# thegedge/StereoReconstruction

Hardware: AMD Instinct MI355X
Metric: Mdisparity-hypotheses/s (WxHxD) (higher is better)
Workload: dtype f64; 1 GPU; C3: synthetic rectified 1920x1080 pair, 256 depth levels, GeodesicWeight r=5; TwoView WTA both directions + cross-check; one pair per GPU; width=1920, height=1080, depth_levels=256, window_radius=5, weights=geodesic, pairs_per_gpu=1, pair_seed_rank0=1592590339, pair_seed_of_rank_r=seed + 0x10000*r, parallelism=single GPU

## Files before the change

### stereoreconstruction_amd/csrc/srh_api.hip

```cpp
#include "srh_internal.hpp"
#include "srh_geom.hpp"

#include <algorithm>
#include <cassert>
#include <cstdarg>
#include <cstdio>
#include <cstdlib>
#include <cstring>
#include <map>
#include <mutex>
#include <string>
#include <utility>
#include <limits>
#include <vector>

using namespace srh;

static thread_local char g_err[512] = "";

static int fail(int code, const char *fmt, ...) {
	va_list ap;
	va_start(ap, fmt);
	vsnprintf(g_err, sizeof(g_err), fmt, ap);
	va_end(ap);
	return code;
}

#define HIP_TRY(expr)                                                                   \
	do {                                                                                \
		hipError_t e_ = (expr);                                                         \
		if (e_ != hipSuccess)                                                           \
			return fail(SRH_E_DEVICE, "%s: %s (%s:%d)", #expr, hipGetErrorString(e_), __FILE__, __LINE__); \
	} while (0)

static thread_local bool g_oom = false;
static thread_local size_t g_alloc_limit = 0;

struct PoolBlock { void *p; size_t bytes; int device; };
static std::mutex g_pool_mu;
static std::vector<PoolBlock> g_pool;
static size_t g_pool_bytes = 0, g_pool_cap = (size_t)65536 << 20;
static const size_t POOL_MIN_BYTES = (size_t)4 << 20;

static void pool_flush(int device) {
	std::vector<PoolBlock> out;
	{
		std::lock_guard<std::mutex> g(g_pool_mu);
		for (size_t k = 0; k < g_pool.size();)
			if (device < 0 || g_pool[k].device == device) { out.push_back(g_pool[k]); g_pool_bytes -= g_pool[k].bytes; g_pool[k] = g_pool.back(); g_pool.pop_back(); }
			else ++k;
	}
	int cur = 0;
	const bool have = hipGetDevice(&cur) == hipSuccess;
	for (const PoolBlock &b : out) { (void)hipSetDevice(b.device); (void)hipFree(b.p); }
	if (have) (void)hipSetDevice(cur);
}
static size_t pool_bytes_on(int device) {
	std::lock_guard<std::mutex> g(g_pool_mu);
	size_t b = 0;
	for (const PoolBlock &k : g_pool) if (k.device == device) b += k.bytes;
	return b;
}
static void pool_give(void *p, size_t bytes) {
	if (!p) return;
	int dev = 0;
	if (bytes >= POOL_MIN_BYTES && hipGetDevice(&dev) == hipSuccess) {
		std::lock_guard<std::mutex> g(g_pool_mu);
		if (g_pool_bytes + bytes <= g_pool_cap) { g_pool.push_back({p, bytes, dev}); g_pool_bytes += bytes; return; }
	}
	(void)hipFree(p);
}
static void *pool_take(size_t bytes, size_t *got) {
	int dev = 0;
	if (bytes < POOL_MIN_BYTES || hipGetDevice(&dev) != hipSuccess) return nullptr;
	std::lock_guard<std::mutex> g(g_pool_mu);
	size_t best = g_pool.size();
	for (size_t k = 0; k < g_pool.size(); ++k)
		if (g_pool[k].device == dev && g_pool[k].bytes >= bytes && g_pool[k].bytes <= bytes + bytes/2 &&
		    (best == g_pool.size() || g_pool[k].bytes < g_pool[best].bytes)) best = k;
	if (best == g_pool.size()) return nullptr;
	void *p = g_pool[best].p;
	*got = g_pool[best].bytes;
	g_pool_bytes -= g_pool[best].bytes;
	g_pool[best] = g_pool.back(); g_pool.pop_back();
	return p;
}

static hipError_t dev_alloc(void **p, size_t bytes, size_t *got) {
	if ((*p = pool_take(bytes, got))) return hipSuccess;
	hipError_t e = hipMalloc(p, bytes);
	if (e == hipErrorOutOfMemory) {
		(void)hipGetLastError();
		int dev = 0;
		if (hipGetDevice(&dev) == hipSuccess && pool_bytes_on(dev)) { pool_flush(dev); e = hipMalloc(p, bytes); }
	}
	if (e != hipSuccess) { *p = nullptr; (void)hipGetLastError(); return e; }
	*got = bytes;
	return hipSuccess;
}

template <class T>
struct DevBuf {
	T *p = nullptr;
	size_t n = 0, block = 0;
	DevBuf() = default;
	DevBuf(DevBuf &&o) noexcept { *this = std::move(o); }
	DevBuf &operator=(DevBuf &&o) noexcept {
		assert(!p && "a held block is released, not overwritten");
		p = o.p; n = o.n; block = o.block;
		o.p = nullptr; o.n = o.block = 0;
		return *this;
	}
	operator T *() const { return p; }
	T *operator->() const { return p; }
	size_t bytes() const { return block; }
	hipError_t alloc(size_t count) {
		void *q = nullptr;
		size_t got = 0;
		const hipError_t e = dev_alloc(&q, count*sizeof(T), &got);
		if (e == hipSuccess) { p = (T *)q; n = got/sizeof(T); block = got; }
		return e;
	}
	int ensure(size_t need) {
		if (n >= need) return SRH_OK;
		if (p) { (void)hipDeviceSynchronize(); release(); }
		if (g_alloc_limit && need*sizeof(T) > g_alloc_limit) {
			g_oom = true;
			return fail(SRH_E_DEVICE, "band buffer of %zu bytes refused (debug_alloc_limit_mb)", need*sizeof(T));
		}
		const hipError_t e = alloc(need);
		if (e == hipErrorOutOfMemory) g_oom = true;
		if (e != hipSuccess) return fail(SRH_E_DEVICE, "hipMalloc of a %zu-byte band buffer: %s", need*sizeof(T), hipGetErrorString(e));
		return SRH_OK;
	}
	void release() { pool_give(p, block); p = nullptr; n = block = 0; }
	void free() { if (p) (void)hipFree(p); p = nullptr; n = block = 0; }
};

struct BandBuffers {
	DevBuf<double> wbuf;
	DevBuf<double> cost;
	DevBuf<double> tnum;
	DevBuf<double> pconst;
	DevBuf<PixRange> prange;
	DevBuf<uint32_t> cflag;
	DevBuf<uint8_t> stpl;
	DevBuf<uint32_t> tileflag;
	DevBuf<int32_t> lcount;
	DevBuf<uint32_t> lcand;
	DevBuf<uint32_t> lrowinfo;
	DevBuf<int32_t> lmeta;
	DevBuf<uint32_t> mvs_wdesc;
	DevBuf<int32_t> mvs_nwin;
	template <class F> void each(F f) {
		f(wbuf); f(cost); f(tnum); f(pconst); f(prange); f(cflag); f(stpl); f(tileflag);
		f(lcount); f(lcand); f(lrowinfo); f(lmeta); f(mvs_wdesc); f(mvs_nwin);
	}
	size_t bytes() { size_t b = 0; each([&](auto &x) { b += x.bytes(); }); return b; }
	void release() { each([](auto &x) { x.release(); }); }
	void free() { each([](auto &x) { x.free(); }); }
};

struct ViewHost {
	int w = 0, h = 0;
	bool present = false;
	DevBuf<uint32_t> rgba;
	DevBuf<uint8_t>  mask;
	DevBuf<double>   gray, gray_tv, depth;
	DevBuf<double>   edges;
	DevBuf<uint8_t>  full;
	int              full_r = 0;
	DevBuf<double>   tvp;   bool tvp_valid = false;
	DevBuf<double>   geo5;  bool geo5_valid = false;
	bool             geo5_denied = false;
	DevBuf<uint8_t>  fullp; int fullp_r = 0;
	DevBuf<uint8_t>  fulls; int fulls_r = 0;
	DevBuf<double>   grayp; bool grayp_valid = false;
	DevBuf<uint8_t>  fullsp; int fullsp_r = 0;
	uint8_t   list_mode[SRH_MAX_VIEWS] = {0};
	DevBuf<uint32_t> act;
	std::vector<uint32_t> act_row, act_host;
	std::vector<uint8_t> hmask;
	bool act_valid = false;
	srh_camera cam;
	DevBuf<int32_t> wta_xy;
	DevBuf<double>  wta_cost;
	int wta_flags = 0, wta_oth = -1;
	DevBuf<double> peaks; int peaks_k = 0;
	DevBuf<double> mrf;
};

struct ProfEntry { double ms = 0; int64_t n = 0; };
struct PendingEvt { std::string name; hipEvent_t a, b; };

#ifndef SRH_MVS_SLOTS
#define SRH_MVS_SLOTS 2
#endif
struct MvsSlot {
	hipStream_t stream = nullptr;
	hipEvent_t ev = nullptr, done = nullptr;
	int *h_maxc = nullptr;
	bool own_buffers = false;
	BandBuffers band;
	DevBuf<Counters> d_cnt; DevBuf<int> d_span;
	bool pending = false;
	int view = -1, nneigh = 0, y0 = 0, y1 = 0, cmax = 0;
	int32_t neigh[SRH_MAX_NEIGH] = {0};
	srh_params p;
};

struct srh_context {
	int device = 0;
	hipStream_t own_stream = nullptr;
	hipStream_t stream = nullptr;
	ViewHost views[SRH_MAX_VIEWS];
	DevBuf<ViewDev> d_views;
	DevBuf<int32_t> d_slots;
	int32_t slots_host[SRH_MAX_VIEWS] = {0}; int slots_n = 0;
	DevBuf<Counters> d_cnt;
	DevBuf<int> d_span;
	BandBuffers band;
	hipStream_t mrf_stream[SRH_MAX_VIEWS] = { nullptr };
	void *mrf_host = nullptr;
	DevBuf<double> mrf_peaks;
	DevBuf<double> mrf;
	int mrf_w = 0, mrf_h = 0, mrf_k = 0;
	DevBuf<double> tvmrf;
	DevBuf<double> tvmrf_costs;
	int tvmrf_w = 0, tvmrf_h = 0, tvmrf_l = 0;
	bool tvmrf_own_costs = false;
	int geodma = 1;
	int tscan = 1;
	int strip = 1;
	int num_cus = 256;
	bool force_walk = false;
	int list_count_pass = 0;
	int list_cmax_hint = 0;
	int list_smax_hint = 0;
	int mvs_cmax_hint = 0;
	hipStream_t side_stream = nullptr;
	hipEvent_t side_go = nullptr, side_done = nullptr;
	int mvs_async = 1;
	MvsSlot mvs_slot[SRH_MVS_SLOTS];
	int mvs_turn = 0, mvs_last = -1;
	bool in_settle = false;
	int mvs_staged = 1;
	bool list_rows = true;
	void *comm = nullptr; int comm_ranks = 0, comm_rank = 0;
	size_t wbuf_budget = (size_t)32768 << 20;
	size_t budget_cap = 0;
	size_t budget_used = 0;
	size_t mem_limit = 0;
	int debug_trace = 0;
	size_t alloc_limit = 0;
	const volatile int *cancel = nullptr;
	srh_progress_fn progress = nullptr;
	void *user = nullptr;
	bool profiling = false;
	bool force_generic = false;
 	bool use_fused = false;
	int arith = 3;
	struct TvDefer { Counters *host = nullptr; int *span = nullptr; bool queued = false, strip = false, cert = false, lists = false, guessed = false;
	                 int cmax = 0, smax = 0, ref = -1, oth = -1; };
	TvDefer tv_defer[2];
	TvDefer *defer = nullptr;
	struct TvSlot {
		hipStream_t stream = nullptr;
		hipEvent_t go = nullptr, done = nullptr;
		DevBuf<Counters> d_cnt; DevBuf<int> d_span;
		BandBuffers band;
	} tv_slot;
	int tv_overlap = 1;
	int f32_form = 0;
	int rows_masked = 1;
	int side_weights = 1;
	int cert_form = 1;
	bool force_dense = false;
	struct Diag { int form = 0; bool raw = false; double *cost = nullptr; size_t cost_doubles = 0; int32_t *range = nullptr;
	              int cstride = 0, rows = 0; bool done = false, strip = false; } *diag = nullptr;
	std::map<std::string, ProfEntry> prof;
	std::vector<PendingEvt> pending;
	srh_stats stats;
	bool last_fused = false;
	int filter_invalid = 0;
	int filter_gap_width = 2;
	int filter_replay = 0;
	int cost_kind = SRH_COST_NCC;
	int sad_dense = 0;
	int wta_outputs = 0;
};

static bool cancelled(srh_context *c) { return c->cancel && *c->cancel; }
static void progress(srh_context *c, int step, const char *stage) { if (c->progress) c->progress(step, stage, c->user); }

static int drain_profile(srh_context *c) {
	for (auto &p : c->pending) {
		float ms = 0;
		HIP_TRY(hipEventSynchronize(p.b));
		HIP_TRY(hipEventElapsedTime(&ms, p.a, p.b));
		ProfEntry &e = c->prof[p.name];
		e.ms += ms; e.n += 1;
		hipEventDestroy(p.a); hipEventDestroy(p.b);
	}
	c->pending.clear();
	return SRH_OK;
}

struct Scope {
// ... 549 lines not shown
	if (runner_xy) HIP_TRY(hipMemcpyAsync(runner_xy, v.wta_xy + 2*n, 2*n*sizeof(int32_t), hipMemcpyDeviceToHost, c->stream));
	if (min_cost) HIP_TRY(hipMemcpyAsync(min_cost, v.wta_cost, n*sizeof(double), hipMemcpyDeviceToHost, c->stream));
	if (second_cost) HIP_TRY(hipMemcpyAsync(second_cost, v.wta_cost + n, n*sizeof(double), hipMemcpyDeviceToHost, c->stream));
	HIP_TRY(hipStreamSynchronize(c->stream));
	return SRH_OK;
}

extern "C" int srh_view_depth_copy_to_device(srh_context *c, int slot, void *dst_dev, size_t dst_bytes) {
	int rc = check_slot(c, slot, true); if (rc) return rc;
	if (!dst_dev) return fail(SRH_E_INVALID, "null destination");
	HIP_TRY(hipSetDevice(c->device));
	const ViewHost &v = c->views[slot];
	if (dst_bytes < (size_t)v.w*v.h*sizeof(double))
		return fail(SRH_E_INVALID, "destination of %zu bytes is smaller than the %dx%d depth map of slot %d", dst_bytes, v.w, v.h, slot);
	HIP_TRY(hipMemcpyAsync(dst_dev, v.depth, (size_t)v.w*v.h*sizeof(double), hipMemcpyDeviceToDevice, c->stream));
	return SRH_OK;
}

extern "C" int srh_view_depth_copy_from_device(srh_context *c, int slot, const void *src_dev, size_t src_bytes) {
	int rc = check_slot(c, slot, true); if (rc) return rc;
	if (!src_dev) return fail(SRH_E_INVALID, "null source");
	HIP_TRY(hipSetDevice(c->device));
	const ViewHost &v = c->views[slot];
	if (src_bytes < (size_t)v.w*v.h*sizeof(double))
		return fail(SRH_E_INVALID, "source of %zu bytes is smaller than the %dx%d depth map of slot %d", src_bytes, v.w, v.h, slot);
	HIP_TRY(hipMemcpyAsync(v.depth, src_dev, (size_t)v.w*v.h*sizeof(double), hipMemcpyDeviceToDevice, c->stream));
	return SRH_OK;
}

static size_t held_band_bytes(srh_context *c) {
	size_t b = c->band.bytes() + c->tv_slot.band.bytes();
	for (MvsSlot &S : c->mvs_slot) b += S.band.bytes();
	for (const ViewHost &v : c->views) b += v.geo5.bytes();
	return b;
}

static size_t band_budget(srh_context *c) {
	size_t b = c->wbuf_budget;
	if (c->budget_cap && b > c->budget_cap) b = c->budget_cap;
	size_t free_b = 0, total_b = 0;
	if (hipMemGetInfo(&free_b, &total_b) == hipSuccess) {
		size_t avail = free_b + held_band_bytes(c) + pool_bytes_on(c->device);
		if (c->mem_limit && avail > c->mem_limit) avail = c->mem_limit;
		if (b > avail/4) b = avail/4;
	} else (void)hipGetLastError();
	if (b < ((size_t)1 << 20)) b = (size_t)1 << 20;
	c->budget_used = b;
	return b;
}

static void release_band_buffers(srh_context *c) {
	pool_flush(c->device);
	c->band.free();
	for (MvsSlot &S : c->mvs_slot) S.band.free();
	c->tv_slot.band.free();
	for (ViewHost &v : c->views)
		if (v.geo5) { v.geo5.free(); v.geo5_valid = false; v.geo5_denied = true; }
}

template <class F>
static int with_thinner_bands(srh_context *c, F body) {
	for (;;) {
		g_oom = false;
		g_alloc_limit = c->alloc_limit;
		const int rc = body();
		if (rc != SRH_E_DEVICE || !g_oom) return rc;
		g_oom = false;
		const size_t used = c->budget_used;
		if (used <= ((size_t)1 << 20)) return rc;
		for (MvsSlot &S : c->mvs_slot) if (S.stream) (void)hipStreamSynchronize(S.stream);
		if (c->side_stream) (void)hipStreamSynchronize(c->side_stream);
		(void)hipStreamSynchronize(c->stream);
		if (c->tv_slot.stream) (void)hipStreamSynchronize(c->tv_slot.stream);
		release_band_buffers(c);
		c->budget_cap = used/2;
		c->stats.band_retries += 1;
	}
}

static int band_rows(srh_context *c, int W, int H, int T) {
	size_t rows = band_budget(c) / ((size_t)T*sizeof(double)*(size_t)W);
	if (rows < 1) rows = 1;
	if (rows > (size_t)H) rows = H;
	return (int)rows;
}

static int fetch_counters(srh_context *c, int used_dense) {
	Counters h;
	HIP_TRY(hipMemcpyAsync(&h, c->d_cnt, sizeof(h), hipMemcpyDeviceToHost, c->stream));
	HIP_TRY(hipStreamSynchronize(c->stream));
	c->stats.n_pixels = (int64_t)h.n_pixels;
	c->stats.n_eval = (int64_t)h.n_eval;
	c->stats.n_eval_device = (int64_t)h.n_eval_device;
	c->stats.scan_tiles_template = (int64_t)h.scan_tiles_template;
	c->stats.scan_tiles_walked = (int64_t)h.scan_tiles_walked;
	c->stats.mvs_waves_staged = (int64_t)h.mvs_waves_staged;
	c->stats.mvs_waves_listed = (int64_t)h.mvs_waves_listed;
	c->stats.used_dense_path = used_dense;
	c->stats.used_fused_kernel = c->last_fused ? 1 : 0;
#ifdef SRH_PROFILE_PHASES
	{
		unsigned long long g[8];
		geodesic_phases_fetch(g);
		if (g[7])
			fprintf(stderr, "[srh prof] geodesic kernel: %llu waves, cycles per wave: staging %.0f  sweeps %.0f  exp %.0f  rows out %.0f  pconst: first sweep %.0f  second sweep %.0f  rest %.0f\n",
			        g[7], (double)g[0]/g[7], (double)g[1]/g[7], (double)g[2]/g[7], (double)g[4]/g[7], (double)g[5]/g[7], (double)g[6]/g[7], (double)g[3]/g[7]);
	}
	if (h.dbg_waves && h.dbg_blocks && h.dbg_phase[3] && h.strip_ticket) {
		const double nw = (double)h.dbg_waves, nt = (double)h.dbg_blocks/nw;
		fprintf(stderr, "[srh dbg] strip: waves %llu, tiles/wave %.1f (%.1f with phase 2), cycles/wave %.0f | per tile: ticket %.0f  own requests %.0f  barriers %.0f  setup %.0f  "
		        "block loops %.0f  p2 lists %.0f  p2 blocks %.0f  p2 singles %.0f\n", h.dbg_waves, nt, (double)h.dbg_cycles/nw, (double)h.dbg_total_cycles/nw,
		        h.dbg_phase[0]/nw/nt, h.dbg_phase[1]/nw/nt, h.dbg_phase[2]/nw/nt, h.dbg_phase[3]/nw/nt, h.dbg_phase[4]/nw/nt,
		        h.dbg_phase[5]/nw/nt, h.dbg_phase[6]/nw/nt, h.dbg_phase[7]/nw/nt);
		static const char *names[8] = { "ticket", "own requests", "barriers", "setup", "block loops", "p2 lists", "p2 blocks", "p2 singles" };
		const int nwv = h.dbg_wave[8*4 + 4] ? 8 : 4;
		for (int k = 0; k < 8; ++k) {
			fprintf(stderr, "[srh dbg]   %-13s by wave:", names[k]);
			for (int w = 0; w < nwv; ++w) fprintf(stderr, " %8.0f", h.dbg_wave[8*k + w]/((double)h.dbg_blocks/nwv));
			fprintf(stderr, "\n");
		}
	} else
	if (h.dbg_waves && !c->last_fused)
		fprintf(stderr, "[srh dbg] dense: waves %llu, cycles/wave %.0f, fast blocks/wave %.1f, cycles/fast block %.0f\n",
		        h.dbg_waves, (double)h.dbg_total_cycles/h.dbg_waves, (double)h.dbg_blocks/h.dbg_waves,
		        h.dbg_blocks ? (double)h.dbg_cycles/h.dbg_blocks : 0.0);
	if (h.dbg_waves && !c->last_fused && !h.strip_ticket)
		fprintf(stderr, "[srh dbg] phases/wave: stage_w %.0f prologue %.0f sync %.0f stage_rt %.0f compute %.0f tail %.0f\n",
		        (double)h.dbg_phase[0]/h.dbg_waves, (double)h.dbg_phase[1]/h.dbg_waves, (double)h.dbg_phase[2]/h.dbg_waves,
		        (double)h.dbg_phase[3]/h.dbg_waves, (double)h.dbg_phase[4]/h.dbg_waves, (double)h.dbg_phase[5]/h.dbg_waves);
	if (h.dbg_waves && c->last_fused)
		fprintf(stderr, "[srh dbg] fused: %llu tiles, %llu with select-form work, %llu pixels with an unusable tap of their own\n",
		        h.dbg_waves, h.n_listed, h.n_slots);
	if (h.dbg_waves && c->last_fused)
		fprintf(stderr, "[srh dbg] fused, role wave cycles/tile: A geometry %.0f  B accept %.0f  C stage %.0f  D prologue %.0f  E1 blocks %.0f  E2 general %.0f  F wta %.0f  barriers %.0f | other waves: blocks %.0f barriers %.0f total %.0f\n",
		        (double)h.dbg_phase[0]/h.dbg_waves, (double)h.dbg_phase[1]/h.dbg_waves, (double)h.dbg_phase[2]/h.dbg_waves,
		        (double)h.dbg_phase[3]/h.dbg_waves, (double)h.dbg_phase[4]/h.dbg_waves, (double)h.dbg_phase[5]/h.dbg_waves,
		        (double)h.dbg_phase[6]/h.dbg_waves, (double)h.dbg_phase[7]/h.dbg_waves,
		        (double)h.dbg_cycles/(3.0*h.dbg_waves), (double)h.dbg_blocks/(3.0*h.dbg_waves), (double)h.dbg_total_cycles/(3.0*h.dbg_waves));
	if (h.dbg_phase[6] && !c->last_fused)
		fprintf(stderr, "[srh dbg] rows: tasks %llu fast %llu, rows/pixel %.2f, slots/px %.1f, wave iterations %llu all-fast %llu\n",
		        h.dbg_phase[6], h.dbg_phase[7], (double)h.dbg_cycles/(double)h.n_pixels, 8.0*h.dbg_phase[6]/(double)h.n_pixels,
		        h.dbg_blocks, h.dbg_total_cycles);
	if (h.dbg_phase[6] && !c->last_fused && h.dbg_wave[8])
		fprintf(stderr, "[srh dbg] rows cost kernel, wave tiles %llu: cycles per tile: staging %.0f  constants %.0f  phase 1 %.0f  p2 blocks %.0f  p2 singles %.0f | tiles with blocks %llu (%llu blocks: %.0f cycles per such tile), with singles %llu (%llu singles: %.0f cycles per such tile); rounds if the tile's tasks were dealt to its 64 lanes: %.2f per tile\n",
		        h.dbg_wave[8], (double)h.dbg_wave[0]/h.dbg_wave[8], (double)h.dbg_wave[1]/h.dbg_wave[8], (double)h.dbg_wave[2]/h.dbg_wave[8],
		        (double)h.dbg_wave[3]/h.dbg_wave[8], (double)h.dbg_wave[4]/h.dbg_wave[8], h.dbg_wave[9], h.dbg_wave[10],
		        h.dbg_wave[9] ? (double)h.dbg_wave[3]/h.dbg_wave[9] : 0.0, h.dbg_wave[11], h.dbg_wave[12], h.dbg_wave[11] ? (double)h.dbg_wave[4]/h.dbg_wave[11] : 0.0, (double)h.dbg_wave[13]/h.dbg_wave[8]);
#endif
	return SRH_OK;
}

static void run_weights(srh_context *c, int ref, int W, const srh_params &p, int by, int nr, size_t wstride,
                        double *pconst = nullptr, bool wimg = false) {
	if (p.weight_kind == SRH_WEIGHT_GEODESIC && !c->force_generic && wimg && c->geodma && p.window_radius == 5 && !c->views[ref].geo5_denied) {
		ViewHost &v = c->views[ref];
		bool ok = true;
		if (!v.geo5) {
			if (v.geo5.alloc(geo5_doubles(v.w, v.h)) != hipSuccess) ok = false;
			v.geo5_valid = false;
		}
		if (ok && !v.geo5_valid) {
			Scope s(c, "geo5_planes_kernel");
			launch_geo5_planes(c->stream, v.edges, v.gray_tv, v.mask, v.w, v.h, v.geo5);
			v.geo5_valid = true;
		}
		if (ok) {
			Scope s(c, "geodesic_dma_kernel");
			if (launch_geodesic_dma(c->stream, c->d_views, ref, W, v.geo5, p, by, nr, c->band.wbuf, pconst, c->num_cus)) return;
		}
	}
	if (p.weight_kind == SRH_WEIGHT_GEODESIC && !c->force_generic) {
		Scope s(c, "geodesic_reg_kernel");
		if (launch_geodesic_reg(c->stream, c->d_views, ref, W, c->views[ref].edges, p, by, nr, c->band.wbuf, wstride, pconst, wimg)) return;
	}
	if (p.weight_kind == SRH_WEIGHT_ADAPTIVE && !c->force_generic) {
		Scope s(c, "adaptive_reg_kernel");
		if (launch_adaptive_reg(c->stream, c->d_views, ref, W, p, by, nr, c->band.wbuf, wstride, pconst, wimg)) return;
	}
	Scope s(c, "weights_kernel");
	launch_weights(c->stream, c->d_views, ref, W, p, by, nr, c->band.wbuf, wstride, pconst, wimg);
}

static bool rig_is_row_aligned(const srh_camera &a, const srh_camera &b, double *fx_bx) {
	if (a.is_distorted || b.is_distorted || a.is_refractive || b.is_refractive) return false;
	for (int k = 0; k < 9; ++k) if (fabs(a.R[k] - b.R[k]) > 1e-13) return false;
	for (int k = 3; k < 9; ++k) if (fabs(a.K[k] - b.K[k]) > 1e-9*(1.0 + fabs(a.K[k]))) return false;
	if (fabs(a.K[1]) > 1e-12 || fabs(b.K[1]) > 1e-12 || fabs(a.K[3]) > 1e-12 || fabs(a.K[6]) > 1e-12 || fabs(a.K[7]) > 1e-12)
		return false;
	const Vec3 d = load3(b.C) - load3(a.C);
	const Vec3 bc = matvec(a.R, d);
	const double len = norm(bc);
	if (!(len > 0) || fabs(bc.y) > 1e-12*len || fabs(bc.z) > 1e-12*len) return false;
	*fx_bx = fabs(b.K[0]*bc.x);
	return true;
}

static int twoview_wta_run(srh_context *c, int ref, int oth, const srh_params *p, int y0, int y1);

static int ensure_wta_planes(srh_context *c, int ref, int oth) {
	ViewHost &v = c->views[ref];
	if (!c->wta_outputs) { v.wta_flags = 0; return SRH_OK; }
	const size_t n = (size_t)v.w*v.h;
	if (v.wta_flags == c->wta_outputs && v.wta_oth == oth) return SRH_OK;
	if (!v.wta_xy) HIP_TRY(v.wta_xy.alloc(4*n));
	if ((c->wta_outputs & SRH_WTA_COSTS) && !v.wta_cost) HIP_TRY(v.wta_cost.alloc(2*n));
	HIP_TRY(hipMemsetAsync(v.wta_xy, 0xff, 4*n*sizeof(int32_t), c->stream));
	if (c->wta_outputs & SRH_WTA_COSTS) launch_fill(c->stream, v.wta_cost, 2*n, __builtin_inf());
	v.wta_flags = c->wta_outputs; v.wta_oth = oth;
	return SRH_OK;
}

static void estimate_list_capacity(const srh_camera &rc, const srh_camera &oc, int W, int H, int OW, int OH,
                                   const srh_params &p, int y0, int y1, int &cmax, int &smax, bool mvs = false)
{
	(void)H;
	const int D = p.num_depth_levels, NL = D < 9 ? D : 9, GX = 13, GY = 9;
	const Vec3 normal = load3(rc.pdir);
	long best_len = 0, best_rows = 0;
	for (int gy = 0; gy < GY; ++gy)
		for (int gx = 0; gx < GX; ++gx) {
			const int x = (int)((gx*(long)(W - 1))/(GX - 1)), y = y0 + (int)((gy*(long)(y1 - y0 - 1))/(GY - 1));
			const Ray ray = cam_unproject(rc, (x + 0.5)/p.image_scale, (y + 0.5)/p.image_scale);
			long len = 0, rows = 0;
			bool have = false;
			int px = 0, py = 0;
			for (int k = 0; k < NL; ++k) {
				const int d = NL > 1 ? (int)(((long)k*(D - 1))/(NL - 1)) : 0;
				Vec3 point = load3(rc.C);
				if (!point_from_depth(ray, normal, depth_from_label(p, mvs, d), point)) continue;
				if (!cam_project(oc, point)) continue;
				const double cxd = fmin(fmax(point.x*p.image_scale, -64.0), (double)OW + 64.0);
				const double cyd = fmin(fmax(point.y*p.image_scale, -64.0), (double)OH + 64.0);
				if (!(cxd == cxd) || !(cyd == cyd)) continue;
				const int ix = (int)cxd, iy = (int)cyd;
				if (have) {
					const long dx = labs((long)ix - px), dy = labs((long)iy - py);
					len += dx > dy ? dx : dy;
					rows += dy;
				}
				have = true; px = ix; py = iy;
			}
			if (len > best_len) best_len = len;
			if (rows > best_rows) best_rows = rows;
		}
	if (best_rows > SRH_ROWS_NR) best_rows = SRH_ROWS_NR;
	long cm = best_len + best_len/8 + (mvs ? 0 : (best_len < D - 1 ? best_len : D - 1)) + 40;
	if (cm > 65520) cm = 65520;
	cmax = (int)((cm + 7) & ~7L);
	long sm = cmax + 8*(best_rows + 2) + 32;
	if (sm > 65528) sm = 65528;
	smax = (int)((sm + 7) & ~7L);
}

static int ensure_sad_planes(srh_context *c, ViewHost &v, int R) {
	if (!v.tvp) HIP_TRY(v.tvp.alloc(padded_size(v.w, v.h)));
	if (!v.tvp_valid) {
		Scope s(c, "padded_plane_kernel");
		launch_padded_plane(c->stream, v.gray_tv, v.w, v.h, v.tvp);
		v.tvp_valid = true;
	}
	if (!v.grayp) HIP_TRY(v.grayp.alloc(padded_size(v.w, v.h)));
	if (!v.grayp_valid) {
		Scope s(c, "padded_gray_kernel");
		launch_padded_gray(c->stream, v.gray, v.mask, v.w, v.h, v.grayp);
		v.grayp_valid = true;
	}
	if (v.fulls_r != R) {
		if (!v.fulls) HIP_TRY(v.fulls.alloc((size_t)v.w*v.h));
		Scope s(c, "sad_full_window_kernel");
		launch_sad_full_window(c->stream, v.mask, v.w, v.h, R, v.fulls);
		v.fulls_r = R;
		v.fullsp_r = 0;
	}
	if (!v.fullsp) HIP_TRY(v.fullsp.alloc(padded_size(v.w, v.h)));
	if (v.fullsp_r != R) {
		Scope s(c, "padded_bytes_kernel");
		launch_padded_bytes(c->stream, v.fulls, v.w, v.h, v.fullsp);
		v.fullsp_r = R;
	}
	return SRH_OK;
}

extern "C" int srh_twoview_wta(srh_context *c, int ref, int oth, const srh_params *p, int y0, int y1) {
	int rc;
	if ((rc = check_slot(c, ref, true)) || (rc = check_slot(c, oth, true)) || (rc = check_params(p))) return rc;
	return with_thinner_bands(c, [&] { return twoview_wta_run(c, ref, oth, p, y0, y1); });
}

static int twoview_wta_run(srh_context *c, int ref, int oth, const srh_params *p, int y0, int y1) {
	int rc;
	if (ref == oth) return fail(SRH_E_INVALID, "ref and other view are the same slot");
	const ViewHost &L = c->views[ref], &Rv = c->views[oth];
	if (L.w != Rv.w || L.h != Rv.h)
		return fail(SRH_E_INVALID, "TwoViewStereo needs equal-sized views (%dx%d vs %dx%d; twoviewstereo.cpp:116-119)",
		            L.w, L.h, Rv.w, Rv.h);
	HIP_TRY(hipSetDevice(c->device));
	const int W = L.w, H = L.h;
	if (y0 < 0) y0 = 0;
	if (y1 <= 0 || y1 > H) y1 = H;
	if (y1 <= y0) return SRH_OK;
	const int R = p->window_radius;
	const int T = (2*R + 1)*(2*R + 1);
	const size_t budget = band_budget(c);
	if (!c->diag && (rc = ensure_wta_planes(c, ref, oth))) return rc;
	int32_t *const wout = (c->wta_outputs && !c->diag) ? (int32_t *)c->views[ref].wta_xy : nullptr;
	auto winner_costs = [&](int by, int nr, bool wimg_layout) {
		if (!wout || !(c->wta_outputs & SRH_WTA_COSTS)) return;
		Scope s(c, "twoview_winner_costs_kernel");
		double *mc = c->views[ref].wta_cost;
		launch_twoview_winner_costs(c->stream, c->d_views, ref, oth, W, *p, c->cost_kind == SRH_COST_SAD, by, nr, c->band.wbuf, wimg_layout,
		                            wout, mc, mc + (size_t)W*H);
	};

	const bool sad = c->cost_kind == SRH_COST_SAD;
	bool dense = !c->force_generic && (!sad || c->sad_dense) && (R == 5 || R == 2);
	int cstride = 0;
	double fx_bx = 0;
	if (dense && !rig_is_row_aligned(L.cam, Rv.cam, &fx_bx)) {
		const bool pinhole = !L.cam.is_distorted && !Rv.cam.is_distorted && !L.cam.is_refractive && !Rv.cam.is_refractive;
		if (c->force_dense && pinhole) fx_bx = (double)(W + 8)/(p->image_scale*fabs(1.0/p->min_depth - 1.0/p->max_depth));
		else dense = false;
	}
	if (dense) {
		const double span = fx_bx*p->image_scale*fabs(1.0/p->min_depth - 1.0/p->max_depth);
		if (!(p->min_depth > 0) || !(p->max_depth > 0) || !(span < 4096.0)) dense = false;
		else cstride = (((int)ceil(span) + 3) + 7) & ~7;
		if (cstride > W + 8) cstride = (W + 8 + 7) & ~7;
		if (sad && dense && cstride + SRH_WTILE > strip_chunk_columns()) dense = false;
	}

	c->last_fused = false;
	if (dense && !sad && c->use_fused && (c->arith == 0 || c->arith == 3) && p->num_depth_levels <= SRH_FUSED_MAXC &&
	    fx_bx*p->image_scale*fabs(1.0/p->min_depth - 1.0/p->max_depth) + 1.0 <= (double)SRH_FUSED_MAXC) {
// ... 101 lines not shown
							}
						}
					}
				}
				for (int by = y0; by < y1; by += (int)lrows) {
					if (cancelled(c)) return fail(SRH_E_CANCELLED, "cancelled");
					const int nr = std::min((int)lrows, y1 - by);
					int32_t *cnt_band = c->band.lcount + (size_t)(by - y0)*W;
					if (rows_mode) {
						if (!c->side_stream) {
							HIP_TRY(hipStreamCreateWithFlags(&c->side_stream, hipStreamNonBlocking));
							HIP_TRY(hipEventCreateWithFlags(&c->side_go, hipEventDisableTiming));
							HIP_TRY(hipEventCreateWithFlags(&c->side_done, hipEventDisableTiming));
						}
						HIP_TRY(hipEventRecord(c->side_go, c->stream));
						{ Scope s(c, "twoview_rows_list_kernel");
						  launch_twoview_rows_list(c->stream, c->d_views, ref, oth, W, *p, by, nr, c->band.lcand, cmax,
						                           cnt_band, c->band.lrowinfo, c->band.lmeta, smax, c->d_cnt, c->d_span, c->band.tnum); }
						if (c->side_weights) {
							HIP_TRY(hipStreamWaitEvent(c->side_stream, c->side_go, 0));
							std::swap(c->stream, c->side_stream);
							run_weights(c, ref, W, *p, by, nr, SRH_WTILE, rows_pc ? c->band.pconst : nullptr, true);
							std::swap(c->stream, c->side_stream);
							HIP_TRY(hipEventRecord(c->side_done, c->side_stream));
							HIP_TRY(hipStreamWaitEvent(c->stream, c->side_done, 0));
						} else run_weights(c, ref, W, *p, by, nr, SRH_WTILE, rows_pc ? c->band.pconst : nullptr, true);
						if (rows_cert) HIP_TRY(hipMemsetAsync(c->band.cflag, 0, sizeof(uint32_t), c->stream));
						HIP_TRY(hipMemsetAsync(&c->d_cnt->strip_ticket, 0, 2*sizeof(unsigned int), c->stream));
						if (sad) {
							Scope s(c, "twoview_rows_sad_kernel");
							launch_twoview_rows_sad(c->stream, c->d_views, ref, oth, W, *p, by, nr, c->band.wbuf, O.fulls,
							                        c->band.lrowinfo, c->band.lmeta, c->band.cost, smax, c->d_cnt);
						} else
						{ Scope s(c, "twoview_rows_cost_kernel");
						  launch_twoview_rows_cost(c->stream, c->d_views, ref, oth, W, *p, by, nr, c->band.wbuf, O.full,
						                           c->band.lrowinfo, c->band.lmeta, c->band.cost, smax, c->d_cnt, rows_cert ? (c->cert_form == 1 ? 5 : 3) : 0,
						                           rows_pc ? c->band.pconst : nullptr, rows_cert && c->rows_masked ? O.tvp : nullptr, c->num_cus,
						                           c->rows_masked == 1 ? (const uint32_t *)(O.full + full_stat_offset((size_t)O.w*O.h)) : nullptr); }
						{ Scope s(c, "twoview_rows_scan_kernel");
						  launch_twoview_rows_scan(c->stream, c->d_views, ref, oth, W, *p, by, nr, cnt_band, c->band.lcand, cmax,
						                           c->band.lrowinfo, c->band.lmeta, c->band.cost, smax, rows_cert ? c->band.cflag : nullptr, -1, c->d_cnt, wout); }
						if (rows_cert) {
							const int cap = redo_capacity((size_t)nr*W);
							{ Scope s(c, "twoview_rows_refill_kernel");
							  launch_twoview_rows_refill(c->stream, W, O.w, *p, by, c->band.cflag, cap, c->band.wbuf, c->views[ref].tvp, O.tvp,
							                             c->band.lrowinfo, c->band.lmeta, c->band.cost, smax, c->d_cnt); }
							Scope s(c, "twoview_rows_rescan_kernel");
							launch_twoview_rows_scan(c->stream, c->d_views, ref, oth, W, *p, by, nr, cnt_band, c->band.lcand, cmax,
							                         c->band.lrowinfo, c->band.lmeta, c->band.cost, smax, c->band.cflag, cap, c->d_cnt, wout);
						}
						winner_costs(by, nr, true);
						continue;
					}
					run_weights(c, ref, W, *p, by, nr, SRH_WTILE);
					{ Scope s(c, "twoview_list_kernel");
					  launch_twoview_list(c->stream, c->d_views, ref, oth, W, *p, by, nr, c->band.lcand, cmax,
					                      cnt_band, c->d_cnt, c->d_span, c->band.tnum); }
					if (sad) {
						Scope s(c, "twoview_list_sad_kernel");
						launch_twoview_list_sad(c->stream, c->d_views, ref, oth, W, *p, by, nr, c->band.wbuf,
						                        cnt_band, c->band.lcand, c->band.cost, cmax, c->d_cnt);
					} else
					{ Scope s(c, "twoview_list_cost_kernel");
					  launch_twoview_list_cost(c->stream, c->d_views, ref, oth, W, *p, by, nr, c->band.wbuf, O.full,
					                           cnt_band, c->band.lcand, c->band.cost, cmax, c->d_cnt); }
					{ Scope s(c, "twoview_list_scan_kernel");
					  launch_twoview_list_scan(c->stream, c->d_views, ref, oth, W, *p, by, nr, cnt_band, c->band.lcand, c->band.cost, cmax, wout); }
					winner_costs(by, nr, false);
				}
				if (c->defer && attempt == 0 && pass == 0 && rows_mode &&
				    ((c->list_cmax_hint > 0 && c->list_smax_hint > 0 && c->views[ref].list_mode[oth] == 1) ||
				     (guessed && c->views[ref].list_mode[oth] == 0))) {
					HIP_TRY(hipMemcpyAsync(c->defer->host, c->d_cnt, sizeof(Counters), hipMemcpyDeviceToHost, c->stream));
					HIP_TRY(hipMemcpyAsync(c->defer->span, c->d_span, 4*sizeof(int), hipMemcpyDeviceToHost, c->stream));
					c->defer->queued = true; c->defer->lists = true; c->defer->strip = false; c->defer->cert = rows_cert;
					c->defer->cmax = cmax; c->defer->smax = smax;
					c->defer->guessed = guessed; c->defer->ref = ref; c->defer->oth = oth;
					if (c->debug_trace) fprintf(stderr, "[srh trace] lists %d>%d queued unverified: cmax %d smax %d guessed %d\n", ref, oth, cmax, smax, (int)guessed);
					c->stats.used_strip_kernel = 0;
					c->stats.used_dense_path = 0;
					HIP_TRY(hipGetLastError());
					return SRH_OK;
				}
				int mx[4] = { 0, 0, 0, 0 };
				HIP_TRY(hipMemcpyAsync(mx, c->d_span, 4*sizeof(int), hipMemcpyDeviceToHost, c->stream));
				HIP_TRY(hipStreamSynchronize(c->stream));
				const int maxc = mx[0];
				if (c->debug_trace) fprintf(stderr, "[srh trace] lists %d>%d verified pass %d: cmax %d smax %d guessed %d -> longest list %d, slots %d, rows over %d\n",
				                            ref, oth, pass, cmax, smax, (int)guessed, mx[0], mx[1], mx[2]);
				if (rows_mode) {
					const int need = (mx[1] + 7) & ~7;
					if (mx[2] || need > 65528) {
						rows_mode = false; c->views[ref].list_mode[oth] = 2;
						if (maxc > cmax) cmax = (maxc + 7) & ~7;
						continue;
					}
					if (maxc <= cmax && need <= smax) {
						const int cm = guessed ? std::max(8, (maxc + 7) & ~7) : cmax;
						const int sm = guessed ? std::max(cm + 64, need) : smax;
						if (cm > c->list_cmax_hint) c->list_cmax_hint = cm;
						if (sm > c->list_smax_hint) c->list_smax_hint = sm;
						Counters hc;
						HIP_TRY(hipMemcpyAsync(&hc, c->d_cnt, sizeof(hc), hipMemcpyDeviceToHost, c->stream));
						HIP_TRY(hipStreamSynchronize(c->stream));
						c->views[ref].list_mode[oth] = (hc.n_slots > 2.2*(double)hc.n_listed) ? 2 : 1;
						if (hc.cert_overflow != 0) { cert_ok = false; continue; }
						if (rows_cert) { c->stats.n_certified = (int64_t)hc.n_pixels; c->stats.n_flagged = (int64_t)hc.n_flagged; }
						break;
					}
					if (maxc > cmax) { cmax = (maxc + 7) & ~7; if (need <= smax) smax = std::max(smax, cmax + 64); }
					if (need > smax) smax = need;
					guessed = false;
					continue;
				}
				if (maxc <= cmax) {
					const int cm = guessed ? std::max(8, (maxc + 7) & ~7) : cmax;
					if (cm > c->list_cmax_hint) c->list_cmax_hint = cm;
					break;
				}
				cmax = (maxc + 7) & ~7;
				guessed = false;
			}
			HIP_TRY(hipGetLastError());
			break;
		}
		const bool tscan = dense && c->tscan != 0;
		if (dense) {
			if ((rc = c->band.tnum.ensure((size_t)p->num_depth_levels + 8))) return rc;
			{ Scope s(c, "pinhole_label_table_kernel");
			  launch_pinhole_label_table(c->stream, c->d_views, ref, *p, false, c->band.tnum); }
			if (tscan) {
				if ((rc = c->band.stpl.ensure(scan_template_bytes()))) return rc;
				Scope s(c, "twoview_template_kernel");
				launch_scan_template(c->stream, c->d_views, ref, oth, *p, y0, y1 - y0, c->band.tnum, c->band.stpl);
			}
		}
		size_t rows = 0;
		for (int pass = 0; pass < 2; ++pass) {
			const int wdoubles = strip ? (2*R + 1)*wimg_wp(R) : T;
			const size_t per_pixel = (size_t)wdoubles*sizeof(double) + (dense ? (size_t)cstride*sizeof(double) : 0);
			rows = budget / (per_pixel*(size_t)W);
			if (rows < 1) rows = 1;
			if (rows > (size_t)(y1 - y0)) rows = (size_t)(y1 - y0);
			if (strip && !sad && c->strip == 1 && (size_t)((W + SRH_WTILE - 1)/SRH_WTILE)*rows < (size_t)48*2*c->num_cus) strip = false;
			else break;
		}
		const bool wimg = strip;
		const size_t wstride = SRH_WTILE;
		if ((rc = c->band.wbuf.ensure(wimg ? wimg_doubles(W, (int)rows, R) : wbuf_doubles(W, (int)rows, T)))) return rc;
		if (dense && (rc = c->band.cost.ensure(rows*(size_t)((W + 31)/32)*32*(size_t)cstride))) return rc;
		if (dense && (rc = c->band.pconst.ensure((rows*(size_t)W + SRH_WTILE)*SRH_PC))) return rc;
		int lanes = 8;
		if (dense && (rc = c->band.prange.ensure(rows*(size_t)W + SRH_WTILE))) return rc;
		if (tscan && (rc = c->band.tileflag.ensure(rows*(size_t)((W + 63)/64) + 1))) return rc;
		const bool cert = dense && cert_ok;
		const int cost_arith = c->arith == 3 ? (cert ? (c->cert_form == 1 ? 5 : 3) : 0) : c->arith;
		if (cert && (rc = c->band.cflag.ensure(rows*(size_t)W + 1))) return rc;
		const bool planes = dense && (R == 5 || R == 2);
		if (strip) lanes = strip_block_lanes(cstride, c->strip == 1 ? 0 : c->strip);
		if (planes) {
			for (int k = 0; k < 2; ++k) {
				ViewHost &v = c->views[k == 0 ? ref : oth];
				if (!v.tvp) HIP_TRY(v.tvp.alloc(padded_size(v.w, v.h)));
				if (!v.tvp_valid) {
					Scope s(c, "padded_plane_kernel");
					launch_padded_plane(c->stream, v.gray_tv, v.w, v.h, v.tvp);
					v.tvp_valid = true;
				}
			}
		}
		if (strip && sad) {
			if ((rc = ensure_sad_planes(c, c->views[oth], R))) return rc;
		} else if (strip) {
			ViewHost &O = c->views[oth];
			if (!O.fullp) HIP_TRY(O.fullp.alloc(padded_size(O.w, O.h)));
			if (O.fullp_r != R) {
				Scope s(c, "padded_full_kernel");
				launch_padded_full(c->stream, O.gray_tv, O.w, O.h, R, O.fullp);
				O.fullp_r = R;
			}
		}

		for (int by = y0; by < y1; by += (int)rows) {
			if (cancelled(c)) return fail(SRH_E_CANCELLED, "cancelled");
			const int nr = std::min((int)rows, y1 - by);
			run_weights(c, ref, W, *p, by, nr, wstride, dense && !sad ? c->band.pconst : nullptr, wimg);
			if (dense) {
				Scope s(c, "pixel_range_kernel");
				launch_pixel_range(c->stream, c->d_views, ref, oth, W, *p, by, nr, c->band.tnum, cstride, c->band.prange);
			}
			if (dense) {
				auto cost_pass = [&](int arith) -> int {
					if (sad) {
						HIP_TRY(hipMemsetAsync(&c->d_cnt->strip_ticket, 0, 2*sizeof(unsigned int), c->stream));
						Scope s(c, "twoview_strip_sad_kernel");
						if (!launch_twoview_strip_sad(c->stream, W, H, *p, by, nr, c->band.wbuf, c->band.prange, c->views[ref].tvp,
						                              c->views[oth].grayp, c->views[oth].fullsp, c->band.cost, cstride, c->d_cnt, c->num_cus))
							return fail(SRH_E_UNSUPPORTED, "twoview_strip_sad_kernel: no instantiation for radius %d", R);
					} else if (strip) {
						HIP_TRY(hipMemsetAsync(&c->d_cnt->strip_ticket, 0, 2*sizeof(unsigned int), c->stream));
						{ Scope s(c, "twoview_strip_cost_kernel");
						  launch_twoview_strip_cost(c->stream, c->d_views, ref, oth, W, H, *p, by, nr, c->band.wbuf, c->band.pconst, c->band.prange,
						                            c->views[ref].tvp, c->views[oth].tvp, c->views[oth].fullp, c->band.cost, cstride,
						                            c->d_cnt, arith, c->num_cus, lanes, c->diag && c->diag->raw); }
						Scope s(c, "twoview_lazy_fill_kernel");
						launch_twoview_lazy_fill(c->stream, c->d_views, ref, oth, W, *p, by, nr, c->band.prange, c->band.wbuf, wstride,
						                         c->views[ref].tvp, c->views[oth].tvp, true, lanes, lanes == 8, c->band.cost, cstride, c->d_cnt);
					} else {
						{ Scope s(c, "twoview_dense_cost_kernel");
						  if (arith == 2)
							launch_twoview_dense_cost_f32(c->stream, c->d_views, ref, oth, W, *p, by, nr, c->band.wbuf, wstride,
							                              c->band.tnum, c->band.cost, cstride, c->d_cnt, c->band.pconst, c->f32_form);
						  else
							launch_twoview_dense_cost(c->stream, c->d_views, ref, oth, W, *p, by, nr, c->band.wbuf, wstride,
							                          c->band.tnum, c->band.cost, cstride, c->d_cnt, c->band.pconst, arith, c->band.prange); }
						Scope s(c, "twoview_lazy_fill_kernel");
						launch_twoview_lazy_fill(c->stream, c->d_views, ref, oth, W, *p, by, nr, c->band.prange, c->band.wbuf, wstride,
						                         planes ? c->views[ref].tvp : nullptr, planes ? c->views[oth].tvp : nullptr, false, 8,
						                         arith != 5, c->band.cost, cstride, c->d_cnt);
					}
					return SRH_OK;
				};
				if (c->diag) {
					srh_context::Diag &dg = *c->diag;
					dg.cstride = cstride; dg.rows = nr; dg.strip = strip;
					const size_t nd = (size_t)nr*((W + 31)/32)*32*(size_t)cstride;
					if (by != y0 || nr != y1 - y0) return fail(SRH_E_UNSUPPORTED, "cost rows: the rows asked for do not fit one band (%d of %d)", nr, y1 - y0);
					if (dg.cost) {
						if (dg.cost_doubles < nd) return fail(SRH_E_INVALID, "cost rows: buffer of %zu doubles, %zu needed", dg.cost_doubles, nd);
						HIP_TRY(hipMemsetAsync(c->band.cost, 0xff, nd*sizeof(double), c->stream));
						if ((rc = cost_pass(dg.form))) return rc;
						HIP_TRY(hipMemcpyAsync(dg.cost, c->band.cost, nd*sizeof(double), hipMemcpyDeviceToHost, c->stream));
						if (dg.range) HIP_TRY(hipMemcpyAsync(dg.range, c->band.prange, (size_t)nr*W*sizeof(PixRange), hipMemcpyDeviceToHost, c->stream));
						HIP_TRY(hipStreamSynchronize(c->stream));
					}
					dg.done = true;
					return SRH_OK;
				}
				if (cert) HIP_TRY(hipMemsetAsync(c->band.cflag, 0, sizeof(uint32_t), c->stream));
				if ((rc = cost_pass(cost_arith))) return rc;
				{ Scope s(c, "twoview_scan_kernel");
				  launch_twoview_scan(c->stream, c->d_views, ref, oth, W, *p, by, nr, c->band.tnum, c->band.cost, cstride, c->d_cnt, c->band.prange,
				                      cert ? c->band.cflag : nullptr, -1, cert && strip ? c->band.pconst : nullptr, tscan ? c->band.stpl : nullptr, c->band.tileflag, c->num_cus, wout); }
				if (cert) {
					const int cap = redo_capacity((size_t)nr*W);
					{ Scope s(c, "twoview_refill_kernel");
					  launch_twoview_refill(c->stream, W, *p, by, c->band.prange, c->band.cflag, cap, c->band.wbuf, wimg, c->views[ref].tvp,
					                        c->views[oth].tvp, c->band.cost, cstride, c->d_cnt); }
					Scope s(c, "twoview_rescan_kernel");
					launch_twoview_scan(c->stream, c->d_views, ref, oth, W, *p, by, nr, c->band.tnum, c->band.cost, cstride, c->d_cnt, c->band.prange,
					                    c->band.cflag, cap, nullptr, nullptr, nullptr, c->num_cus, wout);
				}
				winner_costs(by, nr, wimg);
			} else {
				{ Scope s(c, "twoview_generic_kernel");
				  launch_twoview_generic(c->stream, c->d_views, ref, oth, W, *p, by, nr, c->band.wbuf, wstride, c->d_cnt, sad, wout); }
				winner_costs(by, nr, false);
			}
		}
		HIP_TRY(hipGetLastError());
		if (!dense) break;
		if (c->defer && attempt == 0) {
			HIP_TRY(hipMemcpyAsync(c->defer->host, c->d_cnt, sizeof(Counters), hipMemcpyDeviceToHost, c->stream));
			c->defer->queued = true; c->defer->strip = strip; c->defer->cert = cert_ok;
			c->stats.used_strip_kernel = strip ? 1 : 0;
			c->stats.used_dense_path = 1;
			return SRH_OK;
		}
		Counters hc;
		HIP_TRY(hipMemcpyAsync(&hc, c->d_cnt, sizeof(hc), hipMemcpyDeviceToHost, c->stream));
		HIP_TRY(hipStreamSynchronize(c->stream));
		if (strip && sad && hc.strip_overflow != 0) { strip = false; dense = false; continue; }
		if (strip && hc.strip_overflow != 0) { strip = false; continue; }
		if (hc.cert_overflow != 0) { cert_ok = false; continue; }
		c->stats.n_certified = (int64_t)hc.n_certified; c->stats.n_flagged = (int64_t)hc.n_flagged;
		if (hc.not_row_aligned == 0) break;
		dense = false;
		strip = false;
	}
	c->stats.used_strip_kernel = strip ? 1 : 0;
	c->stats.used_dense_path = dense ? 1 : 0;
	return SRH_OK;
}

extern "C" int srh_twoview_cost_rows(srh_context *c, int ref, int oth, const srh_params *p, int y0, int y1, int form, int raw,
                                     double *cost_out, size_t cost_doubles, int32_t *range_out, int *cstride_out, int *used_strip)
{
	int rc;
	if ((rc = check_slot(c, ref, true)) || (rc = check_slot(c, oth, true)) || (rc = check_params(p))) return rc;
	if (form != 0 && form != 3 && form != 5 && form != 1) return fail(SRH_E_INVALID, "form must be 0, 1, 3 or 5");
	if ((form == 3 || form == 5) && !cert_bound(*p).ok) return fail(SRH_E_UNSUPPORTED, "the parameters leave the error bound no room");
	const bool sad = c->cost_kind == SRH_COST_SAD;
	if (sad && !c->sad_dense) return fail(SRH_E_UNSUPPORTED, "cost rows of cost_sad exist on the dense plan only (option sad_dense)");
	if (sad && form != 0) return fail(SRH_E_INVALID, "cost_sad has the reference's arithmetic only: form must be 0");
	srh_context::Diag dg;
	dg.form = form; dg.raw = raw != 0; dg.cost = cost_out; dg.cost_doubles = cost_doubles; dg.range = range_out;
	c->diag = &dg;
	const int keep_arith = c->arith; const bool keep_fused = c->use_fused;
	c->arith = form == 0 ? 0 : 3; c->use_fused = false;
	rc = twoview_wta_run(c, ref, oth, p, y0, y1);
	c->arith = keep_arith; c->use_fused = keep_fused;
	c->diag = nullptr;
	if (rc) return rc;
	if (!dg.done) return fail(SRH_E_UNSUPPORTED, "cost rows exist on the row-aligned dense plan only (radius 5 or 2, rectified pinhole pair)");
	if (cstride_out) *cstride_out = dg.cstride;
	if (used_strip) *used_strip = dg.strip ? 1 : 0;
	return SRH_OK;
}

extern "C" int srh_twoview_pair_costs(srh_context *c, int ref, int oth, const srh_params *p, int kind, int n,
                                      const int32_t *xy, double *out)
{
	int rc;
	if ((rc = check_slot(c, ref, true)) || (rc = check_slot(c, oth, true)) || (rc = check_params(p))) return rc;
	if (kind != SRH_COST_NCC && kind != SRH_COST_SAD) return fail(SRH_E_INVALID, "kind must be SRH_COST_NCC or SRH_COST_SAD");
	if (n < 0 || (n > 0 && (!xy || !out))) return fail(SRH_E_INVALID, "null pairs or output");
	if (p->window_radius > 5) return fail(SRH_E_UNSUPPORTED, "pair costs take window radii up to 5");
	if (n == 0) return SRH_OK;
	const ViewHost &L = c->views[ref];
	for (int k = 0; k < n; ++k)
		if (xy[4*k] < 0 || xy[4*k + 1] < 0 || xy[4*k] >= L.w || xy[4*k + 1] >= L.h)
			return fail(SRH_E_INVALID, "pair %d: reference pixel (%d, %d) outside the %dx%d view", k, xy[4*k], xy[4*k + 1], L.w, L.h);
	HIP_TRY(hipSetDevice(c->device));
	DevBuf<int32_t> dxy; DevBuf<double> dout;
	HIP_TRY(dxy.alloc((size_t)4*n));
	HIP_TRY(dout.alloc((size_t)n));
	HIP_TRY(hipMemcpyAsync(dxy, xy, (size_t)4*n*sizeof(int32_t), hipMemcpyHostToDevice, c->stream));
	{ Scope s(c, "pair_costs_kernel");
	  launch_pair_costs(c->stream, c->d_views, ref, oth, *p, kind == SRH_COST_SAD, n, dxy, dout); }
	HIP_TRY(hipGetLastError());
	HIP_TRY(hipMemcpyAsync(out, dout, (size_t)n*sizeof(double), hipMemcpyDeviceToHost, c->stream));
	HIP_TRY(hipStreamSynchronize(c->stream));
	dxy.free(); dout.free();
	return SRH_OK;
}

extern "C" int srh_debug_exp(srh_context *c, const double *x, int n, double *kernel_out, double *library_out) {
	if (!c || !x || !kernel_out || !library_out || n < 1) return fail(SRH_E_INVALID, "null argument");
	HIP_TRY(hipSetDevice(c->device));
	DevBuf<double> d;
	HIP_TRY(d.alloc((size_t)n*3));
	hipError_t e = hipMemcpyAsync(d, x, (size_t)n*sizeof(double), hipMemcpyHostToDevice, c->stream);
	if (e == hipSuccess) {
		launch_geo_exp_probe(c->stream, d, n, d + n, d + 2*(size_t)n);
		e = hipMemcpyAsync(kernel_out, d + n, (size_t)n*sizeof(double), hipMemcpyDeviceToHost, c->stream);
	}
	if (e == hipSuccess) e = hipMemcpyAsync(library_out, d + 2*(size_t)n, (size_t)n*sizeof(double), hipMemcpyDeviceToHost, c->stream);
	if (e == hipSuccess) e = hipStreamSynchronize(c->stream);
	d.free();
	if (e != hipSuccess) return fail(SRH_E_DEVICE, "srh_debug_exp: %s", hipGetErrorString(e));
	return SRH_OK;
}

extern "C" int srh_twoview_cross_check(srh_context *c, int left, int right, const srh_params *p) {
	int rc;
// ... 1218 lines not shown
```

### stereoreconstruction_amd/csrc/srh_dense.hip

```cpp
#include "srh_internal.hpp"
#include "srh_geom.hpp"
#include "srh_walk.hpp"

#include <algorithm>
#include <type_traits>
#include <utility>

namespace srh {

__device__ __forceinline__ double color_dist_u(uint32_t a, uint32_t b) {
	const double dr = (double)((int)(a & 255u) - (int)(b & 255u));
	const double dg = (double)((int)((a >> 8) & 255u) - (int)((b >> 8) & 255u));
	const double db = (double)((int)((a >> 16) & 255u) - (int)((b >> 16) & 255u));
	return sqrt(dr*dr + dg*dg + db*db);
}

__global__ void edge_planes_kernel(const uint32_t *__restrict__ rgba, int W, int H, double *__restrict__ edges)
{
	const size_t n = (size_t)W*H;
	const double inf = __builtin_inf();
	for (size_t i = (size_t)blockIdx.x*blockDim.x + threadIdx.x; i < n; i += (size_t)gridDim.x*blockDim.x) {
		const int x = (int)(i % (size_t)W), y = (int)(i / (size_t)W);
		const uint32_t c = rgba[i];
		edges[0*n + i] = (x + 1 < W) ? color_dist_u(rgba[i + 1], c) : inf;
// ... 67 lines not shown
	GEO_EACH(p[j] = __builtin_fma(r[j], p[j], GEO_D(0x3fe000000000000b)))
	GEO_EACH(p[j] = __builtin_fma(r[j], p[j], 1.0))
	GEO_EACH(p[j] = __builtin_fma(r[j], p[j], 1.0))
	GEO_EACH(p[j] = __builtin_ldexp(p[j], (int)n[j]))
	if constexpr (RANGE) {
		GEO_EACH(asm volatile("" : "+v"(p[j])))
		GEO_EACH(p[j] = x[j] < -1075.0 ? 0.0 : p[j])
		GEO_EACH(x[j] = x[j] > 1024.0 ? __builtin_inf() : p[j])
	} else {
		GEO_EACH(x[j] = p[j])
	}
}
template <int WS, int B0, int N>
__device__ __forceinline__ void geo_exp_chunk(double (&w)[WS], const SharedDivisor &sg, bool fast, double sigma) {
	double x[N];
	if (fast) {
		double m[N];
		GEO_EACH(x[j] = -w[B0 + j])
		GEO_EACH(m[j] = x[j]*sg.r)
		GEO_EACH(x[j] = __builtin_fma(-sg.b, m[j], x[j]))
		GEO_EACH(x[j] = __builtin_fma(x[j], sg.r, m[j]))
		geo_exp_n<N, false>(x);
	} else {
		GEO_EACH(x[j] = -w[B0 + j] / sigma)
		geo_exp_n<N, true>(x);
	}
	GEO_EACH(w[B0 + j] = x[j])
}
#undef GEO_EACH
template <int WS, int B0 = 0>
__device__ __forceinline__ void geo_exp_row(double (&w)[WS], const SharedDivisor &sg, bool fast, double sigma) {
	if constexpr (B0 < WS) {
		constexpr int N = WS - B0 < GEO_EXPN ? WS - B0 : ((WS - B0 > GEO_EXPN && WS - B0 < 2*GEO_EXPN) ? (WS - B0 + 1)/2 : GEO_EXPN);
		geo_exp_chunk<WS, B0, N>(w, sg, fast, sigma);
		geo_exp_row<WS, B0 + N>(w, sg, fast, sigma);
	}
}

__global__ void geo_exp_probe_kernel(const double *__restrict__ x, int n, double *__restrict__ kout, double *__restrict__ lout) {
	const int k = blockIdx.x*blockDim.x + threadIdx.x;
	if (k >= n) return;
	double a[1] = { x[k] }, b[1] = { x[k] };
	geo_exp_n<1, true>(a);
	if (x[k] <= 0.0 && x[k] >= -0x1p30) { geo_exp_n<1, false>(b); if (__builtin_bit_cast(unsigned long long, a[0]) != __builtin_bit_cast(unsigned long long, b[0])) a[0] = __builtin_nan(""); }
	kout[k] = a[0];
	lout[k] = exp(x[k]);
}
void launch_geo_exp_probe(hipStream_t st, const double *x, int n, double *kout, double *lout) {
	hipLaunchKernelGGL(geo_exp_probe_kernel, dim3((unsigned)((n + 255)/256)), dim3(256), 0, st, x, n, kout, lout);
}
template <int R, int TWD, int PL, int S>
__device__ __forceinline__ void geo_edges(GeoLds tb, double &e0, double &e1, double &e2, double &e3) {
	using C = GeoCell<R, S>;
	constexpr int yy = C::yy, xx = C::xx;
	if constexpr (C::fwd) {
		if constexpr (C::c0) e0 = tb[2*PL + (yy-1)*TWD + xx - 1];
		if constexpr (C::c1) e1 = tb[1*PL + (yy-1)*TWD + xx];
		if constexpr (C::c2) e2 = tb[3*PL + (yy-1)*TWD + xx + 1];
		if constexpr (C::c3) e3 = tb[0*PL + yy*TWD + xx - 1];
	} else {
		if constexpr (C::c0) e0 = tb[3*PL + yy*TWD + xx];
		if constexpr (C::c1) e1 = tb[1*PL + yy*TWD + xx];
		if constexpr (C::c2) e2 = tb[2*PL + yy*TWD + xx];
		if constexpr (C::c3) e3 = tb[0*PL + yy*TWD + xx];
	}
}
template <int R, int TWD, int PL, int KA, int NS, int S>
__device__ __forceinline__ void geo_step(double (&w)[2*R+1][2*R+1], double (&er)[KA][4], GeoLds tb) {
	using C = GeoCell<R, S>;
	constexpr int yy = C::yy, xx = C::xx, dy = C::fwd ? -1 : 1, dx = C::fwd ? -1 : 1;
	double (&e)[4] = er[S % KA];
	double wt = w[yy][xx];
	if constexpr (C::c0) wt = geo_min(w[yy+dy][xx-1] + e[0], wt);
	if constexpr (C::c1) wt = geo_min(w[yy+dy][xx]   + e[1], wt);
	if constexpr (C::c2) wt = geo_min(w[yy+dy][xx+1] + e[2], wt);
	if constexpr (C::c3) wt = geo_min(w[yy][xx+dx]   + e[3], wt);
	w[yy][xx] = wt;
	__builtin_amdgcn_sched_barrier(0);
	if constexpr (S + KA < NS) {
		geo_edges<R, TWD, PL, S + KA>(tb, e[0], e[1], e[2], e[3]);
		__builtin_amdgcn_sched_barrier(0);
	}
}
template <int R, int TWD, int PL, int KA, int... S>
__device__ __forceinline__ void geo_prologue(double (&er)[KA][4], GeoLds tb, std::integer_sequence<int, S...>) {
	(geo_edges<R, TWD, PL, S>(tb, er[S][0], er[S][1], er[S][2], er[S][3]), ...);
}
template <int R, int TWD, int PL, int KA, int NS, int... S>
__device__ __forceinline__ void geo_iteration(double (&w)[2*R+1][2*R+1], double (&er)[KA][4], GeoLds tb, std::integer_sequence<int, S...>) {
	(geo_step<R, TWD, PL, KA, NS, S>(w, er, tb), ...);
}
template <int R, int TWD, int TH>
__device__ __forceinline__ void geodesic_sweeps(double (&w)[2*R+1][2*R+1], GeoLds tb, int iters) {
	constexpr int WS = 2*R + 1, NS = 2*WS*WS, KA = GEO_AHEAD < NS ? GEO_AHEAD : NS, PL = TH*TWD;
	double er[KA][4];
#pragma unroll 1
	for (int iter = 0; iter < iters; ++iter) {
		geo_prologue<R, TWD, PL, KA>(er, tb, std::make_integer_sequence<int, KA>{});
		__builtin_amdgcn_sched_barrier(0);
		geo_iteration<R, TWD, PL, KA, NS>(w, er, tb, std::make_integer_sequence<int, NS>{});
	}
}

template <int R, int TWD, int KG, int J>
__device__ __forceinline__ void geo_pc1_step(const double (&w)[2*R+1][2*R+1], GeoLds tg, double (&g)[KG], double (&pr)[4],
                                             double &mL, double &tw, double &wmin) {
	constexpr int WS = 2*R + 1, NT = WS*WS, LAG = 2;
	if constexpr (J < NT) {
		pr[J % 4] = w[J / WS][J % WS]*g[J % KG];
		wmin = geo_min(wmin, w[J / WS][J % WS]);
	}
	if constexpr (J >= LAG) {
		mL += pr[(J - LAG) % 4];
		tw += w[(J - LAG) / WS][(J - LAG) % WS];
	}
	__builtin_amdgcn_sched_barrier(0);
	if constexpr (J + KG < NT) { g[J % KG] = tg[((J + KG) / WS)*TWD + (J + KG) % WS]; __builtin_amdgcn_sched_barrier(0); }
}
template <int R, int TWD, int KG, int J>
__device__ __forceinline__ void geo_pc2_step(const double (&w)[2*R+1][2*R+1], GeoLds tg, double (&g)[KG], double (&pr)[4],
                                             double mL, double &s2, double (&fa)[2], double &sa) {
	constexpr int WS = 2*R + 1, NT = WS*WS;
	if constexpr (J < NT) pr[J % 4] = w[J / WS][J % WS]*g[J % KG];
	if constexpr (J < NT) fa[J % 2] = __builtin_fma(w[J / WS][J % WS], g[J % KG], -mL);
	if constexpr (J >= 1 && J - 1 < NT) sa += fa[(J - 1) % 2];
	if constexpr (J >= 1 && J - 1 < NT) pr[(J - 1) % 4] = pr[(J - 1) % 4] - mL;
	if constexpr (J >= 2 && J - 2 < NT) pr[(J - 2) % 4] = pr[(J - 2) % 4]*pr[(J - 2) % 4];
	if constexpr (J >= 3) s2 += pr[(J - 3) % 4];
	__builtin_amdgcn_sched_barrier(0);
	if constexpr (J + KG < NT) { g[J % KG] = tg[((J + KG) / WS)*TWD + (J + KG) % WS]; __builtin_amdgcn_sched_barrier(0); }
}
template <int R, int TWD, int KG, int... J>
__device__ __forceinline__ void geo_pc_fill(GeoLds tg, double (&g)[KG], std::integer_sequence<int, J...>) {
	((g[J] = tg[(J / (2*R+1))*TWD + J % (2*R+1)]), ...);
	__builtin_amdgcn_sched_barrier(0);
}
template <int R, int TWD, int KG, int... J>
__device__ __forceinline__ void geo_pc1(const double (&w)[2*R+1][2*R+1], GeoLds tg, double (&g)[KG], double &mL, double &tw, double &wmin,
                                        std::integer_sequence<int, J...>) {
	double pr[4];
	(geo_pc1_step<R, TWD, KG, J>(w, tg, g, pr, mL, tw, wmin), ...);
}
template <int R, int TWD, int KG, int... J>
__device__ __forceinline__ void geo_pc2(const double (&w)[2*R+1][2*R+1], GeoLds tg, double (&g)[KG], double mL, double &s2, double &sa,
                                        std::integer_sequence<int, J...>) {
	double pr[4], fa[2];
	(geo_pc2_step<R, TWD, KG, J>(w, tg, g, pr, mL, s2, fa, sa), ...);
}

template <int R, bool WIMG>
__global__ __launch_bounds__(GW_TW*GW_ROWS)
void geodesic_reg_kernel(const ViewDev *__restrict__ views, int ref, const double *__restrict__ edges,
                         srh_params P, int y0, int nrows, double *__restrict__ wbuf, size_t wstride,
                         double *__restrict__ pconst)
{
	constexpr int WS = 2*R + 1;
	constexpr int TWD = GW_TW + 2*R;
	const ViewDev &V = views[ref];
	const int W = V.w, H = V.h;
	const size_t n = (size_t)W*H;
	constexpr int TH = WS + GW_ROWS - 1;
	constexpr int NT = GW_TW*GW_ROWS;
	const int tiles_per_row = (W + GW_TW - 1)/GW_TW;
	const int tgrp = blockIdx.x / tiles_per_row;
	const int x0 = (blockIdx.x % tiles_per_row)*GW_TW;
	const int wv = threadIdx.x / GW_TW;
	const int trow = tgrp*GW_ROWS + wv;
	const int cy0 = y0 + tgrp*GW_ROWS;
	const int cy = cy0 + wv;
	const bool rowok = trow < nrows;
#ifdef SRH_PROFILE_PHASES
	unsigned long long gph_t = __builtin_amdgcn_s_memtime(), gph[7] = {0, 0, 0, 0, 0, 0, 0};
#endif

	__shared__ double tile[5][TH][TWD];
	const double inf = __builtin_inf();
	const int cxm = x0 + (int)(threadIdx.x % GW_TW);
	if constexpr (!WIMG) {
		const bool act_ = rowok && cxm < W && V.mask[(size_t)cy*W + cxm] == 1;
		if (!__syncthreads_or(act_)) return;
	}
	{
		constexpr int NB = (TH*TWD + NT - 1)/NT;
		double t0[NB], t1[NB], t2[NB], t3[NB], t4[NB];
		const uint8_t mk = (WIMG && rowok && cxm < W) ? V.mask[(size_t)cy*W + cxm] : (uint8_t)0;
#pragma unroll
		for (int k = 0; k < NB; ++k) {
			const int idx = threadIdx.x + k*NT;
			const int ty = idx / TWD, tx = idx % TWD;
			const int gx = x0 - R + tx, gy = cy0 - R + ty;
			const bool in = idx < TH*TWD && gx >= 0 && gy >= 0 && gx < W && gy < H;
			const size_t gi = in ? (size_t)gy*W + gx : 0;
			t0[k] = in ? edges[0*n + gi] : inf;
			t1[k] = in ? edges[1*n + gi] : inf;
			t2[k] = in ? edges[2*n + gi] : inf;
			t3[k] = in ? edges[3*n + gi] : inf;
			t4[k] = (pconst && in) ? V.gray_tv[gi] : __builtin_nan("");
		}
		if constexpr (WIMG) {
			if (!__syncthreads_or(mk == 1)) return;
		}
#pragma unroll
		for (int k = 0; k < NB; ++k) {
			const int idx = threadIdx.x + k*NT;
			if (idx < TH*TWD) {
				const int ty = idx / TWD, tx = idx % TWD;
				tile[0][ty][tx] = t0[k]; tile[1][ty][tx] = t1[k]; tile[2][ty][tx] = t2[k]; tile[3][ty][tx] = t3[k];
				tile[4][ty][tx] = t4[k];
			}
		}
	}
	__syncthreads();

	const int i = threadIdx.x % GW_TW;
	const int cx = x0 + i;
	const bool active = rowok && cx < W && V.mask[(size_t)(rowok ? cy : y0)*W + (cx < W ? cx : 0)] == 1;
	const unsigned long long amask = WIMG ? __ballot(active) : 0ull;
	if (!WIMG && !active) return;

	GEO_STAMP(0)
	double w[WS][WS];
#pragma unroll
	for (int a = 0; a < WS; ++a)
#pragma unroll
		for (int b = 0; b < WS; ++b) w[a][b] = P.geodesic_init;
	w[R][R] = 0.0;

	geodesic_sweeps<R, TWD, TH>(w, (GeoLds)&tile[0][wv][i], P.geodesic_iters);
	GEO_STAMP(1)
	const SharedDivisor sg = shared_divisor(P.geodesic_sigma);
	const bool sdiv = sg.ok && P.geodesic_sigma > 0 && P.geodesic_init > 0x1p-300 && P.geodesic_init < 0x1p300 && P.geodesic_init < 0x1p30*P.geodesic_sigma;
	if constexpr (WIMG) {
		constexpr int WP = (WS + 1) & ~1;
		static_assert(GW_TW == 2*SRH_WTILE, "a wave covers two window-buffer tiles");
		__shared__ __align__(16) double stage_buf[GW_ROWS][GW_TW*WP];
		double *stage = stage_buf[wv];
		double *wt = wbuf + wimg_offset(W, R, rowok ? trow : 0, x0);
		constexpr size_t TILE_D = (size_t)SRH_WTILE*WS*WP;
		constexpr int NPIECE = GW_TW*WP/2, NK = (NPIECE + GW_TW - 1)/GW_TW;
		bool st[NK];
		unsigned goff[NK];
#pragma unroll
		for (int k = 0; k < NK; ++k) {
			const int q = i + k*GW_TW;
			const int pix = (2*q)/WP;
			const int half = pix/SRH_WTILE;
			st[k] = q < NPIECE && ((amask >> pix) & 1ull);
			goff[k] = (unsigned)(half*(int)TILE_D + (2*q - half*SRH_WTILE*WP));
		}
#pragma unroll
		for (int a = 0; a < WS; ++a) {
			__builtin_amdgcn_fence(__ATOMIC_ACQ_REL, "wavefront");
			__builtin_amdgcn_wave_barrier();
			geo_exp_row<WS>(w[a], sg, sdiv, P.geodesic_sigma);
			GEO_STAMP(2)
#pragma unroll
			for (int b = 0; b + 1 < WS; b += 2) {
				double2 v; v.x = w[a][b]; v.y = w[a][b + 1];
				*reinterpret_cast<double2 *>(stage + i*WP + b) = v;
			}
			stage[i*WP + WS - 1] = w[a][WS - 1];
			__builtin_amdgcn_fence(__ATOMIC_ACQ_REL, "wavefront");
			__builtin_amdgcn_wave_barrier();
			double2 v[NK];
#pragma unroll
			for (int k = 0; k < NK; ++k) v[k] = *reinterpret_cast<const double2 *>(stage + 2*((i + k*GW_TW) < NPIECE ? (i + k*GW_TW) : 0));
#pragma unroll
			for (int k = 0; k < NK; ++k) asm volatile("" : "+v"(v[k].x), "+v"(v[k].y));
			double *wrow = wt + (size_t)a*(SRH_WTILE*WP);
#pragma unroll
			for (int k = 0; k < NK; ++k)
				if (st[k]) { typedef double d2v __attribute__((ext_vector_type(2))); d2v t; t.x = v[k].x; t.y = v[k].y; __builtin_nontemporal_store(t, reinterpret_cast<d2v *>(wrow + goff[k])); }
			GEO_STAMP(4)
		}
	} else {
		double *wb = wbuf + wbuf_offset(W, WS*WS, trow, cx);
#pragma unroll
		for (int a = 0; a < WS; ++a) {
			geo_exp_row<WS>(w[a], sg, sdiv, P.geodesic_sigma);
#pragma unroll
			for (int b = 0; b < WS; ++b) __builtin_nontemporal_store(w[a][b], &wb[(size_t)(a*WS + b)*wstride]);
			asm volatile("" ::: "memory");
		}
	}
	GEO_STAMP(2)
	if (pconst && active) {
		constexpr int NT = WS*WS, KG = GEO_AHEAD < NT ? GEO_AHEAD : NT;
		const GeoLds tg = (GeoLds)&tile[4][wv][i];
		double g[KG];
		double mL = 0, tw = 0, wmin = __builtin_inf();
		geo_pc_fill<R, TWD, KG>(tg, g, std::make_integer_sequence<int, KG>{});
		geo_pc1<R, TWD, KG>(w, tg, g, mL, tw, wmin, std::make_integer_sequence<int, NT + 2>{});
		bool all = mL == mL && wmin > P.weight_cutoff;
		GEO_STAMP(5)
		double s2 = 0, sa = 0;
		if (all && !(tw < 1e-10)) {
			mL /= tw;
			geo_pc_fill<R, TWD, KG>(tg, g, std::make_integer_sequence<int, KG>{});
			geo_pc2<R, TWD, KG>(w, tg, g, mL, s2, sa, std::make_integer_sequence<int, NT + 3>{});
			GEO_STAMP(6)
		} else all = false;
		double *pc = pconst + ((size_t)trow*W + cx)*SRH_PC;
		pc[0] = mL; pc[1] = tw; pc[2] = s2; pc[3] = all ? 1.0/tw : 0.0;
		pc[4] = sa; pc[5] = 0.0;
	}
#ifdef SRH_PROFILE_PHASES
	GEO_STAMP(3)
	if (i == 0 && rowok) {
		for (int k = 0; k < 7; ++k) atomicAdd(&g_geo_phase[k], gph[k]);
		atomicAdd(&g_geo_phase[7], 1ull);
	}
#endif
}
#undef GEO_STAMP

#define GD_ROWS 4
#define GD_PADL 5
#define GD_PADR 70
#define GD_PADT 5
#define GD_PADB (5 + GD_ROWS - 1)
static inline __host__ __device__ int geo5_stride(int w) { return (w + GD_PADL + GD_PADR + 1) & ~1; }
static inline __host__ __device__ int geo5_rows(int h) { return h + GD_PADT + GD_PADB; }
static inline __host__ __device__ int geo5_mstride(int w) { return (w + 64 + 3) & ~3; }
static inline __host__ __device__ size_t geo5_plane_doubles(int w, int h) { return (size_t)5*geo5_stride(w)*geo5_rows(h); }
size_t geo5_doubles(int w, int h) { return geo5_plane_doubles(w, h) + ((size_t)geo5_mstride(w)*(h + 4) + 7)/8; }

__global__ void geo5_planes_kernel(const double *__restrict__ edges, const double *__restrict__ gray_tv,
                                   const uint8_t *__restrict__ mask, int W, int H, double *__restrict__ out)
{
	{
		uint8_t *mo = (uint8_t *)(out + geo5_plane_doubles(W, H));
		const int MS = geo5_mstride(W);
		const size_t mt = (size_t)MS*(H + 4);
		for (size_t q = (size_t)blockIdx.x*blockDim.x + threadIdx.x; q < mt; q += (size_t)gridDim.x*blockDim.x) {
			const int y = (int)(q / MS), x = (int)(q % MS);
			mo[q] = (x < W && y < H) ? mask[(size_t)y*W + x] : (uint8_t)0;
		}
	}
	const int GS = geo5_stride(W), GR = geo5_rows(H);
	const size_t n = (size_t)W*H, pl = (size_t)GS*GR, tot = 5*pl;
	for (size_t q = (size_t)blockIdx.x*blockDim.x + threadIdx.x; q < tot; q += (size_t)gridDim.x*blockDim.x) {
		const int k = (int)(q / pl);
		const size_t r = q - (size_t)k*pl;
		const int y = (int)(r / GS) - GD_PADT, x = (int)(r % GS) - GD_PADL;
		const bool in = x >= 0 && y >= 0 && x < W && y < H;
		out[q] = k < 4 ? (in ? edges[(size_t)k*n + (size_t)y*W + x] : __builtin_inf())
		               : (in ? gray_tv[(size_t)y*W + x] : __builtin_nan(""));
	}
}
void launch_geo5_planes(hipStream_t st, const double *edges, const double *gray_tv, const uint8_t *mask, int w, int h, double *out) {
	hipLaunchKernelGGL(geo5_planes_kernel, dim3(4096), dim3(256), 0, st, edges, gray_tv, mask, w, h, out);
}

template <int R>
__global__ __launch_bounds__(GW_TW*GD_ROWS)
void geodesic_dma_kernel(const ViewDev *__restrict__ views, int ref, const double *__restrict__ geo5,
                         srh_params P, int y0, int nrows, double *__restrict__ wbuf, double *__restrict__ pconst)
{
	static_assert(R == GD_PADL, "the padded planes are laid out for this radius");
	constexpr int WS = 2*R + 1, TWD = GW_TW + 2*R, TH = WS + GD_ROWS - 1, PL = TH*TWD;
	constexpr int TILE_BYTES = 5*PL*8, NPC = (TILE_BYTES + 1023)/1024;
	constexpr int WP = (WS + 1) & ~1;
	static_assert((TWD*8) % 16 == 0 && GW_TW == 2*SRH_WTILE, "tile rows are whole 16-byte pieces; a wave covers two window-buffer tiles");
	const ViewDev &V = views[ref];
	const int W = V.w, H = V.h;
	const int GS = geo5_stride(W);
	const size_t GPL = (size_t)GS*geo5_rows(H);
	const int tiles_per_row = (W + GW_TW - 1)/GW_TW;
	const int total_tiles = tiles_per_row*((nrows + GD_ROWS - 1)/GD_ROWS);
	const int wv = threadIdx.x / GW_TW, i = threadIdx.x % GW_TW;
	__shared__ __align__(16) double tile[2][5][TH][TWD];
	__shared__ __align__(16) double stage_buf[GD_ROWS][GW_TW*WP];
	__shared__ __align__(16) unsigned mtile[2][GD_ROWS][GW_TW/4];
	double *stage = stage_buf[wv];
	typedef __attribute__((address_space(3))) void lvoid;
	const int MS = geo5_mstride(W);
	const char *gm5 = (const char *)(geo5 + geo5_plane_doubles(W, H));

	auto request = [&](int tl, int buf) {
		const int tg = tl / tiles_per_row, xa = (tl % tiles_per_row)*GW_TW, ya = y0 + tg*GD_ROWS;
		const char *org = (const char *)geo5 + ((size_t)(ya - R + GD_PADT)*GS + (size_t)(xa - R + GD_PADL))*8;
#pragma unroll
		for (int p = wv; p < NPC; p += GD_ROWS) {
			const int o = p*1024 + i*16;
			if (o < TILE_BYTES) {
				const int plane = o / (PL*8), rem = o - plane*(PL*8), row = rem / (TWD*8), colb = rem - row*(TWD*8);
				const char *src = org + ((size_t)plane*GPL + (size_t)row*GS)*8 + colb;
				const unsigned dst = (unsigned)(size_t)(lvoid *)((char *)&tile[buf][0][0][0] + p*1024);
				asm volatile("s_mov_b32 m0, %1\n\ts_nop 0\n\tglobal_load_lds_dwordx4 %0, off" :: "v"(src), "s"(__builtin_amdgcn_readfirstlane(dst)) : "m0", "memory");
			}
		}
		if (i < GW_TW/4) {
			const char *src = gm5 + (size_t)(ya + wv)*MS + xa + 4*i;
			const unsigned dst = (unsigned)(size_t)(lvoid *)&mtile[buf][wv][0];
			asm volatile("s_mov_b32 m0, %1\n\ts_nop 0\n\tglobal_load_lds_dword %0, off" :: "v"(src), "s"(__builtin_amdgcn_readfirstlane(dst)) : "m0", "memory");
		}
	};
	int tl = blockIdx.x;
	if (tl >= total_tiles) return;
	request(tl, 0);
	asm volatile("s_waitcnt vmcnt(0)" ::: "memory");
	const SharedDivisor sg = shared_divisor(P.geodesic_sigma);
	const bool sdiv = sg.ok && P.geodesic_sigma > 0 && P.geodesic_init > 0x1p-300 && P.geodesic_init < 0x1p300 && P.geodesic_init < 0x1p30*P.geodesic_sigma;
#pragma unroll 1
	for (int kt = 0; tl < total_tiles; ++kt, tl += gridDim.x) {
		const int buf = kt & 1;
		const int tgrp = tl / tiles_per_row, x0 = (tl % tiles_per_row)*GW_TW;
		const int trow = tgrp*GD_ROWS + wv;
		const bool rowok = trow < nrows;
		const int cx = x0 + i;
		__syncthreads();
		const bool active = rowok && cx < W && ((const volatile __attribute__((address_space(3))) uint8_t *)&mtile[buf][wv][0])[i] == 1;
		if (tl + (int)gridDim.x < total_tiles) request(tl + gridDim.x, buf ^ 1);
		const unsigned long long amask = __ballot(active);
		if (amask == 0ull) { asm volatile("s_waitcnt vmcnt(0)" ::: "memory"); continue; }

		double w[WS][WS];
#pragma unroll
		for (int a = 0; a < WS; ++a)
#pragma unroll
			for (int b = 0; b < WS; ++b) w[a][b] = P.geodesic_init;
		w[R][R] = 0.0;
		geodesic_sweeps<R, TWD, TH>(w, (GeoLds)&tile[buf][0][wv][i], P.geodesic_iters);
		asm volatile("s_waitcnt vmcnt(0)" ::: "memory");

		{
			double *wt = wbuf + wimg_offset(W, R, rowok ? trow : 0, x0);
			constexpr size_t TILE_D = (size_t)SRH_WTILE*WS*WP;
			constexpr int NPIECE = GW_TW*WP/2, NK = (NPIECE + GW_TW - 1)/GW_TW;
			bool st[NK];
			unsigned goff[NK];
#pragma unroll
			for (int k = 0; k < NK; ++k) {
				const int q = i + k*GW_TW;
				const int pix = (2*q)/WP;
				const int half = pix/SRH_WTILE;
				st[k] = q < NPIECE && ((amask >> pix) & 1ull);
				goff[k] = (unsigned)(half*(int)TILE_D + (2*q - half*SRH_WTILE*WP));
			}
#pragma unroll
			for (int a = 0; a < WS; ++a) {
				__builtin_amdgcn_fence(__ATOMIC_ACQ_REL, "wavefront");
				__builtin_amdgcn_wave_barrier();
				geo_exp_row<WS>(w[a], sg, sdiv, P.geodesic_sigma);
#pragma unroll
				for (int b = 0; b + 1 < WS; b += 2) {
					double2 v; v.x = w[a][b]; v.y = w[a][b + 1];
					*reinterpret_cast<double2 *>(stage + i*WP + b) = v;
				}
				stage[i*WP + WS - 1] = w[a][WS - 1];
				__builtin_amdgcn_fence(__ATOMIC_ACQ_REL, "wavefront");
				__builtin_amdgcn_wave_barrier();
				double2 v[NK];
#pragma unroll
				for (int k = 0; k < NK; ++k) v[k] = *reinterpret_cast<const double2 *>(stage + 2*((i + k*GW_TW) < NPIECE ? (i + k*GW_TW) : 0));
#pragma unroll
				for (int k = 0; k < NK; ++k) asm volatile("" : "+v"(v[k].x), "+v"(v[k].y));
				double *wrow = wt + (size_t)a*(SRH_WTILE*WP);
#pragma unroll
				for (int k = 0; k < NK; ++k)
					if (st[k]) { typedef double d2v __attribute__((ext_vector_type(2))); d2v t; t.x = v[k].x; t.y = v[k].y; __builtin_nontemporal_store(t, reinterpret_cast<d2v *>(wrow + goff[k])); }
			}
		}
		if (pconst && active) {
			constexpr int NT = WS*WS, KG = GEO_AHEAD < NT ? GEO_AHEAD : NT;
			const GeoLds tg = (GeoLds)&tile[buf][4][wv][i];
			double g[KG];
			double mL = 0, tw = 0, wmin = __builtin_inf();
			geo_pc_fill<R, TWD, KG>(tg, g, std::make_integer_sequence<int, KG>{});
			geo_pc1<R, TWD, KG>(w, tg, g, mL, tw, wmin, std::make_integer_sequence<int, NT + 2>{});
			bool all = mL == mL && wmin > P.weight_cutoff;
			double s2 = 0, sa = 0;
			if (all && !(tw < 1e-10)) {
				mL /= tw;
				geo_pc_fill<R, TWD, KG>(tg, g, std::make_integer_sequence<int, KG>{});
				geo_pc2<R, TWD, KG>(w, tg, g, mL, s2, sa, std::make_integer_sequence<int, NT + 3>{});
			} else all = false;
			double *pc = pconst + ((size_t)trow*W + cx)*SRH_PC;
			pc[0] = mL; pc[1] = tw; pc[2] = s2; pc[3] = all ? 1.0/tw : 0.0;
			pc[4] = sa; pc[5] = 0.0;
		}
	}
}

bool launch_geodesic_dma(hipStream_t st, const ViewDev *views, int ref, int width, const double *geo5, const srh_params &P,
                         int y0, int nrows, double *wbuf, double *pconst, int num_cus)
{
	if (P.window_radius != GD_PADL) return false;
	const int tiles = (width + GW_TW - 1)/GW_TW, total = tiles*((nrows + GD_ROWS - 1)/GD_ROWS);
	const int grid = total < num_cus ? total : num_cus;
	hipLaunchKernelGGL((geodesic_dma_kernel<GD_PADL>), dim3((unsigned)grid), dim3(GW_TW*GD_ROWS), 0, st, views, ref, geo5, P, y0, nrows, wbuf, pconst);
	return true;
}

#define AW_TW 64
template <int R>
__global__ __launch_bounds__(AW_TW)
void adaptive_reg_kernel(const ViewDev *__restrict__ views, int ref, srh_params P, int y0, int nrows,
                         double *__restrict__ wbuf, size_t wstride, double *__restrict__ pconst, int wimg)
{
	constexpr int WS = 2*R + 1, TWD = AW_TW + 2*R;
	const ViewDev &V = views[ref];
	const int W = V.w, H = V.h;
	const int tiles = (W + AW_TW - 1)/AW_TW;
	const int trow = blockIdx.x / tiles, x0 = (blockIdx.x % tiles)*AW_TW;
	const int cy = y0 + trow;
	const int i = threadIdx.x, cx = x0 + i;
	__shared__ uint32_t ct[WS][TWD];
	__shared__ double gt[WS][TWD];
	for (int k = i; k < WS*TWD; k += AW_TW) {
		const int ty = k / TWD, tx = k % TWD;
		const int gx = x0 - R + tx, gy = cy - R + ty;
		const bool in = gx >= 0 && gy >= 0 && gx < W && gy < H;
		ct[ty][tx] = in ? V.rgba[(size_t)gy*W + gx] : 0u;
		gt[ty][tx] = (pconst && in) ? V.gray_tv[(size_t)gy*W + gx] : __builtin_nan("");
	}
	__syncthreads();
	if (cx >= W || V.mask[(size_t)cy*W + cx] != 1) return;
	double dw[R + 1];
#pragma unroll
	for (int k = 0; k <= R; ++k) dw[k] = exp(-k / (1.0*R));
	const uint32_t crgb = ct[R][i + R];
	double *wb = wbuf + (wimg ? wimg_offset(W, R, trow, cx) : wbuf_offset(W, WS*WS, trow, cx));
	const size_t wra = wimg ? (size_t)wimg_row_stride(R) : (size_t)WS*wstride, wcb = wimg ? 1 : wstride;
	bool all = true;
	double mL = 0, tw = 0;
#pragma unroll 1
	for (int a = 0; a < WS; ++a) {
		const int py = cy - R + a;
		const double dwr = dw[a < R ? R - a : a - R];
#pragma unroll
		for (int b = 0; b < WS; ++b) {
			const int px = cx - R + b;
			double weight = 0.0;
			if (!(px < 0 || py < 0 || px >= W || py >= H)) {
				const uint32_t q = ct[a][i + b];
				const double dr = (double)((int)(q & 255u) - (int)(crgb & 255u));
				const double dg = (double)((int)((q >> 8) & 255u) - (int)((crgb >> 8) & 255u));
				const double db = (double)((int)((q >> 16) & 255u) - (int)((crgb >> 16) & 255u));
				const double diff = sqrt(dr*dr + dg*dg + db*db);
				const double w1 = dwr*dw[b < R ? R - b : b - R];
				const double w2 = exp(-diff / P.adaptive_color_sigma);
				weight = w1*w2;
				if (weight != weight) weight = 0.0;
			}
			wb[(size_t)a*wra + (size_t)b*wcb] = weight;
			if (pconst) {
				const double gl = gt[a][i + b];
				if (!(gl == gl && weight > P.weight_cutoff)) all = false;
				mL += weight*gl;
				tw += weight;
			}
		}
	}
	if (pconst) {
		double s2 = 0, sa = 0;
		if (all && !(tw < 1e-10)) {
			mL /= tw;
#pragma unroll 1
			for (int a = 0; a < WS; ++a) {
				double wr[WS];
#pragma unroll
				for (int b = 0; b < WS; ++b) wr[b] = wb[(size_t)a*wra + (size_t)b*wcb];
#pragma unroll
				for (int b = 0; b < WS; ++b) { const double t = wr[b]*gt[a][i + b] - mL; s2 += t*t; sa += __builtin_fma(wr[b], gt[a][i + b], -mL); }
			}
		} else all = false;
		double *pc = pconst + ((size_t)trow*W + cx)*SRH_PC;
		pc[0] = mL; pc[1] = tw; pc[2] = s2; pc[3] = all ? 1.0/tw : 0.0;
		pc[4] = sa; pc[5] = 0.0;
	}
}

bool launch_adaptive_reg(hipStream_t st, const ViewDev *views, int ref, int width, const srh_params &P, int y0, int nrows,
                         double *wbuf, size_t wstride, double *pconst, bool wimg)
{
	if (wstride != SRH_WTILE) return false;
	const dim3 grid((unsigned)(((width + AW_TW - 1)/AW_TW)*nrows)), block(AW_TW);
	if (P.window_radius == 5) hipLaunchKernelGGL(adaptive_reg_kernel<5>, grid, block, 0, st, views, ref, P, y0, nrows, wbuf, wstride, pconst, wimg ? 1 : 0);
	else if (P.window_radius == 2) hipLaunchKernelGGL(adaptive_reg_kernel<2>, grid, block, 0, st, views, ref, P, y0, nrows, wbuf, wstride, pconst, wimg ? 1 : 0);
	else return false;
	return true;
}

bool launch_geodesic_reg(hipStream_t st, const ViewDev *views, int ref, int width, const double *edges,
                         const srh_params &P, int y0, int nrows, double *wbuf, size_t wstride, double *pconst, bool wimg)
{
	const int tiles = (width + GW_TW - 1)/GW_TW;
	const dim3 grid((unsigned)(tiles*((nrows + GW_ROWS - 1)/GW_ROWS))), block(GW_TW*GW_ROWS);
	const int wi = wimg ? 1 : 0;
	switch (P.window_radius) {
	case 5:
		if (wi) hipLaunchKernelGGL((geodesic_reg_kernel<5, true>), grid, block, 0, st, views, ref, edges, P, y0, nrows, wbuf, wstride, pconst);
		else    hipLaunchKernelGGL((geodesic_reg_kernel<5, false>), grid, block, 0, st, views, ref, edges, P, y0, nrows, wbuf, wstride, pconst);
		return true;
	case 2:
		if (wi) hipLaunchKernelGGL((geodesic_reg_kernel<2, true>), grid, block, 0, st, views, ref, edges, P, y0, nrows, wbuf, wstride, pconst);
		else    hipLaunchKernelGGL((geodesic_reg_kernel<2, false>), grid, block, 0, st, views, ref, edges, P, y0, nrows, wbuf, wstride, pconst);
		return true;
	default: return false;
	}
}

__global__ void pinhole_label_table_kernel(const ViewDev *__restrict__ views, int ref, srh_params P, int mvs,
                                           double *__restrict__ tnum)
{
	const int d = blockIdx.x*blockDim.x + threadIdx.x;
	if (d < P.num_depth_levels) tnum[d] = pinhole_label_tnum(views[ref].cam, P, mvs != 0, d);
}

__global__ void label_plane_table_kernel(const ViewDev *__restrict__ views, int ref, srh_params P, int mvs,
                                         double *__restrict__ tdist)
{
	const int d = blockIdx.x*blockDim.x + threadIdx.x;
	if (d < P.num_depth_levels) tdist[d] = label_plane_dist(views[ref].cam, P, mvs != 0, d);
}

void launch_label_plane_table(hipStream_t st, const ViewDev *views, int ref, const srh_params &P, bool mvs, double *tdist) {
	hipLaunchKernelGGL(label_plane_table_kernel, dim3((unsigned)((P.num_depth_levels + 63)/64)), dim3(64), 0, st,
	                   views, ref, P, mvs ? 1 : 0, tdist);
}

void launch_pinhole_label_table(hipStream_t st, const ViewDev *views, int ref, const srh_params &P, bool mvs, double *tnum) {
	hipLaunchKernelGGL(pinhole_label_table_kernel, dim3((unsigned)((P.num_depth_levels + 63)/64)), dim3(64), 0, st,
	                   views, ref, P, mvs ? 1 : 0, tnum);
}

#define DC_TP 32
#define DC_G 8
#define DC_THREADS (DC_TP*DC_G)

template <int R, int DC_NCB, int DC_CHUNK>
struct DenseSmem {
	static constexpr int WS = 2*R + 1;
	static constexpr int T = WS*WS;
	static constexpr int WP = (WS + 1) & ~1;
	static constexpr int WPIX = WS*WP;
	static constexpr int RW = DC_CHUNK + 2*R + DC_NCB + 2;
	static constexpr int LW = DC_TP + 2*R;
	double w[DC_TP][WPIX];
	double rt[WS][RW];
	double lt[WS][LW];
	double meanL[DC_TP], totalW[DC_TP], sum2[DC_TP], sumA[DC_TP];
	int lall[DC_TP];
	int pxmin[DC_TP], pxmax[DC_TP];
	unsigned char rfull[RW];
	unsigned char colok[RW];
	static constexpr int GL_CAP = 2048;
	static_assert(DC_CHUNK <= 512 && DC_TP <= 64, "work-list entry = pixel*512 + column in 16 bits");
	unsigned short glist[GL_CAP];
	int glist_n;
};

template <int R, int DC_NCB, int DC_CHUNK>
__device__ __noinline__ double dense_cost_general(const DenseSmem<R, DC_NCB, DC_CHUNK> &S, int i, int rc,
                                                  double weight_cutoff, double bad_ret, double max_color_diff)
{
	constexpr int WS = 2*R + 1;
	constexpr int WP = DenseSmem<R, DC_NCB, DC_CHUNK>::WP;
	double meanL = 0, meanR = 0, totalWeight = 0.0;
#pragma unroll 1
	for (int row = 0; row < WS; ++row) {
		double gl[WS], gr[WS], wt[WS];
#pragma unroll
		for (int col = 0; col < WS; ++col) { gl[col] = S.lt[row][i + col]; gr[col] = S.rt[row][rc + col]; wt[col] = S.w[i][row*WP + col]; }
#pragma unroll
		for (int col = 0; col < WS; ++col) {
			const bool ok = gl[col] == gl[col] && gr[col] == gr[col] && wt[col] > weight_cutoff;
			const double pl = wt[col]*gl[col], pr = wt[col]*gr[col];
			meanL += ok ? pl : 0.0;
			meanR += ok ? pr : 0.0;
			totalWeight += ok ? wt[col] : 0.0;
		}
	}
	if (totalWeight < 1e-10) return bad_ret;
	meanL /= totalWeight;
	meanR /= totalWeight;
	double sum1 = 0, sum2 = 0, sum3 = 0;
#pragma unroll 1
	for (int row = 0; row < WS; ++row) {
		double gl[WS], gr[WS], wt[WS];
#pragma unroll
		for (int col = 0; col < WS; ++col) { gl[col] = S.lt[row][i + col]; gr[col] = S.rt[row][rc + col]; wt[col] = S.w[i][row*WP + col]; }
#pragma unroll
		for (int col = 0; col < WS; ++col) {
			const bool ok = gl[col] == gl[col] && gr[col] == gr[col] && wt[col] > weight_cutoff;
			const double a = wt[col]*gl[col] - meanL;
			const double b = wt[col]*gr[col] - meanR;
			const double ab = a*b, aa = a*a, bb = b*b;
			sum1 += ok ? ab : 0.0;
			sum2 += ok ? aa : 0.0;
			sum3 += ok ? bb : 0.0;
		}
	}
	const double v = 255*(1.0 - fabs(sum1) / sqrt(sum2 * sum3));
	return (v < max_color_diff) ? v : max_color_diff;
}

#ifdef SRH_EXPERIMENT
__device__ int g_exp_repeat = 1;
__device__ int g_exp_scan_mode = 0;
int g_exp_lds_pad = 0;
void exp_set_scan(int mode) { (void)hipMemcpyToSymbol(HIP_SYMBOL(g_exp_scan_mode), &mode, sizeof(int)); }
void strip_exp_set(int repeat);
void exp_set(int repeat, int lds_pad) {
	if (repeat >= 0) { (void)hipMemcpyToSymbol(HIP_SYMBOL(g_exp_repeat), &repeat, sizeof(int)); strip_exp_set(repeat); }
	if (lds_pad >= 0) g_exp_lds_pad = lds_pad;
}
#endif

template <int R, int DC_NCB, int DC_CHUNK, int MINW, int AR>
__global__ __launch_bounds__(DC_THREADS, MINW)
void twoview_dense_cost_kernel(const ViewDev *__restrict__ views, int ref, int oth, srh_params P,
                               int y0, int nrows, const double *__restrict__ wbuf, size_t wstride,
                               const double *__restrict__ tnum, double *__restrict__ cost, int cstride,
                               Counters *__restrict__ cnt, const double *__restrict__ pconst, const CertBound cb,
                               const PixRange *__restrict__ prange)
{
	constexpr bool FMA = AR != 0, CERT = AR == 3 || AR == 5, ONEPASS = AR == 5;
	constexpr int WS = 2*R + 1;
	constexpr int T = WS*WS;
	typedef DenseSmem<R, DC_NCB, DC_CHUNK> Smem;
	constexpr int WP = Smem::WP;
	constexpr int NR = DC_NCB + 2*R;
	static_assert(NR % 2 == 0 && WP % 2 == 0 && Smem::RW % 2 == 0 && DC_CHUNK % 2 == 0, "16-byte rows");
	extern __shared__ __align__(16) unsigned char smem_raw[];
	Smem &S = *reinterpret_cast<Smem *>(smem_raw);

	const ViewDev &L = views[ref];
	const ViewDev &Rv = views[oth];
	const int W = L.w, H = L.h;
	const int tiles_per_row = (W + DC_TP - 1)/DC_TP;
	const int trow = blockIdx.x / tiles_per_row;
	const int x0 = (blockIdx.x % tiles_per_row)*DC_TP;
	const int y = y0 + trow;
	const int tid = threadIdx.x;
	const int lane = tid & 63;
	const int i = (tid >> 6)*8 + (lane & 7);
	const int g = lane >> 3;
	const int x = x0 + i;

	const double nan = __builtin_nan("");

#ifdef SRH_PROFILE_PHASES
	unsigned long long ph[8] = {0, 0, 0, 0, 0, 0, 0, 0};
	unsigned long long tp = __builtin_readcyclecounter();
	unsigned long long t_fast = 0, n_fast = 0;
	const unsigned long long t_begin = tp;
#define SRH_STAMP(k) do { const unsigned long long tn_ = __builtin_readcyclecounter(); ph[k] += tn_ - tp; tp = tn_; } while (0)
#else
#define SRH_STAMP(k) do { } while (0)
// ... 1255 lines not shown
```

### stereoreconstruction_amd/csrc/srh_internal.hpp

```cpp
#pragma once

#include <hip/hip_runtime.h>
#include <stdint.h>

#include "stereo_recon_hip.h"

namespace srh {

struct ViewDev {
	int32_t w, h;
	const uint32_t *rgba;
	const uint8_t  *mask;
	const double   *gray;
	const double   *gray_tv;
	double         *depth;
	srh_camera      cam;
};

#define SRH_WTILE 32
__host__ __device__ inline size_t wbuf_doubles(int W, int nrows, int T) {
	return (size_t)nrows*((W + SRH_WTILE - 1)/SRH_WTILE)*SRH_WTILE*T;
}
__host__ __device__ inline size_t wbuf_offset(int W, int T, int band_row, int x) {
	const size_t tile = (size_t)band_row*((W + SRH_WTILE - 1)/SRH_WTILE) + x/SRH_WTILE;
	return tile*(size_t)T*SRH_WTILE + (x % SRH_WTILE);
}

__host__ __device__ inline int wimg_wp(int R) { return ((2*R + 1) + 1) & ~1; }
__host__ __device__ inline int wimg_row_stride(int R) { return SRH_WTILE*wimg_wp(R); }
__host__ __device__ inline size_t wimg_doubles(int W, int nrows, int R) {
	return (size_t)nrows*((W + SRH_WTILE - 1)/SRH_WTILE)*SRH_WTILE*(size_t)((2*R + 1)*wimg_wp(R));
}
__host__ __device__ inline size_t wimg_offset(int W, int R, int band_row, int x) {
	const size_t tile = (size_t)band_row*((W + SRH_WTILE - 1)/SRH_WTILE) + x/SRH_WTILE;
	return tile*SRH_WTILE*(size_t)((2*R + 1)*wimg_wp(R)) + (size_t)(x % SRH_WTILE)*wimg_wp(R);
}
#define SRH_PADL 8
#define SRH_PADR 344
#define SRH_PADY 8
__host__ __device__ inline int padded_stride(int w) { return w + SRH_PADL + SRH_PADR; }
__host__ __device__ inline size_t padded_size(int w, int h) { return (size_t)padded_stride(w)*(size_t)(h + 2*SRH_PADY); }
struct PixRange { int32_t lo, hi; };

struct CertBound {
	double e0, m_hi, k1, k2, room;
	double zmax2;
	int ok;
	__host__ __device__ inline double sigma3(double s2) const {
		const double d = room - k2/sqrt(s2);
		if (!(d > 0)) return __builtin_inf();
		const double b = k1/d;
		return b*b*(1.0 + 0x1p-20);
	}
};
__host__ __device__ inline bool cert_sure(double x, double clamp, double m_hi) { return x == clamp || x > m_hi; }
__host__ __device__ inline bool cert_pixel_exact(const CertBound &cb, double sum2, double all_taps_usable) {
	return !(all_taps_usable != 0.0) || !(cb.sigma3(sum2) < __builtin_inf());
}
#ifdef __HIPCC__
__device__ __forceinline__ double onepass_finish(double P, double Q, double U, double SA, double itw, double s2, double TT,
                                                 double sig3, double zmax2, bool &okc)
{
	const double m = P*itw, p2 = P + P;
	const double s3 = __builtin_fma(-m, __builtin_fma(-TT, m, p2), U);
	const double s1 = __builtin_fma(-m, SA, Q);
	const double q3 = __builtin_fma(m, __builtin_fma(TT, m, p2), U);
	const double x = s2*s3;
	const double y0 = __builtin_amdgcn_rsq(x);
	const double e = __builtin_fma(-(x*y0), y0, 1.0);
	const double y1 = __builtin_fma(y0*e, __builtin_fma(0.375, e, 0.5), y0);
	const bool c1 = s3 >= sig3, c2 = s3*zmax2 >= q3, c3 = __builtin_fabs(e) <= 0x1p-20;
	okc = c1 & c2 & c3;
	return __builtin_fma(-255.0, __builtin_fabs(s1)*y1, 255.0);
}
#endif
inline CertBound cert_bound(const srh_params &P, bool mvs = false) {
	const double u = 0x1p-53, G = 256.0;
	const int T = (2*P.window_radius + 1)*(2*P.window_radius + 1);
	auto gamma = [&](int k) { return k*u/(1.0 - k*u); };
	const double eps_b = gamma(T + 4)*G, eps_a = 2*u*G, rt = sqrt((double)T);
	const double scale = mvs ? 1.0 : 255.0;
	CertBound c;
	c.e0 = mvs ? 0x1p-36 : 0x1p-26;
	c.k1 = 2*scale*1.01*3*eps_b*rt;
	c.k2 = 2*scale*1.01*eps_a*rt;
	const double k3 = 2*scale*1.01*2*gamma(T) + (mvs ? 40 : 2600)*u;
	c.room = c.e0 - k3;
	c.m_hi = P.max_color_diff + c.e0;
	{
		const double g = gamma(T + 6), rhs = (c.e0/2 - 2600*u)/(scale*1.01*g);
		const double z = rhs > 0 ? (-3.0 + sqrt(9.0 + 4*2.002*rhs))/(2*2.002) : 0.0;
		c.zmax2 = z*z*(1.0 - 0x1p-20);
	}
	const bool weights_ok = P.weight_kind == SRH_WEIGHT_GEODESIC ? P.geodesic_sigma > 0 : P.adaptive_color_sigma > 0;
	if (mvs) { c.ok = c.room > 0 && weights_ok && fabs(P.peak_threshold) <= 1e5; return c; }
	c.ok = c.room > 0 && c.m_hi > P.max_color_diff && P.max_color_diff <= 1e5 && fabs(P.bad_ret) <= 1e5 &&
	       P.wta_margin >= 0 && P.wta_margin <= 1e5 && fabs(P.second_best_factor) <= 1e5 && weights_ok;
	return c;
}

#ifdef __HIPCC__
__device__ __forceinline__ void wta_store(int32_t *__restrict__ wout, size_t npix, size_t pv, int wx, int wy, int rx, int ry) {
	*reinterpret_cast<int2 *>(wout + 2*pv) = make_int2(wx, wy);
	*reinterpret_cast<int2 *>(wout + 2*(npix + pv)) = make_int2(rx, ry);
}
#endif
void launch_twoview_winner_costs(hipStream_t st, const ViewDev *views, int ref, int oth, int width, const srh_params &P, bool sad,
                                 int y0, int nrows, const double *wbuf, bool wimg, const int32_t *wout,
                                 double *min_cost, double *second_cost);

struct Counters {
	unsigned long long n_pixels;
	unsigned long long n_eval;
	unsigned long long n_eval_device;
	unsigned long long not_row_aligned;
	unsigned long long n_listed, n_slots;
	unsigned long long strip_overflow;
	unsigned long long n_certified, n_flagged;
	unsigned long long cert_overflow;
	unsigned long long scan_tiles_template, scan_tiles_walked;
	unsigned long long mvs_waves_staged, mvs_waves_listed;
	unsigned int strip_ticket, strip_ticket_border;
	unsigned long long dbg_cycles, dbg_blocks, dbg_total_cycles, dbg_waves;
	unsigned long long dbg_phase[8];
	unsigned long long dbg_wave[64];
};

#define SRH_MAX_NEIGH 8
struct NeighList { int32_t n[SRH_MAX_NEIGH]; };
inline NeighList make_neigh_list(const int32_t *neigh, int nneigh) {
	NeighList l;
	for (int i = 0; i < SRH_MAX_NEIGH; ++i) l.n[i] = (i < nneigh) ? neigh[i] : 0;
	return l;
}

struct Extent { int32_t xmin, xmax; };

void launch_prep_view(hipStream_t st, const uint32_t *rgba, const uint8_t *mask, int w, int h,
                      double *gray, double *gray_tv);
void launch_fill(hipStream_t st, double *p, size_t n, double v);
#define SRH_PC 6
void launch_weights(hipStream_t st, const ViewDev *views, int ref, int width, const srh_params &P,
                    int y0, int nrows, double *wbuf, size_t wstride, double *pconst = nullptr, bool wimg = false);
void launch_twoview_generic(hipStream_t st, const ViewDev *views, int ref, int oth, int width, const srh_params &P,
                            int y0, int nrows, const double *wbuf, size_t wstride, Counters *cnt, bool sad = false,
                            int32_t *wout = nullptr);
void launch_twoview_cross_check(hipStream_t st, const ViewDev *views, int self, int other, int w, int h,
                                const srh_params &P);
void launch_mvs_generic(hipStream_t st, const ViewDev *views, int ref, const int32_t *neigh, int nneigh, int width,
                        const srh_params &P, int y0, int nrows, const double *wbuf, size_t wstride,
                        double *peaks, double *best, Counters *cnt);
void launch_mvs_cross_check(hipStream_t st, const ViewDev *views, const int32_t *slots_dev, int nviews,
                            int view_index, int w, int h, const srh_params &P);

void launch_edge_planes(hipStream_t st, const uint32_t *rgba, int w, int h, double *edges);
void launch_geo_exp_probe(hipStream_t st, const double *x, int n, double *kout, double *lout);
size_t geo5_doubles(int w, int h);
void launch_geo5_planes(hipStream_t st, const double *edges, const double *gray_tv, const uint8_t *mask, int w, int h, double *out);
bool launch_geodesic_dma(hipStream_t st, const ViewDev *views, int ref, int width, const double *geo5, const srh_params &P,
                         int y0, int nrows, double *wbuf, double *pconst, int num_cus);
bool launch_geodesic_reg(hipStream_t st, const ViewDev *views, int ref, int width, const double *edges,
                         const srh_params &P, int y0, int nrows, double *wbuf, size_t wstride, double *pconst = nullptr,
                         bool wimg = false);
bool launch_adaptive_reg(hipStream_t st, const ViewDev *views, int ref, int width, const srh_params &P, int y0, int nrows,
                         double *wbuf, size_t wstride, double *pconst = nullptr, bool wimg = false);
void launch_label_plane_table(hipStream_t st, const ViewDev *views, int ref, const srh_params &P, bool mvs, double *tdist);
void launch_pinhole_label_table(hipStream_t st, const ViewDev *views, int ref, const srh_params &P, bool mvs, double *tnum);
bool launch_twoview_dense_cost_f32(hipStream_t st, const ViewDev *views, int ref, int oth, int width, const srh_params &P,
                                   int y0, int nrows, const double *wbuf, size_t wstride,
                                   const double *tnum, double *cost, int cstride, Counters *cnt, const double *pconst, int form = 0);
bool launch_twoview_dense_cost(hipStream_t st, const ViewDev *views, int ref, int oth, int width, const srh_params &P,
                               int y0, int nrows, const double *wbuf, size_t wstride,
                               const double *tnum, double *cost, int cstride, Counters *cnt, const double *pconst, int arith = 0,
                               const PixRange *prange = nullptr);
void launch_twoview_scan(hipStream_t st, const ViewDev *views, int ref, int oth, int width, const srh_params &P,
                         int y0, int nrows, const double *tnum, const double *cost, int cstride,
                         Counters *cnt, const PixRange *prange, uint32_t *cflag = nullptr, int nlist = -1,
                         const double *pexact = nullptr,
                         const void *tpl = nullptr, uint32_t *tilelist = nullptr,
                         int num_cus = 256, int32_t *wout = nullptr);
size_t scan_template_bytes();
void launch_scan_template(hipStream_t st, const ViewDev *views, int ref, int oth, const srh_params &P, int y0, int nrows,
                          const double *tnum, void *tpl);
bool launch_twoview_refill(hipStream_t st, int width, const srh_params &P, int y0, const PixRange *prange, const uint32_t *cflag, int cap,
                           const double *wbuf, bool wimg, const double *ref_tvp, const double *oth_tvp, double *cost, int cstride, Counters *cnt);
void launch_twoview_lazy_fill(hipStream_t st, const ViewDev *views, int ref, int oth, int width, const srh_params &P,
                              int y0, int nrows, const PixRange *prange, const double *wbuf, size_t wstride,
                              const double *ref_tvp, const double *oth_tvp,
                              bool wimg,
                              int lanes, bool padded,
                              double *cost, int cstride, Counters *cnt);

void launch_padded_plane(hipStream_t st, const double *gray_tv, int w, int h, double *out);
void launch_padded_full(hipStream_t st, const double *gray_tv, int w, int h, int R, uint8_t *out);
void launch_pixel_range(hipStream_t st, const ViewDev *views, int ref, int oth, int width, const srh_params &P,
                        int y0, int nrows, const double *tnum, int cstride, PixRange *prange);
int  strip_chunk_columns();
int  strip_block_lanes(int cstride, int form);
bool launch_twoview_strip_cost(hipStream_t st, const ViewDev *views, int ref, int oth, int width, int height,
                               const srh_params &P, int y0, int nrows, const double *wimg, const double *pconst,
                               const PixRange *prange, const double *ref_tvp, const double *oth_tvp,
                               const uint8_t *oth_fullp, double *cost, int cstride, Counters *cnt, int arith, int num_cus,
                               int lanes, bool raw = false);

#ifdef SRH_PROFILE_PHASES
void geodesic_phases_fetch(unsigned long long out[8]);
#endif
#ifdef SRH_EXPERIMENT
void exp_set(int repeat, int lds_pad);
void exp_set_scan(int mode);
void exp_set_walk(int mode);
void exp_set_rows(int mode);
#endif

#define SRH_FUSED_MAXC 256
bool launch_twoview_fused(hipStream_t st, const ViewDev *views, int ref, int oth, int width, const srh_params &P,
                          int y0, int nrows, const double *wbuf, const double *tnum, Counters *cnt, int32_t *wout = nullptr);

void launch_twoview_count(hipStream_t st, const ViewDev *views, int ref, int oth, int width, const srh_params &P,
                          int y0, int nrows, int32_t *count, Counters *cnt, int *max_count, const double *tdist);
void launch_twoview_list(hipStream_t st, const ViewDev *views, int ref, int oth, int width, const srh_params &P,
                         int y0, int nrows, uint32_t *cand, int cmax, int32_t *count, Counters *cnt, int *max_count,
                         const double *tdist);
void launch_full_window(hipStream_t st, const double *gray_tv, int w, int h, int R, uint8_t *full, uint32_t *stat = nullptr);
inline size_t full_stat_offset(size_t npix) { return (npix + 15) & ~(size_t)15; }
bool launch_twoview_list_cost(hipStream_t st, const ViewDev *views, int ref, int oth, int width, const srh_params &P,
                              int y0, int nrows, const double *wbuf, const uint8_t *full_oth,
                              const int32_t *count, const uint32_t *cand, double *cost, int cmax, Counters *cnt);
void launch_twoview_list_scan(hipStream_t st, const ViewDev *views, int ref, int oth, int width, const srh_params &P,
                              int y0, int nrows, const int32_t *count, const uint32_t *cand, const double *cost, int cmax,
                              int32_t *wout = nullptr);
void mvs_staging_shape(int *maxw, size_t *desc_words_per_wave);
void launch_mvs_walk(hipStream_t st, const ViewDev *views, int ref, const int32_t *neigh, int nneigh, int width,
                     const srh_params &P, int y0, int nrows, const double *tnum, uint32_t *cand, int cmax, int32_t *count,
                     Counters *cnt, int *max_count, uint32_t *wdesc, int32_t *nwin, const uint32_t *act, int nact, bool peaks,
                     bool fast_pinhole = false);
void launch_mvs_staged_cost(hipStream_t st, const ViewDev *views, int ref, const int32_t *neigh, int nneigh, int width,
                            const srh_params &P, int y0, int nrows, const double *wbuf, size_t wstride,
                            const uint32_t *cand, int cmax, const int32_t *count, double *best,
                            const uint32_t *wdesc, const int32_t *nwin, Counters *cnt, const uint32_t *act, int nact,
                            double *unit_peaks, bool cert = false);
void launch_mvs_list_cost(hipStream_t st, const ViewDev *views, int ref, const int32_t *neigh, int nneigh, int width,
                          const srh_params &P, int y0, int nrows, const double *wbuf, size_t wstride,
                          const uint32_t *cand, int cmax, const int32_t *count, double *best,
                          double *unit_peaks, bool peaks, const int32_t *nwin, const uint32_t *act, int nact);
void launch_mvs_combine(hipStream_t st, const ViewDev *views, int ref, int nneigh, int width, const srh_params &P,
                        int y0, int nrows, const double *best, const double *unit_peaks, double *peaks);
void launch_filter_gaps(hipStream_t st, const double *D, double *G, int w, int h, int gap, unsigned long long *cnt);
void launch_filter_holes(hipStream_t st, const uint8_t *mask, double *D, int w, int h, bool median, uint32_t *holes,
                         unsigned long long *cnt);
void launch_filter_median(hipStream_t st, const ViewDev *views, int slot, const srh_params &P, const double *G,
                          const uint32_t *holes, int nholes, double *D, unsigned long long *cnt);
void launch_sad_full_window(hipStream_t st, const uint8_t *mask, int w, int h, int R, uint8_t *full);
bool launch_twoview_rows_sad(hipStream_t st, const ViewDev *views, int ref, int oth, int width, const srh_params &P,
                             int y0, int nrows, const double *wbuf, const uint8_t *full_sad_oth,
                             const uint32_t *rowinfo, const int32_t *meta, double *cost, int smax, Counters *cnt);
void launch_twoview_list_sad(hipStream_t st, const ViewDev *views, int ref, int oth, int width, const srh_params &P,
                             int y0, int nrows, const double *wbuf, const int32_t *count, const uint32_t *cand,
                             double *cost, int cmax, Counters *cnt);
void launch_padded_gray(hipStream_t st, const double *gray, const uint8_t *mask, int w, int h, double *out);
void launch_padded_bytes(hipStream_t st, const uint8_t *in, int w, int h, uint8_t *out);
bool launch_twoview_strip_sad(hipStream_t st, int width, int height, const srh_params &P, int y0, int nrows,
                              const double *wimg, const PixRange *prange, const double *ref_tvp, const double *oth_grayp,
                              const uint8_t *oth_fullp, double *cost, int cstride, Counters *cnt, int num_cus);
void launch_pair_costs(hipStream_t st, const ViewDev *views, int ref, int oth, const srh_params &P, bool sad, int n,
                       const int32_t *xy, double *out);
void launch_point_cloud(hipStream_t st, const ViewDev *views, int slot, int w, int h, const srh_params &P,
                        double *xyz, uint8_t *rgb, uint8_t *valid, unsigned long long *counts);
struct MrfLayout {
	double *pz, *D, *Mh, *Mv, *partial, *energy;
	unsigned long long *hand; size_t hand_words;
	unsigned *status, *sync;
	int32_t *ans;
	int nparts, nbands;
	size_t sync_words, total_doubles;
};
size_t mrf_scratch_doubles(int w, int h);
void launch_mrf_layout(double *buf, int w, int h, MrfLayout &lay);
hipError_t launch_mrf_setup(hipStream_t st, double *buf, int w, int h, int K, double beta, double lambda, double phiu,
                            const double *peaks, MrfLayout &lay);
hipError_t launch_mrf_sweep(hipStream_t st, double *buf, int w, int h, int K, double psiu, int sweep);
hipError_t launch_mrf_energy(hipStream_t st, double *buf, int w, int h, int K, double psiu);
hipError_t launch_mrf_depth(hipStream_t st, const ViewDev *views, int slot, double *buf, int w, int h, int K);
struct TvMrfLayout {
	double *Mh, *Mv, *trash, *partial, *energy;
	unsigned long long *hand; size_t hand_words;
	unsigned *status, *sync;
	int32_t *ans;
	int nparts, nbands;
	size_t sync_words, total_doubles;
};
size_t twoview_mrf_scratch_doubles(int w, int h, int L);
void launch_twoview_mrf_layout(double *buf, int w, int h, int L, TvMrfLayout &lay);
hipError_t launch_twoview_mrf_setup(hipStream_t st, double *buf, int w, int h, int L, TvMrfLayout &lay);
hipError_t launch_twoview_mrf_sweep(hipStream_t st, double *buf, const double *costs, int w, int h, int L, double lambda, double smax, int sweep);
hipError_t launch_twoview_mrf_energy(hipStream_t st, double *buf, const double *costs, int w, int h, int L, double lambda, double smax);
hipError_t launch_twoview_mrf_depth(hipStream_t st, const ViewDev *views, int slot, const srh_params &P, double *buf, int w, int h, int L);
hipError_t launch_twoview_label_costs(hipStream_t st, const ViewDev *views, int ref, int oth, int width, const srh_params &P, bool sad,
                                      int y0, int nrows, double fill, double *cost, int32_t *pixel);
void launch_epipolar_preview(hipStream_t st, const ViewDev *views, int ref, int oth, double zmin, double zmax, int nd,
                             int nq, const double *xy, double *out, int32_t *counts);
void launch_refraction_error(hipStream_t st, const ViewDev *views, int v1, int v2, int n, const double *p1, const double *p2, double *err);
void launch_epipolar_curves(hipStream_t st, const ViewDev *views, int ref, int oth, const srh_params &P, int mvs,
                            int nq, const int32_t *xy, int32_t *out, int cap, int32_t *counts);

#define SRH_ROWS_NR 32
void launch_twoview_rows_list(hipStream_t st, const ViewDev *views, int ref, int oth, int width, const srh_params &P,
                              int y0, int nrows, uint32_t *cand, int cmax, int32_t *count, uint32_t *rowinfo,
                              int32_t *meta, int smax, Counters *cnt, int *maxes, const double *tdist);
bool launch_twoview_rows_cost(hipStream_t st, const ViewDev *views, int ref, int oth, int width, const srh_params &P,
                              int y0, int nrows, const double *wbuf, const uint8_t *full_oth,
                              const uint32_t *rowinfo, const int32_t *meta, double *cost, int smax, Counters *cnt, int arith = 0,
                              const double *pconst = nullptr,
                              const double *oth_tvp = nullptr, int num_cus = 256, const uint32_t *full_stat = nullptr);
void launch_twoview_rows_scan(hipStream_t st, const ViewDev *views, int ref, int oth, int width, const srh_params &P,
                              int y0, int nrows, const int32_t *count, const uint32_t *cand, int cmax,
                              const uint32_t *rowinfo, const int32_t *meta, const double *cost, int smax,
                              uint32_t *cflag = nullptr, int nlist = -1, Counters *cnt = nullptr, int32_t *wout = nullptr);
bool launch_twoview_rows_refill(hipStream_t st, int width, int oth_width, const srh_params &P, int y0,
                                const uint32_t *cflag, int cap, const double *wbuf, const double *ref_tvp, const double *oth_tvp,
                                const uint32_t *rowinfo, const int32_t *meta, double *cost, int smax, Counters *cnt);
const char *rccl_unique_id_get(void *out128);
const char *rccl_comm_init(void **comm, int nranks, int rank, const void *id128);
const char *rccl_comm_destroy(void *comm);
bool rccl_available();
const char *rccl_wait_stream(void *comm, hipStream_t st, const char *what);
void rccl_comm_abort(void *comm);
void rccl_set_timeout_ms(int ms);
int  rccl_version();
const char *rccl_gather_f64(void *comm, int nranks, int rank, int root, const double *send, double *recv,
                            size_t count, hipStream_t st);
const char *rccl_allgather_f64(void *comm, const double *send, double *recv, size_t count, hipStream_t st);

}
```

### stereoreconstruction_amd/csrc/srh_kernels.hip

```cpp
#include "srh_internal.hpp"
#include "srh_geom.hpp"
#include "srh_walk.hpp"
#include "srh_window.hpp"

#include <cstdlib>

namespace srh {

static inline int grid_for(size_t n, int block, int cap) {
	size_t b = (n + block - 1)/block;
	if (b > (size_t)cap) b = cap;
	if (b < 1) b = 1;
	return (int)b;
}

__global__ void prep_view_kernel(const uint32_t *__restrict__ rgba, const uint8_t *__restrict__ mask,
                                 int w, int h, double *__restrict__ gray, double *__restrict__ gray_tv)
{
	const size_t n = (size_t)w*h;
	for (size_t i = (size_t)blockIdx.x*blockDim.x + threadIdx.x; i < n; i += (size_t)gridDim.x*blockDim.x) {
		const uint32_t px = rgba[i];
		const double r = (double)(px & 255u), g = (double)((px >> 8) & 255u), b = (double)((px >> 16) & 255u);
		const double gr = (0.11*r + 0.59*g + 0.3*b);
		const int x = (int)(i % (size_t)w), y = (int)(i / (size_t)w);
		gray[i] = gr;
		const bool ok = mask[i] == 1 && x + 1 < w && y + 1 < h;
		gray_tv[i] = ok ? gr : __builtin_nan("");
	}
}

__global__ void fill_kernel(double *__restrict__ p, size_t n, double v) {
	for (size_t i = (size_t)blockIdx.x*blockDim.x + threadIdx.x; i < n; i += (size_t)gridDim.x*blockDim.x)
		p[i] = v;
}

void launch_prep_view(hipStream_t st, const uint32_t *rgba, const uint8_t *mask, int w, int h,
                      double *gray, double *gray_tv)
{
	hipLaunchKernelGGL(prep_view_kernel, dim3(grid_for((size_t)w*h, 256, 2048)), dim3(256), 0, st,
	                   rgba, mask, w, h, gray, gray_tv);
}

void launch_fill(hipStream_t st, double *p, size_t n, double v) {
	hipLaunchKernelGGL(fill_kernel, dim3(grid_for(n, 256, 2048)), dim3(256), 0, st, p, n, v);
}

__global__ void weights_kernel(const ViewDev *__restrict__ views, int ref, srh_params P,
                               int y0, int nrows, double *__restrict__ wbuf, size_t wstride, double *__restrict__ pconst,
                               int wimg)
{
	const ViewDev &V = views[ref];
	const int W = V.w, H = V.h;
	const size_t q = (size_t)blockIdx.x*blockDim.x + threadIdx.x;
	if (q >= (size_t)nrows*W) return;
	const int cx = (int)(q % W), cy = y0 + (int)(q / W);
	if (V.mask[(size_t)cy*W + cx] != 1) return;
	const int R = P.window_radius, WS = 2*R + 1;
	double *wb = wbuf + (wimg ? wimg_offset(W, R, (int)(q / W), cx) : wbuf_offset(W, WS*WS, (int)(q / W), cx));
	const size_t wrs = wimg ? (size_t)wimg_row_stride(R) : (size_t)WS*wstride, wcs = wimg ? 1 : wstride;
#define WTAP(r, c) wb[(size_t)(r)*wrs + (size_t)(c)*wcs]

	support_window(V, P, cx, cy, [&](int r, int c) -> double & { return WTAP(r, c); });
	if (pconst) {
		bool all = true;
		double mL = 0, tw = 0;
		for (int row = -R; row <= R; ++row)
			for (int col = -R; col <= R; ++col) {
				const int px = cx + col, py = cy + row;
				const double gl = (px < 0 || py < 0 || px >= W || py >= H) ? __builtin_nan("") : V.gray_tv[(size_t)py*W + px];
				const double wt = WTAP(row + R, col + R);
				if (!(gl == gl && wt > P.weight_cutoff)) all = false;
				mL += wt*gl;
				tw += wt;
			}
		double s2 = 0, sa = 0;
		if (all && !(tw < 1e-10)) {
			mL /= tw;
			for (int row = -R; row <= R; ++row)
				for (int col = -R; col <= R; ++col) {
					const double wt_ = WTAP(row + R, col + R), gl_ = V.gray_tv[(size_t)(cy + row)*W + (cx + col)];
					const double t = wt_*gl_ - mL;
					s2 += t*t;
					sa += __builtin_fma(wt_, gl_, -mL);
				}
		} else all = false;
		double *pc = pconst + ((size_t)(q / W)*W + cx)*SRH_PC;
		pc[0] = mL; pc[1] = tw; pc[2] = s2; pc[3] = all ? 1.0/tw : 0.0;
		pc[4] = sa; pc[5] = 0.0;
	}
#undef WTAP
}

void launch_weights(hipStream_t st, const ViewDev *views, int ref, int width, const srh_params &P,
                    int y0, int nrows, double *wbuf, size_t wstride, double *pconst, bool wimg)
{
	const size_t n = (size_t)nrows*width;
	hipLaunchKernelGGL(weights_kernel, dim3((unsigned)((n + 255)/256)), dim3(256), 0, st,
	                   views, ref, P, y0, nrows, wbuf, wstride, pconst, wimg ? 1 : 0);
}

template <bool SAD, bool WTA>
struct TwoViewDirectVisitor {
	const ViewDev &L, &Rv;
	const double *wq;
	size_t wstride;
	const srh_params &P;
	int x, y;
	double minCost, secondBest;
	int wx, wy;
	unsigned n;
	int px, py;
	__device__ __forceinline__ void operator()(int cx, int cy) {
		const double cost = SAD ? tv_cost_sad(L, Rv, wq, wstride, P, x, y, cx, cy) : tv_cost(L, Rv, wq, wstride, P, x, y, cx, cy);
		++n;
		if (cost + P.wta_margin < minCost) {
			secondBest = minCost;
			minCost = cost;
			if (WTA) { px = wx; py = wy; }
			wx = cx; wy = cy;
		}
	}
};

template <bool SAD, bool WTA>
__global__ void twoview_generic_kernel(const ViewDev *__restrict__ views, int ref, int oth, srh_params P,
                                       int y0, int nrows, const double *__restrict__ wbuf, size_t wstride,
                                       Counters *__restrict__ cnt, int32_t *__restrict__ wout)
{
	const ViewDev &L = views[ref];
	const ViewDev &Rv = views[oth];
	const int W = L.w;
	const size_t q = (size_t)blockIdx.x*blockDim.x + threadIdx.x;
	unsigned n_eval = 0, n_pix = 0;
	if (q < (size_t)nrows*W) {
		const int x = (int)(q % W), y = y0 + (int)(q / W);
		const size_t pv = (size_t)y*W + x;
		double depth = __builtin_nan("");
		int ox = -1, oy = -1, rx = -1, ry = -1;
		if (L.mask[pv] == 1) {
			n_pix = 1;
			const Ray ray = cam_unproject(L.cam, (x + 0.5) / P.image_scale, (y + 0.5) / P.image_scale);
			const int T = (2*P.window_radius + 1)*(2*P.window_radius + 1);
			TwoViewDirectVisitor<SAD, WTA> vis = { L, Rv, wbuf + wbuf_offset(W, T, (int)(q / W), x), wstride, P, x, y,
			                             __builtin_inf(), __builtin_inf(), -1, -1, 0, -1, -1 };
			walk_curve<false>(ray, L.cam, Rv, P, vis);
			n_eval = vis.n;
			if (WTA) { ox = vis.wx; oy = vis.wy; rx = vis.px; ry = vis.py; }
			if (vis.wx >= 0)
				depth = candidate_depth(L.cam, Rv.cam, P, ray, vis.wx, vis.wy);
			if (vis.minCost > P.second_best_factor*vis.secondBest)
				depth = __builtin_inf();
		}
		L.depth[pv] = depth;
		if (WTA) wta_store(wout, (size_t)W*L.h, pv, ox, oy, rx, ry);
	}
	block_count_add(&cnt->n_eval, n_eval);
	block_count_add(&cnt->n_eval_device, n_eval);
	block_count_add(&cnt->n_pixels, n_pix);
}

void launch_twoview_generic(hipStream_t st, const ViewDev *views, int ref, int oth, int width, const srh_params &P,
                            int y0, int nrows, const double *wbuf, size_t wstride, Counters *cnt, bool sad, int32_t *wout)
{
	const size_t n = (size_t)nrows*width;
	const dim3 grid((unsigned)((n + 127)/128)), block(128);
#define SRH_GEN_LAUNCH(S_, W_) hipLaunchKernelGGL((twoview_generic_kernel<S_, W_>), grid, block, 0, st, views, ref, oth, P, y0, nrows, wbuf, wstride, cnt, wout)
	if (sad) { if (wout) SRH_GEN_LAUNCH(true, true); else SRH_GEN_LAUNCH(true, false); }
	else     { if (wout) SRH_GEN_LAUNCH(false, true); else SRH_GEN_LAUNCH(false, false); }
#undef SRH_GEN_LAUNCH
}

__global__ void twoview_cross_check_kernel(const ViewDev *__restrict__ views, int self, int other, srh_params P)
{
	const ViewDev &A = views[self];
	const ViewDev &B = views[other];
	const int W = A.w, H = A.h;
	const size_t i = (size_t)blockIdx.x*blockDim.x + threadIdx.x;
	if (i >= (size_t)W*H) return;
	const int x = (int)(i % W), y = (int)(i / W);
	double depth = A.depth[i];
	if (!isfinite_d(depth)) return;
	const double s = P.image_scale;
	const double inf = __builtin_inf();
	const Ray ray = cam_unproject(A.cam, (x + 0.5) / s, (y + 0.5) / s);
	Vec3 p1 = load3(A.cam.C);
	if (point_from_depth(ray, load3(A.cam.pdir), depth, p1)) {
		Vec3 q = p1;
		if (cam_project(B.cam, q)) {
			const double x2 = q.x*s, y2 = q.y*s;
			if (x2 >= 0 && y2 >= 0 && x2 < B.w && y2 < B.h) {
				const double odepth = B.depth[(size_t)((int)y2)*B.w + (int)x2];
				if (isfinite_d(odepth)) {
					const Ray ray2 = cam_unproject(B.cam, (x2 + 0.5) / s, (y2 + 0.5) / s);
					Vec3 p2 = load3(B.cam.C);
					if (point_from_depth(ray2, load3(B.cam.pdir), odepth, p2)) {
						const double nrm = norm(p1 - p2);
						if (!isfinite_d(nrm) || nrm > P.inconsistency_thresh) depth = inf;
					} else depth = inf;
				} else depth = inf;
			} else depth = inf;
		} else depth = inf;
	}
	A.depth[i] = depth;
}

void launch_twoview_cross_check(hipStream_t st, const ViewDev *views, int self, int other, int w, int h,
                                const srh_params &P)
{
	const size_t n = (size_t)w*h;
	hipLaunchKernelGGL(twoview_cross_check_kernel, dim3((unsigned)((n + 255)/256)), dim3(256), 0, st,
	                   views, self, other, P);
}

__global__ void point_cloud_kernel(const ViewDev *__restrict__ views, int slot, srh_params P,
                                   double *__restrict__ xyz, uint8_t *__restrict__ rgb, uint8_t *__restrict__ valid,
                                   unsigned long long *__restrict__ counts)
{
	const ViewDev &A = views[slot];
	const int W = A.w, H = A.h;
	const size_t i = (size_t)blockIdx.x*blockDim.x + threadIdx.x;
	unsigned n_pt = 0, n_mask = 0, n_fin = 0;
	if (i < (size_t)W*H) {
		const int x = (int)(i % W), y = (int)(i / W);
		const double nanv = __builtin_nan("");
		Vec3 pt = v3(nanv, nanv, nanv);
		bool ok = false;
		if (A.mask[i] == 1) {
			n_mask = 1;
			const double depth = A.depth[i];
			if (isfinite_d(depth)) {
				n_fin = 1;
				const Ray ray = cam_unproject(A.cam, (x + 0.5) / P.image_scale, (y + 0.5) / P.image_scale);
				Vec3 q = load3(A.cam.C);
				if (point_from_depth(ray, load3(A.cam.pdir), depth, q)) { pt = q; ok = true; n_pt = 1; }
			}
		}
		if (xyz) { xyz[3*i] = pt.x; xyz[3*i + 1] = pt.y; xyz[3*i + 2] = pt.z; }
		if (rgb) { const uint32_t c = A.rgba[i]; rgb[3*i] = (uint8_t)(c & 255u); rgb[3*i + 1] = (uint8_t)((c >> 8) & 255u); rgb[3*i + 2] = (uint8_t)((c >> 16) & 255u); }
		if (valid) valid[i] = ok ? 1 : 0;
	}
	block_count_add(&counts[0], n_pt);
	block_count_add(&counts[1], n_mask);
	block_count_add(&counts[2], n_fin);
}

void launch_point_cloud(hipStream_t st, const ViewDev *views, int slot, int w, int h, const srh_params &P,
                        double *xyz, uint8_t *rgb, uint8_t *valid, unsigned long long *counts)
{
	const size_t n = (size_t)w*h;
	hipLaunchKernelGGL(point_cloud_kernel, dim3((unsigned)((n + 255)/256)), dim3(256), 0, st, views, slot, P, xyz, rgb, valid, counts);
}
// ... 1234 lines not shown
```

### stereoreconstruction_amd/csrc/srh_strip.hip

```cpp
#include "srh_internal.hpp"
#include "srh_geom.hpp"
#include "srh_walk.hpp"

#include <type_traits>

namespace srh {

#ifdef SRH_EXPERIMENT
__device__ int g_strip_exp_repeat = 1;
void strip_exp_set(int repeat) { (void)hipMemcpyToSymbol(HIP_SYMBOL(g_strip_exp_repeat), &repeat, sizeof(int)); }
#endif

#define ST_TP 32
#define ST_NCB 8
#define ST_CHUNK 320
#define ST_BROWS 1

typedef __attribute__((address_space(3))) void st_lds_void;
typedef __attribute__((address_space(1))) const void st_gbl_void;
typedef __attribute__((address_space(3))) volatile int st_lds_vint;

__global__ void padded_plane_kernel(const double *__restrict__ gray_tv, int W, int H, double *__restrict__ out)
{
	const int SP = padded_stride(W), HP = H + 2*SRH_PADY;
	const size_t n = (size_t)SP*HP;
	const double nan = __builtin_nan("");
	for (size_t k = (size_t)blockIdx.x*blockDim.x + threadIdx.x; k < n; k += (size_t)gridDim.x*blockDim.x) {
		const int x = (int)(k % (size_t)SP) - SRH_PADL, y = (int)(k / (size_t)SP) - SRH_PADY;
		out[k] = (x >= 0 && y >= 0 && x < W && y < H) ? gray_tv[(size_t)y*W + x] : nan;
	}
}

void launch_padded_plane(hipStream_t st, const double *gray_tv, int w, int h, double *out) {
	size_t n = padded_size(w, h);
	size_t b = (n + 255)/256; if (b > 4096) b = 4096;
	hipLaunchKernelGGL(padded_plane_kernel, dim3((unsigned)b), dim3(256), 0, st, gray_tv, w, h, out);
}

__global__ void padded_full_kernel(const double *__restrict__ gray_tv, int W, int H, int R, uint8_t *__restrict__ out)
{
	const int SP = padded_stride(W), HP = H + 2*SRH_PADY;
	const size_t n = (size_t)SP*HP;
	for (size_t k = (size_t)blockIdx.x*blockDim.x + threadIdx.x; k < n; k += (size_t)gridDim.x*blockDim.x) {
		const int x = (int)(k % (size_t)SP) - SRH_PADL, y = (int)(k / (size_t)SP) - SRH_PADY;
		bool ok = x - R >= 0 && y - R >= 0 && x + R < W && y + R < H;
		for (int row = -R; ok && row <= R; ++row)
			for (int col = -R; col <= R; ++col) {
				const double v = gray_tv[(size_t)(y + row)*W + (x + col)];
				ok = ok && (v == v);
			}
		out[k] = ok ? 1 : 0;
	}
}

void launch_padded_full(hipStream_t st, const double *gray_tv, int w, int h, int R, uint8_t *out) {
	size_t n = padded_size(w, h);
	size_t b = (n + 255)/256; if (b > 4096) b = 4096;
	hipLaunchKernelGGL(padded_full_kernel, dim3((unsigned)b), dim3(256), 0, st, gray_tv, w, h, R, out);
}

__global__ void pixel_range_kernel(const ViewDev *__restrict__ views, int ref, int oth, srh_params P, int y0, int nrows,
                                   const double *__restrict__ tnum, int cstride, PixRange *__restrict__ prange)
{
	const ViewDev &L = views[ref];
	const int W = L.w;
	const size_t q = (size_t)blockIdx.x*blockDim.x + threadIdx.x;
	if (q >= (size_t)nrows*W) return;
	const int x = (int)(q % W), y = y0 + (int)(q / W);
	int lo = 0, hi = -1;
	if (L.mask[(size_t)y*W + x] == 1) {
		const Ray ray = cam_unproject(L.cam, (x + 0.5) / P.image_scale, (y + 0.5) / P.image_scale);
		pinhole_column_range(ray, L.cam, views[oth], P, tnum, cstride, lo, hi);
	}
	PixRange r; r.lo = lo; r.hi = hi;
	prange[q] = r;
}

void launch_pixel_range(hipStream_t st, const ViewDev *views, int ref, int oth, int width, const srh_params &P,
                        int y0, int nrows, const double *tnum, int cstride, PixRange *prange)
{
	const size_t n = (size_t)nrows*width;
	hipLaunchKernelGGL(pixel_range_kernel, dim3((unsigned)((n + 255)/256)), dim3(256), 0, st,
	                   views, ref, oth, P, y0, nrows, tnum, cstride, prange);
}

int strip_chunk_columns() { return ST_CHUNK; }

struct StripArgs {
	int W, H, y0, nrows;
	const double *wimg;
	const double *pconst;
	const PixRange *prange;
	const double *ref_tvp, *oth_tvp;
	const uint8_t *oth_fullp;
	double *cost; int cstride;
	Counters *cnt;
	int n1, n2;
	int nitems;
	double weight_cutoff, bad_ret, max_color_diff;
	CertBound cb;
	int redo;
};

static void strip_items(StripArgs &a) {
	a.n1 = ((a.nrows*3/4)/16)*16;
	a.n2 = a.n1 + (((a.nrows - a.n1)*2/3)/8)*8;
	const int nseg = a.n1/16 + (a.n2 - a.n1)/8 + (a.nrows - a.n2 + 3)/4;
	a.nitems = nseg*((a.W + ST_TP - 1)/ST_TP);
}

template <int R, int NBUF>
struct StripSmem {
	static constexpr int WS = 2*R + 1;
	static constexpr int T = WS*WS;
	static constexpr int WP = (WS + 1) & ~1;
	static constexpr int WPIX = WS*WP;
	static constexpr int RW = ST_CHUNK + 2*R + ST_NCB + 2;
	static constexpr int LW = (ST_TP + 2*R + 1) & ~1;
	static constexpr int NS = WS + 1;
	static constexpr int FW = (RW + 4 + 15) & ~15;
	static constexpr int NBMAX = ST_CHUNK/ST_NCB + 1;
	static constexpr int GL_CAP = 3072;
	static constexpr int GL_SINGLES = GL_CAP - ST_TP*NBMAX;
	alignas(16) double w[NBUF][WS][ST_TP][WP];
	alignas(16) double rt[NS][RW];
	alignas(16) double rto[NBUF == 2 ? NS : 1][RW];
	alignas(16) double lt[NS][LW];
	alignas(16) double pc[2][ST_TP][SRH_PC];
	alignas(16) PixRange pr[2][ST_TP];
	alignas(16) unsigned char full[2][FW];
	unsigned short glist[GL_CAP];
	int glist_n, gsingle_n;
	int item;
	unsigned long long badcols[ST_CHUNK/64 + 2];
	int simd[8];
	int prog[NBUF == 2 ? 8 : 1][64];
	static_assert(ST_CHUNK <= 512 && ST_TP <= 64, "work-list entry = pixel*512 + column in 16 bits");
	static_assert(RW % 2 == 0 && LW % 2 == 0 && WP % 2 == 0, "16-byte rows");
	static_assert(RW - R + 4 <= SRH_PADR + 1, "padded planes cover every staged piece");
};

__device__ __forceinline__ void st_dma16(const void *src, void *dst, int nbytes, int lane) {
	for (int off = 0; off < nbytes; off += 1024) {
		if (off + lane*16 < nbytes)
			__builtin_amdgcn_global_load_lds((st_gbl_void *)((const char *)src + off + lane*16),
			                                 (st_lds_void *)((char *)dst + off), 16, 0, 0);
	}
}
__device__ __forceinline__ void st_dma4(const void *src, void *dst, int nbytes, int lane) {
	for (int off = 0; off < nbytes; off += 256) {
		if (off + lane*4 < nbytes)
			__builtin_amdgcn_global_load_lds((st_gbl_void *)((const char *)src + off + lane*4),
			                                 (st_lds_void *)((char *)dst + off), 4, 0, 0);
	}
}

template <int R, int NBUF>
__device__ __noinline__ double strip_cost_general(const StripSmem<R, NBUF> &S, int wb, int s0, int i, int rc,
                                                  double weight_cutoff, double bad_ret, double max_color_diff)
{
	typedef StripSmem<R, NBUF> Smem;
	constexpr int WS = Smem::WS, NS = Smem::NS;
	double meanL = 0, meanR = 0, totalWeight = 0.0;
#pragma unroll 1
	for (int row = 0; row < WS; ++row) {
		const int sl = s0 + row >= NS ? s0 + row - NS : s0 + row;
		double gl[WS], gr[WS], wt[WS];
#pragma unroll
		for (int col = 0; col < WS; ++col) { gl[col] = S.lt[sl][i + col]; gr[col] = S.rt[sl][rc + col]; wt[col] = S.w[wb][row][i][col]; }
#pragma unroll
		for (int col = 0; col < WS; ++col) {
			const bool ok = gl[col] == gl[col] && gr[col] == gr[col] && wt[col] > weight_cutoff;
			const double pl = wt[col]*gl[col], pr = wt[col]*gr[col];
			meanL += ok ? pl : 0.0;
			meanR += ok ? pr : 0.0;
			totalWeight += ok ? wt[col] : 0.0;
		}
	}
	if (totalWeight < 1e-10) return bad_ret;
	meanL /= totalWeight;
	meanR /= totalWeight;
	double sum1 = 0, sum2 = 0, sum3 = 0;
#pragma unroll 1
	for (int row = 0; row < WS; ++row) {
		const int sl = s0 + row >= NS ? s0 + row - NS : s0 + row;
		double gl[WS], gr[WS], wt[WS];
#pragma unroll
		for (int col = 0; col < WS; ++col) { gl[col] = S.lt[sl][i + col]; gr[col] = S.rt[sl][rc + col]; wt[col] = S.w[wb][row][i][col]; }
#pragma unroll
		for (int col = 0; col < WS; ++col) {
			const bool ok = gl[col] == gl[col] && gr[col] == gr[col] && wt[col] > weight_cutoff;
			const double a = wt[col]*gl[col] - meanL;
			const double b = wt[col]*gr[col] - meanR;
			const double ab = a*b, aa = a*a, bb = b*b;
			sum1 += ok ? ab : 0.0;
			sum2 += ok ? aa : 0.0;
			sum3 += ok ? bb : 0.0;
		}
	}
	const double v = 255*(1.0 - fabs(sum1) / sqrt(sum2 * sum3));
	return (v < max_color_diff) ? v : max_color_diff;
}

template <int R, int NBUF>
__device__ __noinline__ void strip_select_block(const StripSmem<R, NBUF> &S, int wb, int s0, int pi, int rc, unsigned store,
                                                double *__restrict__ dst, double weight_cutoff, double bad_ret, double max_color_diff,
                                                int ra, int rb)
{
	typedef StripSmem<R, NBUF> Smem;
	constexpr int WS = Smem::WS, NS = Smem::NS, NCB = ST_NCB, NR = NCB + 2*R;
	double mLs[NCB], mRs[NCB], tws[NCB];
#pragma unroll
	for (int j = 0; j < NCB; ++j) { mLs[j] = 0.0; mRs[j] = 0.0; tws[j] = 0.0; }
#pragma unroll 1
	for (int row = ra; row < rb; ++row) {
		const int sl = s0 + row >= NS ? s0 + row - NS : s0 + row;
		double rr[NR], rv[NR];
		const double2 *rp = reinterpret_cast<const double2 *>((NBUF == 2 && (rc & 1)) ? &S.rto[sl][rc - 1] : &S.rt[sl][rc]);
#pragma unroll
		for (int m = 0; m < NR/2; ++m) { const double2 v = rp[m]; rr[2*m] = v.x; rr[2*m + 1] = v.y; }
#pragma unroll
		for (int m = 0; m < NR; ++m) { const bool okr = rr[m] == rr[m]; rv[m] = okr ? 1.0 : 0.0; rr[m] = okr ? rr[m] : 0.0; }
#pragma unroll
		for (int col = 0; col < WS; ++col) {
			const double gl = S.lt[sl][pi + col], wt = S.w[wb][row][pi][col];
			const bool okl = gl == gl && wt > weight_cutoff;
			const double w0 = okl ? wt : 0.0, pl0 = okl ? wt*gl : 0.0;
#pragma unroll
			for (int j = 0; j < NCB; ++j) {
				mLs[j] += pl0*rv[col + j];
				mRs[j] += w0*rr[col + j];
				tws[j] += w0*rv[col + j];
			}
		}
	}
#pragma unroll
	for (int j = 0; j < NCB; ++j) { mLs[j] /= tws[j]; mRs[j] /= tws[j]; }
	double s1[NCB], s2v[NCB], s3[NCB];
#pragma unroll
	for (int j = 0; j < NCB; ++j) { s1[j] = 0.0; s2v[j] = 0.0; s3[j] = 0.0; }
#pragma unroll 1
	for (int row = ra; row < rb; ++row) {
		const int sl = s0 + row >= NS ? s0 + row - NS : s0 + row;
		double rr[NR], rv[NR];
		const double2 *rp = reinterpret_cast<const double2 *>((NBUF == 2 && (rc & 1)) ? &S.rto[sl][rc - 1] : &S.rt[sl][rc]);
#pragma unroll
		for (int m = 0; m < NR/2; ++m) { const double2 v = rp[m]; rr[2*m] = v.x; rr[2*m + 1] = v.y; }
#pragma unroll
		for (int m = 0; m < NR; ++m) { const bool okr = rr[m] == rr[m]; rv[m] = okr ? 1.0 : 0.0; rr[m] = okr ? rr[m] : 0.0; }
#pragma unroll
		for (int col = 0; col < WS; ++col) {
			const double gl = S.lt[sl][pi + col], wt = S.w[wb][row][pi][col];
			const bool okl = gl == gl && wt > weight_cutoff;
			const double pl = wt*(gl == gl ? gl : 0.0), kl = okl ? 1.0 : 0.0;
#pragma unroll
			for (int j = 0; j < NCB; ++j) {
				const double k = kl*rv[col + j];
				const double a = (pl - mLs[j])*k, bq = (wt*rr[col + j] - mRs[j])*k;
				s1[j] += a*bq;
				s2v[j] += a*a;
				s3[j] += bq*bq;
			}
		}
	}
#pragma unroll
	for (int j = 0; j < NCB; ++j) {
		if ((store >> j) & 1u) {
			double result = bad_ret;
			if (!(tws[j] < 1e-10)) {
				const double v = 255*(1.0 - fabs(s1[j]) / sqrt(s2v[j] * s3[j]));
				result = (v < max_color_diff) ? v : max_color_diff;
			}
			dst[(ptrdiff_t)j*ST_TP] = result;
		}
	}
}

template <int R, int NWV, int NBUF, int AR, bool BORDER>
__global__ __launch_bounds__(NWV*64, 2)
void twoview_strip_cost_kernel(const StripArgs A)
{
	constexpr bool FMA = AR != 0, CERT = AR == 3 || AR == 5, ONEPASS = AR == 5;
	typedef StripSmem<R, NBUF> Smem;
	constexpr int WS = Smem::WS, WP = Smem::WP, WPIX = Smem::WPIX, RW = Smem::RW, LW = Smem::LW, NS = Smem::NS;
	constexpr int NCB = ST_NCB, CHUNK = ST_CHUNK;
	constexpr int NR = NCB + 2*R;
	constexpr int G = 2*NWV;
	constexpr int NT = NWV*64;
	constexpr bool PAD = NBUF == 1;
	static_assert(NR % 2 == 0, "16-byte rows");
	static_assert((NWV == 4 && NBUF == 1) || (NWV == 8 && NBUF == 2), "two forms");
	extern __shared__ __align__(16) unsigned char smem_raw[];
	Smem &S = *reinterpret_cast<Smem *>(smem_raw);
	const Smem &CS = S;

	const int tid = threadIdx.x;
	const int lane = tid & 63;
	const int wv = __builtin_amdgcn_readfirstlane(tid >> 6);
	const int pg = wv & 3;
	const int i = pg*8 + (lane & 7);
	const int g = (lane >> 3) + 8*(wv >> 2);
	const int W = A.W;
	const int tiles_per_row = (W + ST_TP - 1)/ST_TP;
	const int SP = padded_stride(W);
	unsigned n_dev = 0;
	int partner = wv;
	if (NWV == 8) {
		const int simd = (int)__builtin_amdgcn_s_getreg((1 << 11) | (4 << 6) | 4);
		if (lane == 0) S.simd[wv] = simd;
		S.prog[wv][lane] = 0;
		__syncthreads();
		for (int j = 0; j < NWV; ++j) if (j != wv && CS.simd[j] == simd) { partner = j; break; }
		partner = __builtin_amdgcn_readfirstlane(partner);
	}
	int prog = 0;
	auto prog_step = [&](int units, int &seen) {
		if (NWV == 8) {
			prog += units;
			*(st_lds_vint *)&S.prog[wv][lane] = prog;
			seen = *(st_lds_vint *)&S.prog[partner][lane];
		}
	};
	auto prog_yield = [&](int seen) {
		if (NWV == 8) {
			const int ps = __builtin_amdgcn_readfirstlane(seen), pm = __builtin_amdgcn_readfirstlane(prog);
			asm volatile("s_nop 0\n\ts_cmp_gt_i32 %0, %1\n\ts_cbranch_scc1 1f\n\ts_setprio 1\n\ts_branch 2f\n1:\n\ts_setprio 0\n2:"
			             :: "s"(pm), "s"(ps) : "scc");
		}
	};
#ifdef SRH_PROFILE_PHASES
	unsigned long long ph[8] = {0, 0, 0, 0, 0, 0, 0, 0};
	unsigned long long tp = __builtin_readcyclecounter();
	const unsigned long long t_begin = tp;
	unsigned long long n_tiles = 0, n_gen = 0;
#define ST_STAMP(k) do { const unsigned long long tn_ = __builtin_readcyclecounter(); ph[k] += tn_ - tp; tp = tn_; } while (0)
#else
#define ST_STAMP(k) do { } while (0)
#endif

	for (;;) {
		if (tid == 0) S.item = (int)atomicAdd(BORDER ? &A.cnt->strip_ticket_border : &A.cnt->strip_ticket, 1u);
		__syncthreads();
		const int item = __builtin_amdgcn_readfirstlane(S.item);
		ST_STAMP(0);
		if (item >= A.nitems) break;
		int seg = item / tiles_per_row, tx = item - seg*tiles_per_row;
		if (BORDER) {
			const int nseg = (A.n1 + ST_BROWS - 1)/ST_BROWS + (A.nrows - A.n2 + ST_BROWS - 1)/ST_BROWS;
			const int k = item / nseg;
			seg = item - k*nseg;
			tx = k == 0 ? 0 : k == 1 ? tiles_per_row - 1 : k - 1;
		}
		int ya, nh;
		if (BORDER) {
			const int st = (A.n1 + ST_BROWS - 1)/ST_BROWS;
			if (seg < st) { ya = seg*ST_BROWS; nh = A.n1 - ya; }
			else { ya = A.n2 + (seg - st)*ST_BROWS; nh = A.nrows - ya; }
			if (nh > ST_BROWS) nh = ST_BROWS;
		} else {
			const int s16 = A.n1 >> 4, s8 = (A.n2 - A.n1) >> 3;
			if (seg < s16) { ya = seg*16; nh = 16; }
			else if (seg < s16 + s8) { ya = A.n1 + (seg - s16)*8; nh = 8; }
			else { ya = A.n2 + (seg - s16 - s8)*4; nh = 4; }
			if (ya + nh > A.nrows) nh = A.nrows - ya;
		}
		const int x0 = tx*ST_TP;
		const int x = x0 + i;
		int cs = 0, rowbase = 0;

		auto issue_tile_inputs = [&](int r, int buf, int wb, bool consts, bool windows) {
			const size_t px0 = (size_t)r*W + x0;
			if (consts && wv == 0) st_dma16(A.pconst + px0*SRH_PC, &S.pc[buf][0][0], ST_TP*SRH_PC*8, lane);
			if (consts && wv == 1) st_dma4(A.prange + px0, &S.pr[buf][0], ST_TP*8, lane);
			if (windows) {
				const double *wt = A.wimg + ((size_t)r*tiles_per_row + tx)*(size_t)(ST_TP*WPIX);
				if (NBUF == 1) {
					for (int a = 0; a < WS; ++a)
						st_dma16(wt + (size_t)a*(ST_TP*WP) + pg*8*WP, &S.w[wb][a][pg*8][0], 8*WP*8, lane);
				} else {
					constexpr int NBYTES = ST_TP*WPIX*8;
					for (int off = wv*1024; off < NBYTES; off += NWV*1024)
						if (off + lane*16 < NBYTES)
							__builtin_amdgcn_global_load_lds((st_gbl_void *)((const char *)wt + off + lane*16),
							                                 (st_lds_void *)((char *)&S.w[wb][0][0][0] + off), 16, 0, 0);
				}
			}
		};
		auto issue_row = [&](int yy, int sl) {
			const double *src = A.oth_tvp + (size_t)(yy + SRH_PADY)*SP + (cs - R + SRH_PADL);
			if (wv < 3) { if (wv*1024 + lane*16 < RW*8) __builtin_amdgcn_global_load_lds((st_gbl_void *)((const char *)src + wv*1024 + lane*16),
			                                                                              (st_lds_void *)((char *)&S.rt[sl][0] + wv*1024), 16, 0, 0); }
			else if (wv == 3) st_dma16(A.ref_tvp + (size_t)(yy + SRH_PADY)*SP + (x0 - R + SRH_PADL), &S.lt[sl][0], LW*8, lane);
			else if (NBUF == 2 && wv < 7) {
				const int pc = wv - 4;
				if (pc*1024 + lane*16 < RW*8) __builtin_amdgcn_global_load_lds((st_gbl_void *)((const char *)(src + 1) + pc*1024 + lane*16),
				                                                                (st_lds_void *)((char *)&S.rto[sl][0] + pc*1024), 16, 0, 0);
			}
		};
		static_assert(RW*8 <= 3*1024, "three pieces per row of the other view");
		auto issue_full = [&](int fy, int fb) {
			const size_t a0 = (size_t)(fy + SRH_PADY)*SP + (size_t)(cs + SRH_PADL);
			if (!BORDER && wv == NWV - 1) st_dma4(A.oth_fullp + (a0 & ~(size_t)3), &S.full[fb][0], (RW + 4 + 3) & ~3, lane);
		};

		bool first = true;
		for (int r = ya; r < ya + nh; ++r) {
			const int y = A.y0 + r;
			const int cur = (r - ya) & 1, nxt = cur ^ 1;
			const int wcur = NBUF == 2 ? cur : 0, wnxt = NBUF == 2 ? nxt : 0;
			const bool has_next = r + 1 < ya + nh;
			if (first) issue_tile_inputs(r, cur, wcur, true, true);
			asm volatile("s_waitcnt vmcnt(0)" ::: "memory");
			ST_STAMP(1);
			__builtin_amdgcn_s_barrier();
			ST_STAMP(2);

			int cmin, cmax, cmin_raw;
			{
				const int pi = lane & 31;
				const PixRange q = CS.pr[cur][pi];
				int lo = q.lo, hi = q.hi;
				if (x0 + pi >= W) { lo = 0; hi = -1; }
				if (hi >= lo) hi = dense_cover_hi(lo, hi, NCB, G, PAD);
				int mn = hi >= lo ? lo : 2147483647, mx = hi >= lo ? hi : -2147483647;
#define ST_ROR(v, n) __builtin_amdgcn_update_dpp(0, (v), 0x120 + (n), 0xf, 0xf, false)
#pragma unroll
				for (int d = 8; d >= 1; d >>= 1) {
					const int on = d == 8 ? ST_ROR(mn, 8) : d == 4 ? ST_ROR(mn, 4) : d == 2 ? ST_ROR(mn, 2) : ST_ROR(mn, 1);
					const int ox = d == 8 ? ST_ROR(mx, 8) : d == 4 ? ST_ROR(mx, 4) : d == 2 ? ST_ROR(mx, 2) : ST_ROR(mx, 1);
					mn = on < mn ? on : mn; mx = ox > mx ? ox : mx;
				}
#undef ST_ROR
				{
					const int m0 = __builtin_amdgcn_readlane(mn, 0), m1 = __builtin_amdgcn_readlane(mn, 16);
					const int x0_ = __builtin_amdgcn_readlane(mx, 0), x1_ = __builtin_amdgcn_readlane(mx, 16);
					cmin_raw = m0 < m1 ? m0 : m1;
					cmax = x0_ > x1_ ? x0_ : x1_;
				}
				cmin = cmin_raw & ~1;
			}
			const bool any = cmin_raw <= cmax;
			if (first || (any && (cmin < cs || cmax > cs + CHUNK - 1))) {
				if (!first) __builtin_amdgcn_s_barrier();
				cs = any ? cmin : 0;
				rowbase = y - R;
				for (int rr = 0; rr < WS; ++rr) issue_row(y - R + rr, rr);
				issue_full(y, cur);
				asm volatile("s_waitcnt vmcnt(0)" ::: "memory");
				__builtin_amdgcn_s_barrier();
			}
			if (any && cmax > cs + CHUNK - 1) {
				if (tid == 0) atomicAdd(&A.cnt->strip_overflow, 1ull);
				cmax = cs + CHUNK - 1;
			}
			first = false;
			const int s0 = (y - R - rowbase) % NS;
			if (has_next) {
				issue_row(y + R + 1, (y + R + 1 - rowbase) % NS);
				issue_full(y + 1, nxt);
				issue_tile_inputs(r + 1, nxt, wnxt, true, NBUF == 2);
			}
			const int foff = BORDER ? 0 : (int)(((size_t)(y + SRH_PADY)*SP + (size_t)(cs + SRH_PADL)) & 3);
			const unsigned char *rfull = &CS.full[cur][foff];
			const int bra = BORDER ? (y < R ? R - y : 0) : 0;
			const int brb = BORDER ? (y + R > A.H - 2 ? WS - (y + R - (A.H - 2)) : WS) : WS;
			if (BORDER) {
				unsigned char *cok = &S.full[nxt][0];
				for (int k = tid; k < RW; k += NT) {
					bool ok = true;
					for (int row = bra; row < brb; ++row) {
						const int sl = s0 + row >= NS ? s0 + row - NS : s0 + row;
						const double v = CS.rt[sl][k];
						ok = ok && v == v;
					}
					cok[k] = ok ? 1 : 0;
				}
				if (g == 0) {
					bool all = x < W;
					double mL = 0, tw = 0;
					for (int row = bra; row < brb; ++row) {
						const int sl = s0 + row >= NS ? s0 + row - NS : s0 + row;
						for (int col = 0; col < WS; ++col) {
							const double gl = CS.lt[sl][i + col], wt = CS.w[wcur][row][i][col];
							all = all && gl == gl && wt > A.weight_cutoff;
							mL += wt*gl;
							tw += wt;
						}
					}
					double s2 = 0;
					if (all && !(tw < 1e-10)) {
						mL /= tw;
						for (int row = bra; row < brb; ++row) {
							const int sl = s0 + row >= NS ? s0 + row - NS : s0 + row;
							for (int col = 0; col < WS; ++col) {
								const double t = CS.w[wcur][row][i][col]*CS.lt[sl][i + col] - mL;
								s2 += t*t;
							}
						}
					} else all = false;
					S.pc[cur][i][0] = mL; S.pc[cur][i][1] = tw; S.pc[cur][i][2] = s2; S.pc[cur][i][3] = all ? 1.0/tw : 0.0;
				}
				__syncthreads();
				for (int k = tid; k < CHUNK + NCB; k += NT) {
					bool ok = true;
					for (int d = 0; d < WS; ++d) ok = ok && cok[k + d] != 0;
					S.full[cur][k] = ok ? 1 : 0;
				}
				__syncthreads();
			}

			bool need_general = false;
			{
				const int pi = lane & 31;
				const PixRange q = CS.pr[cur][pi];
				const bool live = x0 + pi < W && q.hi >= q.lo;
				bool bad = live && !(CS.pc[cur][pi][3] != 0.0);
#pragma unroll
				for (int it = 0; it < (CHUNK + 63)/64 + 1; ++it) {
					const int k = it*64 + lane, c = cs + k;
					const bool colbad = k < CHUNK + NCB && rfull[k] == 0;
					if (colbad && c >= cmin_raw && c <= cmax) bad = true;
					const unsigned long long m = __ballot(colbad);
					if (wv == 0 && lane == 0) S.badcols[it] = m;
				}
				need_general = __any(bad) != 0;
			}

			if (NWV == 8) { prog = 0; *(st_lds_vint *)&S.prog[wv][lane] = 0; __builtin_amdgcn_s_setprio(1); }
			int e_min, e_max;
			{
				const PixRange q = CS.pr[cur][i];
				e_min = q.lo; e_max = q.hi;
				if (x >= W) { e_min = 0; e_max = -1; }
				if (e_max >= e_min) e_max = dense_cover_hi(e_min, e_max, NCB, G, PAD);
			}
			const bool lall = CS.pc[cur][i][3] != 0.0;
			const double sig3 = CERT ? A.cb.sigma3(CS.pc[cur][i][2]) : 0.0;
			const bool pix_exact = CERT && A.redo && !(sig3 < __builtin_inf());
			const size_t tile = (size_t)r*tiles_per_row + tx;
			ST_STAMP(3);
			if (e_max >= e_min) {
				const int lo = e_min > cs ? e_min : cs;
				const int hi = e_max < cs + CHUNK - 1 ? e_max : cs + CHUNK - 1;
				const int lo_e = PAD ? (lo & ~1) : lo;
				const int nblocks = hi >= lo ? (hi - lo_e + NCB)/NCB : 0;
				double *crow = A.cost + tile*(size_t)A.cstride*ST_TP + i;
#ifdef SRH_EXPERIMENT
				const int exp_rep = g_strip_exp_repeat;
				for (int rep = 0; rep < exp_rep; ++rep)
#endif
				for (int b = g; b < (lall ? nblocks : 0); b += G) {
					const int c0 = lo_e + b*NCB;
					const int rc = c0 - cs;
					const double *rbase = (!PAD && (rc & 1)) ? &CS.rto[0][0] - 1 : &CS.rt[0][0];
					unsigned vm = 0;
#pragma unroll
					for (int j = 0; j < NCB; ++j) {
						const int c = c0 + j;
						vm |= (c >= lo && c <= hi && rfull[rc + j] != 0) ? 1u << j : 0u;
					}
					const bool fast = vm != 0;
					n_dev += __builtin_popcount(vm);
					bool bad_blk = false;
					auto two_sweeps = [&](auto fma_c, auto cert_c) {
						constexpr bool FMAc = decltype(fma_c)::value, CERTc = decltype(cert_c)::value;
						const double mL = CS.pc[cur][i][0], tw = CS.pc[cur][i][1], s2 = CS.pc[cur][i][2];
						const int ra = BORDER ? bra : 0, rb = BORDER ? brb : WS;
						const int sa = BORDER ? (s0 + ra >= NS ? s0 + ra - NS : s0 + ra) : s0;
						double r_[NR], wv_[WS], acc[NCB];
						{
							const double2 *rp = reinterpret_cast<const double2 *>(rbase + sa*RW + rc);
							const double2 *wp = reinterpret_cast<const double2 *>(&CS.w[wcur][ra][i][0]);
#pragma unroll
							for (int m = 0; m < NR/2; ++m) { const double2 v = rp[m]; r_[2*m] = v.x; r_[2*m + 1] = v.y; }
#pragma unroll
							for (int m = 0; m < (WS - 1)/2; ++m) { const double2 v = wp[m]; wv_[2*m] = v.x; wv_[2*m + 1] = v.y; }
							wv_[WS - 1] = CS.w[wcur][ra][i][WS - 1];
						}
#pragma unroll
						for (int j = 0; j < NCB; ++j) acc[j] = 0.0;
						__builtin_amdgcn_s_waitcnt(0xC07F);
#pragma unroll 1
						for (int row = ra; row < rb; ++row) {
							int seen = 0;
							prog_step(1, seen);
							const int nrow = row + 1 < rb ? row + 1 : ra;
							const int nsl = s0 + nrow >= NS ? s0 + nrow - NS : s0 + nrow;
							const double2 *rp = reinterpret_cast<const double2 *>(rbase + nsl*RW + rc);
							const double2 *wp = reinterpret_cast<const double2 *>(&CS.w[wcur][nrow][i][0]);
#pragma unroll
							for (int col = 0; col < WS; ++col) {
								if (FMAc) {
#pragma unroll
									for (int j = 0; j < NCB; ++j) acc[j] = __builtin_fma(wv_[col], r_[col + j], acc[j]);
								} else {
									double pr[NCB];
#pragma unroll
									for (int j = 0; j < NCB; ++j) pr[j] = wv_[col]*r_[col + j];
									__builtin_amdgcn_sched_barrier(0);
#pragma unroll
									for (int j = 0; j < NCB; ++j) acc[j] += pr[j];
								}
								__builtin_amdgcn_sched_barrier(0);
								if (col & 1) {
									const double2 v = rp[col >> 1]; r_[col - 1] = v.x; r_[col] = v.y;
									const double2 u = wp[col >> 1]; wv_[col - 1] = u.x; wv_[col] = u.y;
									__builtin_amdgcn_sched_barrier(0);
								}
							}
#pragma unroll
							for (int m = (WS - 1)/2; m < NR/2; ++m) { const double2 v = rp[m]; r_[2*m] = v.x; r_[2*m + 1] = v.y; }
							wv_[WS - 1] = CS.w[wcur][nrow][i][WS - 1];
							prog_yield(seen);
						}
						double mR[NCB], s1[NCB], s3[NCB], av[WS];
#pragma unroll
						for (int col = 0; col < WS; ++col) av[col] = CS.lt[sa][i + col];
#pragma unroll
						for (int j = 0; j < NCB; ++j) { mR[j] = acc[j]/tw; s1[j] = 0.0; s3[j] = 0.0; }
						__builtin_amdgcn_s_waitcnt(0xC07F);
#pragma unroll 1
						for (int row = ra; row < rb; ++row) {
							int seen = 0;
							prog_step(3, seen);
							const int nrow = row + 1 < rb ? row + 1 : ra;
							const int nsl = s0 + nrow >= NS ? s0 + nrow - NS : s0 + nrow;
							const double2 *rp = reinterpret_cast<const double2 *>(rbase + nsl*RW + rc);
							const double2 *wp = reinterpret_cast<const double2 *>(&CS.w[wcur][nrow][i][0]);
							const double *lp = &CS.lt[nsl][i];
#pragma unroll
							for (int col = 0; col < WS; ++col) {
								const double wt = wv_[col];
								if (FMAc) {
									const double a = __builtin_fma(wt, av[col], -mL);
									double bb[NCB];
#pragma unroll
									for (int j = 0; j < NCB; ++j) bb[j] = __builtin_fma(wt, r_[col + j], -mR[j]);
									__builtin_amdgcn_sched_barrier(0);
#pragma unroll
									for (int j = 0; j < NCB; ++j) { s1[j] = __builtin_fma(a, bb[j], s1[j]); s3[j] = __builtin_fma(bb[j], bb[j], s3[j]); }
								} else {
									double bb[NCB], u1[NCB], u3[NCB];
									const double pa = wt*av[col];
#pragma unroll
									for (int j = 0; j < NCB; ++j) bb[j] = wt*r_[col + j];
									__builtin_amdgcn_sched_barrier(0);
									const double a = pa - mL;
#pragma unroll
									for (int j = 0; j < NCB; ++j) bb[j] = bb[j] - mR[j];
									__builtin_amdgcn_sched_barrier(0);
#pragma unroll
									for (int j = 0; j < NCB; ++j) { u1[j] = a*bb[j]; u3[j] = bb[j]*bb[j]; }
									__builtin_amdgcn_sched_barrier(0);
#pragma unroll
									for (int j = 0; j < NCB; ++j) { s1[j] += u1[j]; s3[j] += u3[j]; }
								}
								__builtin_amdgcn_sched_barrier(0);
								av[col] = lp[col];
								if (col & 1) {
									const double2 v = rp[col >> 1]; r_[col - 1] = v.x; r_[col] = v.y;
									const double2 u = wp[col >> 1]; wv_[col - 1] = u.x; wv_[col] = u.y;
								}
								__builtin_amdgcn_sched_barrier(0);
							}
#pragma unroll
							for (int m = (WS - 1)/2; m < NR/2; ++m) { const double2 v = rp[m]; r_[2*m] = v.x; r_[2*m + 1] = v.y; }
							wv_[WS - 1] = CS.w[wcur][nrow][i][WS - 1];
							prog_yield(seen);
						}
#pragma unroll
						for (int j = 0; j < NCB; ++j) {
							const int c = c0 + j;
							if (c >= lo && c <= hi && rfull[rc + j] != 0) {
								const double v = 255*(1.0 - fabs(s1[j]) / sqrt(s2 * s3[j]));
								if (CERTc) {
									if (!(s3[j] >= sig3) && A.redo) bad_blk = true;
									crow[(size_t)(c - e_min)*ST_TP] = !(s3[j] >= sig3) ? __builtin_nan("") : (v > A.cb.m_hi ? A.max_color_diff : v);
								} else crow[(size_t)(c - e_min)*ST_TP] = (v < A.max_color_diff) ? v : A.max_color_diff;
							}
							__builtin_amdgcn_sched_barrier(0);
						}
					};
					if (BORDER) {
						if (fast) two_sweeps(std::false_type(), std::false_type());
					} else if (fast && ONEPASS && !pix_exact) {
						const double mL = CS.pc[cur][i][0], itw = CS.pc[cur][i][3], s2 = CS.pc[cur][i][2];
						double r_[NR], q_[NR], w_[WS], l_[WS], P_[NCB], Q_[NCB], U_[NCB];
						{
							const double2 *rp = reinterpret_cast<const double2 *>(rbase + s0*RW + rc);
							const double2 *wp = reinterpret_cast<const double2 *>(&CS.w[wcur][0][i][0]);
#pragma unroll
							for (int m = 0; m < NR/2; ++m) { const double2 v = rp[m]; r_[2*m] = v.x; r_[2*m + 1] = v.y; }
#pragma unroll
							for (int m = 0; m < (WS - 1)/2; ++m) { const double2 v = wp[m]; w_[2*m] = v.x; w_[2*m + 1] = v.y; }
							w_[WS - 1] = CS.w[wcur][0][i][WS - 1];
#pragma unroll
							for (int col = 0; col < WS; ++col) l_[col] = CS.lt[s0][i + col];
						}
#pragma unroll
						for (int j = 0; j < NCB; ++j) { P_[j] = 0.0; Q_[j] = 0.0; U_[j] = 0.0; }
						__builtin_amdgcn_s_waitcnt(0xC07F);
#pragma unroll 1
						for (int row = 0; row < WS; ++row) {
							int seen = 0;
							prog_step(4, seen);
							const int nrow = row + 1 < WS ? row + 1 : 0;
							const int nsl = s0 + nrow >= NS ? s0 + nrow - NS : s0 + nrow;
							const double2 *rp = reinterpret_cast<const double2 *>(rbase + nsl*RW + rc);
							const double2 *wp = reinterpret_cast<const double2 *>(&CS.w[wcur][nrow][i][0]);
							const double *lp = &CS.lt[nsl][i];
#pragma unroll
							for (int k = 0; k < NCB - 1; ++k) q_[k] = r_[k]*r_[k];
#pragma unroll
							for (int col = 0; col < WS; ++col) {
								q_[col + NCB - 1] = r_[col + NCB - 1]*r_[col + NCB - 1];
								const double a = __builtin_fma(w_[col], l_[col], -mL);
								const double c = a*w_[col], d = w_[col]*w_[col];
								__builtin_amdgcn_sched_barrier(0);
#pragma unroll
								for (int j = 0; j < NCB; ++j) P_[j] = __builtin_fma(w_[col], r_[col + j], P_[j]);
#pragma unroll
								for (int j = 0; j < NCB; ++j) Q_[j] = __builtin_fma(c, r_[col + j], Q_[j]);
#pragma unroll
								for (int j = 0; j < NCB; ++j) U_[j] = __builtin_fma(d, q_[col + j], U_[j]);
								__builtin_amdgcn_sched_barrier(0);
								l_[col] = lp[col];
								if (col & 1) {
									const double2 v = rp[col >> 1]; r_[col - 1] = v.x; r_[col] = v.y;
									const double2 u = wp[col >> 1]; w_[col - 1] = u.x; w_[col] = u.y;
								}
								__builtin_amdgcn_sched_barrier(0);
							}
#pragma unroll
							for (int m = (WS - 1)/2; m < NR/2; ++m) { const double2 v = rp[m]; r_[2*m] = v.x; r_[2*m + 1] = v.y; }
							w_[WS - 1] = CS.w[wcur][nrow][i][WS - 1];
							prog_yield(seen);
						}
						constexpr double TT = (double)(WS*WS);
						const double zmax2 = A.cb.zmax2, mhi = A.cb.m_hi, mcd = A.max_color_diff, SA = CS.pc[cur][i][4];
						const bool redo = A.redo != 0;
#pragma unroll
						for (int j = 0; j < NCB; ++j) {
							bool okc;
							const double v = onepass_finish(P_[j], Q_[j], U_[j], SA, itw, s2, TT, sig3, zmax2, okc);
							const bool st = (vm >> j) & 1u;
							bad_blk |= st & !okc & redo;
							if (st) crow[(size_t)(c0 + j - e_min)*ST_TP] = !okc ? __builtin_nan("") : (v > mhi ? mcd : v);
						}
					} else if (fast && !ONEPASS && !pix_exact) two_sweeps(std::integral_constant<bool, FMA>(), std::integral_constant<bool, CERT>());
					if (!BORDER && fast && CERT && (pix_exact || bad_blk)) two_sweeps(std::false_type(), std::false_type());
				}
			}
			if (NWV == 8) __builtin_amdgcn_s_setprio(2);
			ST_STAMP(4);
			if (need_general) {
				if (tid == 0) { S.glist_n = 0; S.gsingle_n = 0; }
				__syncthreads();
				for (int p = tid; p < ST_TP*Smem::NBMAX; p += NT) {
					const int pi = p / Smem::NBMAX, b = p % Smem::NBMAX;
					const PixRange q = CS.pr[cur][pi];
					int qlo = q.lo, qhi = q.hi;
					if (x0 + pi >= W) { qlo = 0; qhi = -1; }
					if (qhi >= qlo) qhi = dense_cover_hi(qlo, qhi, NCB, G, PAD);
					if (qhi > cs + CHUNK - 1) qhi = cs + CHUNK - 1;
					if (qhi < qlo) continue;
					const int c0 = (PAD ? (qlo & ~1) : qlo) + b*NCB;
					if (c0 > qhi) continue;
					const bool pall = CS.pc[cur][pi][3] != 0.0;
					unsigned need = 0xffu;
					if (qlo > c0) need &= 0xffu << (qlo - c0);
					if (c0 + NCB - 1 > qhi) need &= 0xffu >> (c0 + NCB - 1 - qhi);
					if (pall) {
						const int rc = c0 - cs, wd = rc >> 6, sh = rc & 63;
						unsigned long long bits = CS.badcols[wd] >> sh;
						if (sh) bits |= CS.badcols[wd + 1] << (64 - sh);
						need &= (unsigned)bits;
					}
					if (!need) continue;
					bool as_block = __builtin_popcount(need) == NCB;
					if (!as_block) {
						const int at = atomicAdd(&S.gsingle_n, __builtin_popcount(need));
						if (at + __builtin_popcount(need) <= Smem::GL_SINGLES) {
							int k = 0;
#pragma unroll
							for (int j = 0; j < NCB; ++j)
								if ((need >> j) & 1u) { S.glist[Smem::GL_CAP - 1 - (at + k)] = (unsigned short)(pi*512 + (c0 + j - cs)); ++k; }
						} else {
							for (int k = at; k < at + __builtin_popcount(need) && k < Smem::GL_SINGLES; ++k) S.glist[Smem::GL_CAP - 1 - k] = 0xffffu;
							as_block = true;
						}
					}
					if (as_block) S.glist[atomicAdd(&S.glist_n, 1)] = (unsigned short)(pi*64 + b);
				}
				__syncthreads();
				ST_STAMP(5);
#ifdef SRH_PROFILE_PHASES
				++n_gen;
#endif
				const int nblk = S.glist_n;
				const int nsingle = S.gsingle_n < Smem::GL_SINGLES ? S.gsingle_n : Smem::GL_SINGLES;
				for (int q = tid; q < nblk; q += NT) {
					const int pi = S.glist[q] >> 6, b = S.glist[q] & 63;
					const PixRange pq = CS.pr[cur][pi];
					int qhi = dense_cover_hi(pq.lo, pq.hi, NCB, G, PAD);
					if (qhi > cs + CHUNK - 1) qhi = cs + CHUNK - 1;
					const int c0 = (PAD ? (pq.lo & ~1) : pq.lo) + b*NCB;
					const bool pall = CS.pc[cur][pi][3] != 0.0;
					unsigned store = 0;
#pragma unroll
					for (int j = 0; j < NCB; ++j) {
						const int c = c0 + j;
						if (c >= pq.lo && c <= qhi && !(pall && rfull[c - cs])) { store |= 1u << j; ++n_dev; }
					}
					strip_select_block<R, NBUF>(CS, wcur, s0, pi, c0 - cs, store,
					                            A.cost + (tile*(size_t)A.cstride)*ST_TP + (ptrdiff_t)(c0 - pq.lo)*ST_TP + pi,
					                            A.weight_cutoff, A.bad_ret, A.max_color_diff,
					                            y < R ? R - y : 0, y + R > A.H - 2 ? WS - (y + R - (A.H - 2)) : WS);
				}
				ST_STAMP(6);
				for (int q = tid; q < nsingle; q += NT) {
					const unsigned short e = S.glist[Smem::GL_CAP - 1 - q];
					if (e == 0xffffu) continue;
					const int pi = e >> 9, k = e & 511;
					++n_dev;
					A.cost[(tile*(size_t)A.cstride + (size_t)(cs + k - CS.pr[cur][pi].lo))*ST_TP + pi] =
						strip_cost_general<R, NBUF>(CS, wcur, s0, pi, k, A.weight_cutoff, A.bad_ret, A.max_color_diff);
				}
				ST_STAMP(7);
				__syncthreads();
			}
			if (NBUF == 1 && has_next) issue_tile_inputs(r + 1, nxt, 0, false, true);
			ST_STAMP(2);
#ifdef SRH_PROFILE_PHASES
			++n_tiles;
#endif
		}
	}
	block_count_add(&A.cnt->n_eval_device, n_dev);
#ifdef SRH_PROFILE_PHASES
	if (lane == 0) {
		for (int k = 0; k < 8; ++k) atomicAdd(&A.cnt->dbg_phase[k], ph[k]);
		atomicAdd(&A.cnt->dbg_blocks, n_tiles);
		atomicAdd(&A.cnt->dbg_cycles, n_gen);
		for (int k = 0; k < 8; ++k) atomicAdd(&A.cnt->dbg_wave[8*k + (wv & 7)], ph[k]);
		atomicAdd(&A.cnt->dbg_total_cycles, (unsigned long long)(__builtin_readcyclecounter() - t_begin));
		atomicAdd(&A.cnt->dbg_waves, 1ull);
	}
#endif
#undef ST_STAMP
}

template <int R, int NWV, int NBUF, int AR, bool BORDER>
static void launch_strip_variant(hipStream_t st, const StripArgs &a, int num_cus)
{
	typedef StripSmem<R, NBUF> Smem;
	size_t lds = sizeof(Smem);
	(void)hipFuncSetAttribute((const void *)twoview_strip_cost_kernel<R, NWV, NBUF, AR, BORDER>,
	                          hipFuncAttributeMaxDynamicSharedMemorySize, (int)lds);
	int grid = num_cus*(NBUF == 2 ? 1 : 2);
	if (grid > a.nitems) grid = a.nitems;
	if (grid < 1) grid = 1;
	hipLaunchKernelGGL((twoview_strip_cost_kernel<R, NWV, NBUF, AR, BORDER>), dim3((unsigned)grid), dim3(NWV*64), lds, st, a);
}

template <int R, int NWV, int NBUF>
static void launch_strip_arith(hipStream_t st, const StripArgs &a, int num_cus, int arith)
{
	const int tiles_per_row = (a.W + ST_TP - 1)/ST_TP;
	const int t = std::min(std::max(R - a.y0, 0), a.nrows);
	const int b = std::min(std::max(a.H - 1 - R - a.y0, t), a.nrows);
	if (b > t) {
		StripArgs m = a;
		const size_t tiles = (size_t)t*tiles_per_row;
		m.y0 = a.y0 + t; m.nrows = b - t;
		m.wimg = a.wimg + tiles*(ST_TP*StripSmem<R, NBUF>::WPIX);
		m.pconst = a.pconst + (size_t)t*a.W*SRH_PC;
		m.prange = a.prange + (size_t)t*a.W;
		m.cost = a.cost + tiles*(size_t)a.cstride*ST_TP;
		strip_items(m);
		if (arith == 5) launch_strip_variant<R, NWV, NBUF, 5, false>(st, m, num_cus);
		else if (arith == 3) launch_strip_variant<R, NWV, NBUF, 3, false>(st, m, num_cus);
		else if (arith == 1) launch_strip_variant<R, NWV, NBUF, 1, false>(st, m, num_cus);
		else launch_strip_variant<R, NWV, NBUF, 0, false>(st, m, num_cus);
	}
	if (t > 0 || b < a.nrows) {
		StripArgs e = a;
		e.n1 = t; e.n2 = b;
		e.nitems = ((t + ST_BROWS - 1)/ST_BROWS + (a.nrows - b + ST_BROWS - 1)/ST_BROWS)*tiles_per_row;
		launch_strip_variant<R, NWV, NBUF, 0, true>(st, e, num_cus);
	}
}

int strip_block_lanes(int cstride, int form) {
	if (form == 4) return 8;
	if (form == 8) return 16;
	return cstride > 16*ST_NCB ? 16 : 8;
}

bool launch_twoview_strip_cost(hipStream_t st, const ViewDev *views, int ref, int oth, int width, int height,
                               const srh_params &P, int y0, int nrows, const double *wimg, const double *pconst,
                               const PixRange *prange, const double *ref_tvp, const double *oth_tvp,
                               const uint8_t *oth_fullp, double *cost, int cstride, Counters *cnt, int arith, int num_cus,
                               int lanes, bool raw)
{
	(void)views; (void)ref; (void)oth;
	StripArgs a;
	a.W = width; a.H = height; a.y0 = y0; a.nrows = nrows;
	a.wimg = wimg; a.pconst = pconst; a.prange = prange;
	a.ref_tvp = ref_tvp; a.oth_tvp = oth_tvp; a.oth_fullp = oth_fullp;
	a.cost = cost; a.cstride = cstride; a.cnt = cnt;
	a.weight_cutoff = P.weight_cutoff; a.bad_ret = P.bad_ret; a.max_color_diff = P.max_color_diff;
	a.cb = cert_bound(P);
	a.redo = raw ? 0 : 1;
	const bool wide = lanes == 16;
	switch (P.window_radius) {
	case 5:
		if (wide) launch_strip_arith<5, 8, 2>(st, a, num_cus, arith); else launch_strip_arith<5, 4, 1>(st, a, num_cus, arith);
		return true;
	case 2:
		if (wide) launch_strip_arith<2, 8, 2>(st, a, num_cus, arith); else launch_strip_arith<2, 4, 1>(st, a, num_cus, arith);
		return true;
	default: return false;
	}
}

}
```

Baseline: 45910 Mhyp/s.

## Precompute per-tile disparity ranges and sigma3 bounds outside the strip cost kernel

Adds a tile_record_kernel that, per strip tile, precomputes the min/max cost column range and a flag for whether the general (partial-coverage) path is needed. The strip cost kernel DMA-loads this 16-byte record and reads it with readfirstlane instead of doing per-tile reductions over pixel ranges and visibility masks. The weight kernels now also store the certification sigma3 bound in pconst slot 5 so the cost kernel no longer evaluates it per pixel. The general-path block listing is restructured so each thread scans one (pixel, 8-block run) bitmask. The cost is one extra small kernel launch and buffer per band.

```diff
diff --git a/stereoreconstruction_amd/csrc/srh_api.hip b/stereoreconstruction_amd/csrc/srh_api.hip
--- a/stereoreconstruction_amd/csrc/srh_api.hip
+++ b/stereoreconstruction_amd/csrc/srh_api.hip
@@ -143,6 +143,7 @@
 	DevBuf<double> tnum;
 	DevBuf<double> pconst;
 	DevBuf<PixRange> prange;
+	DevBuf<TileRec> trec;
 	DevBuf<uint32_t> cflag;
 	DevBuf<uint8_t> stpl;
 	DevBuf<uint32_t> tileflag;
@@ -153,7 +154,7 @@
 	DevBuf<uint32_t> mvs_wdesc;
 	DevBuf<int32_t> mvs_nwin;
 	template <class F> void each(F f) {
-		f(wbuf); f(cost); f(tnum); f(pconst); f(prange); f(cflag); f(stpl); f(tileflag);
+		f(wbuf); f(cost); f(tnum); f(pconst); f(prange); f(trec); f(cflag); f(stpl); f(tileflag);
 		f(lcount); f(lcand); f(lrowinfo); f(lmeta); f(mvs_wdesc); f(mvs_nwin);
 	}
 	size_t bytes() { size_t b = 0; each([&](auto &x) { b += x.bytes(); }); return b; }
@@ -1009,6 +1010,7 @@
 
 static void run_weights(srh_context *c, int ref, int W, const srh_params &p, int by, int nr, size_t wstride,
                         double *pconst = nullptr, bool wimg = false) {
+	const CertBound cb = cert_bound(p);
 	if (p.weight_kind == SRH_WEIGHT_GEODESIC && !c->force_generic && wimg && c->geodma && p.window_radius == 5 && !c->views[ref].geo5_denied) {
 		ViewHost &v = c->views[ref];
 		bool ok = true;
@@ -1023,19 +1025,19 @@
 		}
 		if (ok) {
 			Scope s(c, "geodesic_dma_kernel");
-			if (launch_geodesic_dma(c->stream, c->d_views, ref, W, v.geo5, p, by, nr, c->band.wbuf, pconst, c->num_cus)) return;
+			if (launch_geodesic_dma(c->stream, c->d_views, ref, W, v.geo5, p, cb, by, nr, c->band.wbuf, pconst, c->num_cus)) return;
 		}
 	}
 	if (p.weight_kind == SRH_WEIGHT_GEODESIC && !c->force_generic) {
 		Scope s(c, "geodesic_reg_kernel");
-		if (launch_geodesic_reg(c->stream, c->d_views, ref, W, c->views[ref].edges, p, by, nr, c->band.wbuf, wstride, pconst, wimg)) return;
+		if (launch_geodesic_reg(c->stream, c->d_views, ref, W, c->views[ref].edges, p, cb, by, nr, c->band.wbuf, wstride, pconst, wimg)) return;
 	}
 	if (p.weight_kind == SRH_WEIGHT_ADAPTIVE && !c->force_generic) {
 		Scope s(c, "adaptive_reg_kernel");
-		if (launch_adaptive_reg(c->stream, c->d_views, ref, W, p, by, nr, c->band.wbuf, wstride, pconst, wimg)) return;
+		if (launch_adaptive_reg(c->stream, c->d_views, ref, W, p, cb, by, nr, c->band.wbuf, wstride, pconst, wimg)) return;
 	}
 	Scope s(c, "weights_kernel");
-	launch_weights(c->stream, c->d_views, ref, W, p, by, nr, c->band.wbuf, wstride, pconst, wimg);
+	launch_weights(c->stream, c->d_views, ref, W, p, cb, by, nr, c->band.wbuf, wstride, pconst, wimg);
 }
 
 static bool rig_is_row_aligned(const srh_camera &a, const srh_camera &b, double *fx_bx) {
@@ -1443,6 +1445,7 @@
 		if (dense && (rc = c->band.pconst.ensure((rows*(size_t)W + SRH_WTILE)*SRH_PC))) return rc;
 		int lanes = 8;
 		if (dense && (rc = c->band.prange.ensure(rows*(size_t)W + SRH_WTILE))) return rc;
+		if (strip && !sad && (rc = c->band.trec.ensure(rows*(size_t)((W + SRH_WTILE - 1)/SRH_WTILE)))) return rc;
 		if (tscan && (rc = c->band.tileflag.ensure(rows*(size_t)((W + 63)/64) + 1))) return rc;
 		const bool cert = dense && cert_ok;
 		const int cost_arith = c->arith == 3 ? (cert ? (c->cert_form == 1 ? 5 : 3) : 0) : c->arith;
@@ -1480,6 +1483,10 @@
 				Scope s(c, "pixel_range_kernel");
 				launch_pixel_range(c->stream, c->d_views, ref, oth, W, *p, by, nr, c->band.tnum, cstride, c->band.prange);
 			}
+			if (strip && !sad) {
+				Scope s(c, "tile_record_kernel");
+				launch_tile_records(c->stream, W, by, nr, c->band.prange, c->band.pconst, c->views[oth].fullp, lanes, c->band.trec);
+			}
 			if (dense) {
 				auto cost_pass = [&](int arith) -> int {
 					if (sad) {
@@ -1491,7 +1498,7 @@
 					} else if (strip) {
 						HIP_TRY(hipMemsetAsync(&c->d_cnt->strip_ticket, 0, 2*sizeof(unsigned int), c->stream));
 						{ Scope s(c, "twoview_strip_cost_kernel");
-						  launch_twoview_strip_cost(c->stream, c->d_views, ref, oth, W, H, *p, by, nr, c->band.wbuf, c->band.pconst, c->band.prange,
+						  launch_twoview_strip_cost(c->stream, c->d_views, ref, oth, W, H, *p, by, nr, c->band.wbuf, c->band.pconst, c->band.prange, c->band.trec,
 						                            c->views[ref].tvp, c->views[oth].tvp, c->views[oth].fullp, c->band.cost, cstride,
 						                            c->d_cnt, arith, c->num_cus, lanes, c->diag && c->diag->raw); }
 						Scope s(c, "twoview_lazy_fill_kernel");
diff --git a/stereoreconstruction_amd/csrc/srh_dense.hip b/stereoreconstruction_amd/csrc/srh_dense.hip
--- a/stereoreconstruction_amd/csrc/srh_dense.hip
+++ b/stereoreconstruction_amd/csrc/srh_dense.hip
@@ -243,7 +243,7 @@
 __global__ __launch_bounds__(GW_TW*GW_ROWS)
 void geodesic_reg_kernel(const ViewDev *__restrict__ views, int ref, const double *__restrict__ edges,
                          srh_params P, int y0, int nrows, double *__restrict__ wbuf, size_t wstride,
-                         double *__restrict__ pconst)
+                         double *__restrict__ pconst, const CertBound cb)
 {
 	constexpr int WS = 2*R + 1;
 	constexpr int TWD = GW_TW + 2*R;
@@ -393,7 +393,7 @@
 		} else all = false;
 		double *pc = pconst + ((size_t)trow*W + cx)*SRH_PC;
 		pc[0] = mL; pc[1] = tw; pc[2] = s2; pc[3] = all ? 1.0/tw : 0.0;
-		pc[4] = sa; pc[5] = 0.0;
+		pc[4] = sa; pc[5] = pconst_sigma3(cb, s2);
 	}
 #ifdef SRH_PROFILE_PHASES
 	GEO_STAMP(3)
@@ -446,7 +446,7 @@
 template <int R>
 __global__ __launch_bounds__(GW_TW*GD_ROWS)
 void geodesic_dma_kernel(const ViewDev *__restrict__ views, int ref, const double *__restrict__ geo5,
-                         srh_params P, int y0, int nrows, double *__restrict__ wbuf, double *__restrict__ pconst)
+                         srh_params P, int y0, int nrows, double *__restrict__ wbuf, double *__restrict__ pconst, const CertBound cb)
 {
 	static_assert(R == GD_PADL, "the padded planes are laid out for this radius");
 	constexpr int WS = 2*R + 1, TWD = GW_TW + 2*R, TH = WS + GD_ROWS - 1, PL = TH*TWD;
@@ -569,18 +569,18 @@
 			} else all = false;
 			double *pc = pconst + ((size_t)trow*W + cx)*SRH_PC;
 			pc[0] = mL; pc[1] = tw; pc[2] = s2; pc[3] = all ? 1.0/tw : 0.0;
-			pc[4] = sa; pc[5] = 0.0;
+			pc[4] = sa; pc[5] = pconst_sigma3(cb, s2);
 		}
 	}
 }
 
 bool launch_geodesic_dma(hipStream_t st, const ViewDev *views, int ref, int width, const double *geo5, const srh_params &P,
-                         int y0, int nrows, double *wbuf, double *pconst, int num_cus)
+                         const CertBound &cb, int y0, int nrows, double *wbuf, double *pconst, int num_cus)
 {
 	if (P.window_radius != GD_PADL) return false;
 	const int tiles = (width + GW_TW - 1)/GW_TW, total = tiles*((nrows + GD_ROWS - 1)/GD_ROWS);
 	const int grid = total < num_cus ? total : num_cus;
-	hipLaunchKernelGGL((geodesic_dma_kernel<GD_PADL>), dim3((unsigned)grid), dim3(GW_TW*GD_ROWS), 0, st, views, ref, geo5, P, y0, nrows, wbuf, pconst);
+	hipLaunchKernelGGL((geodesic_dma_kernel<GD_PADL>), dim3((unsigned)grid), dim3(GW_TW*GD_ROWS), 0, st, views, ref, geo5, P, y0, nrows, wbuf, pconst, cb);
 	return true;
 }
 
@@ -588,7 +588,7 @@
 template <int R>
 __global__ __launch_bounds__(AW_TW)
 void adaptive_reg_kernel(const ViewDev *__restrict__ views, int ref, srh_params P, int y0, int nrows,
-                         double *__restrict__ wbuf, size_t wstride, double *__restrict__ pconst, int wimg)
+                         double *__restrict__ wbuf, size_t wstride, double *__restrict__ pconst, int wimg, const CertBound cb)
 {
 	constexpr int WS = 2*R + 1, TWD = AW_TW + 2*R;
 	const ViewDev &V = views[ref];
@@ -659,35 +659,35 @@
 		} else all = false;
 		double *pc = pconst + ((size_t)trow*W + cx)*SRH_PC;
 		pc[0] = mL; pc[1] = tw; pc[2] = s2; pc[3] = all ? 1.0/tw : 0.0;
-		pc[4] = sa; pc[5] = 0.0;
-	}
-}
-
-bool launch_adaptive_reg(hipStream_t st, const ViewDev *views, int ref, int width, const srh_params &P, int y0, int nrows,
-                         double *wbuf, size_t wstride, double *pconst, bool wimg)
+		pc[4] = sa; pc[5] = pconst_sigma3(cb, s2);
+	}
+}
+
+bool launch_adaptive_reg(hipStream_t st, const ViewDev *views, int ref, int width, const srh_params &P, const CertBound &cb,
+                         int y0, int nrows, double *wbuf, size_t wstride, double *pconst, bool wimg)
 {
 	if (wstride != SRH_WTILE) return false;
 	const dim3 grid((unsigned)(((width + AW_TW - 1)/AW_TW)*nrows)), block(AW_TW);
-	if (P.window_radius == 5) hipLaunchKernelGGL(adaptive_reg_kernel<5>, grid, block, 0, st, views, ref, P, y0, nrows, wbuf, wstride, pconst, wimg ? 1 : 0);
-	else if (P.window_radius == 2) hipLaunchKernelGGL(adaptive_reg_kernel<2>, grid, block, 0, st, views, ref, P, y0, nrows, wbuf, wstride, pconst, wimg ? 1 : 0);
+	if (P.window_radius == 5) hipLaunchKernelGGL(adaptive_reg_kernel<5>, grid, block, 0, st, views, ref, P, y0, nrows, wbuf, wstride, pconst, wimg ? 1 : 0, cb);
+	else if (P.window_radius == 2) hipLaunchKernelGGL(adaptive_reg_kernel<2>, grid, block, 0, st, views, ref, P, y0, nrows, wbuf, wstride, pconst, wimg ? 1 : 0, cb);
 	else return false;
 	return true;
 }
 
 bool launch_geodesic_reg(hipStream_t st, const ViewDev *views, int ref, int width, const double *edges,
-                         const srh_params &P, int y0, int nrows, double *wbuf, size_t wstride, double *pconst, bool wimg)
+                         const srh_params &P, const CertBound &cb, int y0, int nrows, double *wbuf, size_t wstride, double *pconst, bool wimg)
 {
 	const int tiles = (width + GW_TW - 1)/GW_TW;
 	const dim3 grid((unsigned)(tiles*((nrows + GW_ROWS - 1)/GW_ROWS))), block(GW_TW*GW_ROWS);
 	const int wi = wimg ? 1 : 0;
 	switch (P.window_radius) {
 	case 5:
-		if (wi) hipLaunchKernelGGL((geodesic_reg_kernel<5, true>), grid, block, 0, st, views, ref, edges, P, y0, nrows, wbuf, wstride, pconst);
-		else    hipLaunchKernelGGL((geodesic_reg_kernel<5, false>), grid, block, 0, st, views, ref, edges, P, y0, nrows, wbuf, wstride, pconst);
+		if (wi) hipLaunchKernelGGL((geodesic_reg_kernel<5, true>), grid, block, 0, st, views, ref, edges, P, y0, nrows, wbuf, wstride, pconst, cb);
+		else    hipLaunchKernelGGL((geodesic_reg_kernel<5, false>), grid, block, 0, st, views, ref, edges, P, y0, nrows, wbuf, wstride, pconst, cb);
 		return true;
 	case 2:
-		if (wi) hipLaunchKernelGGL((geodesic_reg_kernel<2, true>), grid, block, 0, st, views, ref, edges, P, y0, nrows, wbuf, wstride, pconst);
-		else    hipLaunchKernelGGL((geodesic_reg_kernel<2, false>), grid, block, 0, st, views, ref, edges, P, y0, nrows, wbuf, wstride, pconst);
+		if (wi) hipLaunchKernelGGL((geodesic_reg_kernel<2, true>), grid, block, 0, st, views, ref, edges, P, y0, nrows, wbuf, wstride, pconst, cb);
+		else    hipLaunchKernelGGL((geodesic_reg_kernel<2, false>), grid, block, 0, st, views, ref, edges, P, y0, nrows, wbuf, wstride, pconst, cb);
 		return true;
 	default: return false;
 	}
diff --git a/stereoreconstruction_amd/csrc/srh_internal.hpp b/stereoreconstruction_amd/csrc/srh_internal.hpp
--- a/stereoreconstruction_amd/csrc/srh_internal.hpp
+++ b/stereoreconstruction_amd/csrc/srh_internal.hpp
@@ -56,6 +56,9 @@
 __host__ __device__ inline bool cert_sure(double x, double clamp, double m_hi) { return x == clamp || x > m_hi; }
 __host__ __device__ inline bool cert_pixel_exact(const CertBound &cb, double sum2, double all_taps_usable) {
 	return !(all_taps_usable != 0.0) || !(cb.sigma3(sum2) < __builtin_inf());
+}
+__host__ __device__ inline double pconst_sigma3(const CertBound &cb, double sum2) {
+	return cb.ok ? cb.sigma3(sum2) : __builtin_inf();
 }
 #ifdef __HIPCC__
 __device__ __forceinline__ double onepass_finish(double P, double Q, double U, double SA, double itw, double s2, double TT,
@@ -140,7 +143,7 @@
                       double *gray, double *gray_tv);
 void launch_fill(hipStream_t st, double *p, size_t n, double v);
 #define SRH_PC 6
-void launch_weights(hipStream_t st, const ViewDev *views, int ref, int width, const srh_params &P,
+void launch_weights(hipStream_t st, const ViewDev *views, int ref, int width, const srh_params &P, const CertBound &cb,
                     int y0, int nrows, double *wbuf, size_t wstride, double *pconst = nullptr, bool wimg = false);
 void launch_twoview_generic(hipStream_t st, const ViewDev *views, int ref, int oth, int width, const srh_params &P,
                             int y0, int nrows, const double *wbuf, size_t wstride, Counters *cnt, bool sad = false,
@@ -158,12 +161,12 @@
 size_t geo5_doubles(int w, int h);
 void launch_geo5_planes(hipStream_t st, const double *edges, const double *gray_tv, const uint8_t *mask, int w, int h, double *out);
 bool launch_geodesic_dma(hipStream_t st, const ViewDev *views, int ref, int width, const double *geo5, const srh_params &P,
-                         int y0, int nrows, double *wbuf, double *pconst, int num_cus);
+                         const CertBound &cb, int y0, int nrows, double *wbuf, double *pconst, int num_cus);
 bool launch_geodesic_reg(hipStream_t st, const ViewDev *views, int ref, int width, const double *edges,
-                         const srh_params &P, int y0, int nrows, double *wbuf, size_t wstride, double *pconst = nullptr,
-                         bool wimg = false);
-bool launch_adaptive_reg(hipStream_t st, const ViewDev *views, int ref, int width, const srh_params &P, int y0, int nrows,
-                         double *wbuf, size_t wstride, double *pconst = nullptr, bool wimg = false);
+                         const srh_params &P, const CertBound &cb, int y0, int nrows, double *wbuf, size_t wstride,
+                         double *pconst = nullptr, bool wimg = false);
+bool launch_adaptive_reg(hipStream_t st, const ViewDev *views, int ref, int width, const srh_params &P, const CertBound &cb,
+                         int y0, int nrows, double *wbuf, size_t wstride, double *pconst = nullptr, bool wimg = false);
 void launch_label_plane_table(hipStream_t st, const ViewDev *views, int ref, const srh_params &P, bool mvs, double *tdist);
 void launch_pinhole_label_table(hipStream_t st, const ViewDev *views, int ref, const srh_params &P, bool mvs, double *tnum);
 bool launch_twoview_dense_cost_f32(hipStream_t st, const ViewDev *views, int ref, int oth, int width, const srh_params &P,
@@ -197,9 +200,12 @@
                         int y0, int nrows, const double *tnum, int cstride, PixRange *prange);
 int  strip_chunk_columns();
 int  strip_block_lanes(int cstride, int form);
+struct TileRec { int32_t cmin_raw, cmax; uint32_t flags, pad; };
+void launch_tile_records(hipStream_t st, int width, int y0, int nrows, const PixRange *prange, const double *pconst,
+                         const uint8_t *oth_fullp, int lanes, TileRec *trec);
 bool launch_twoview_strip_cost(hipStream_t st, const ViewDev *views, int ref, int oth, int width, int height,
                                const srh_params &P, int y0, int nrows, const double *wimg, const double *pconst,
-                               const PixRange *prange, const double *ref_tvp, const double *oth_tvp,
+                               const PixRange *prange, const TileRec *trec, const double *ref_tvp, const double *oth_tvp,
                                const uint8_t *oth_fullp, double *cost, int cstride, Counters *cnt, int arith, int num_cus,
                                int lanes, bool raw = false);
 
diff --git a/stereoreconstruction_amd/csrc/srh_kernels.hip b/stereoreconstruction_amd/csrc/srh_kernels.hip
--- a/stereoreconstruction_amd/csrc/srh_kernels.hip
+++ b/stereoreconstruction_amd/csrc/srh_kernels.hip
@@ -47,7 +47,7 @@
 
 __global__ void weights_kernel(const ViewDev *__restrict__ views, int ref, srh_params P,
                                int y0, int nrows, double *__restrict__ wbuf, size_t wstride, double *__restrict__ pconst,
-                               int wimg)
+                               int wimg, const CertBound cb)
 {
 	const ViewDev &V = views[ref];
 	const int W = V.w, H = V.h;
@@ -86,17 +86,17 @@
 		} else all = false;
 		double *pc = pconst + ((size_t)(q / W)*W + cx)*SRH_PC;
 		pc[0] = mL; pc[1] = tw; pc[2] = s2; pc[3] = all ? 1.0/tw : 0.0;
-		pc[4] = sa; pc[5] = 0.0;
+		pc[4] = sa; pc[5] = pconst_sigma3(cb, s2);
 	}
 #undef WTAP
 }
 
-void launch_weights(hipStream_t st, const ViewDev *views, int ref, int width, const srh_params &P,
+void launch_weights(hipStream_t st, const ViewDev *views, int ref, int width, const srh_params &P, const CertBound &cb,
                     int y0, int nrows, double *wbuf, size_t wstride, double *pconst, bool wimg)
 {
 	const size_t n = (size_t)nrows*width;
 	hipLaunchKernelGGL(weights_kernel, dim3((unsigned)((n + 255)/256)), dim3(256), 0, st,
-	                   views, ref, P, y0, nrows, wbuf, wstride, pconst, wimg ? 1 : 0);
+	                   views, ref, P, y0, nrows, wbuf, wstride, pconst, wimg ? 1 : 0, cb);
 }
 
 template <bool SAD, bool WTA>
diff --git a/stereoreconstruction_amd/csrc/srh_strip.hip b/stereoreconstruction_amd/csrc/srh_strip.hip
--- a/stereoreconstruction_amd/csrc/srh_strip.hip
+++ b/stereoreconstruction_amd/csrc/srh_strip.hip
@@ -86,11 +86,65 @@
 
 int strip_chunk_columns() { return ST_CHUNK; }
 
+template <int G>
+__global__ void tile_record_kernel(int W, int y0, int nrows, const PixRange *__restrict__ prange, const double *__restrict__ pconst,
+                                   const uint8_t *__restrict__ oth_fullp, TileRec *__restrict__ trec)
+{
+	const int tiles_per_row = (W + ST_TP - 1)/ST_TP;
+	const int t = (int)(blockIdx.x*blockDim.x + threadIdx.x);
+	if (t >= nrows*tiles_per_row) return;
+	const int r = t / tiles_per_row, x0 = (t - r*tiles_per_row)*ST_TP;
+	const size_t px0 = (size_t)r*W + x0;
+	const int np = W - x0 < ST_TP ? W - x0 : ST_TP;
+	int mn = 2147483647, mx = -2147483647;
+	bool bad = false;
+#pragma unroll 8
+	for (int pi = 0; pi < ST_TP; ++pi) {
+		const size_t qi = px0 + (pi < np ? pi : 0);
+		const PixRange q = prange[qi];
+		const double itw = pconst[qi*SRH_PC + 3];
+		const bool live = pi < np && q.hi >= q.lo;
+		const int hi = dense_cover_hi(q.lo, q.hi, ST_NCB, G, G == 8);
+		mn = live && q.lo < mn ? q.lo : mn;
+		mx = live && hi > mx ? hi : mx;
+		bad = bad || (live && !(itw != 0.0));
+	}
+	if (!bad && mn <= mx) {
+		const int SP = padded_stride(W);
+		const int c0 = mn > -SRH_PADL ? mn : -SRH_PADL, c1 = mx < W + SRH_PADR - 1 ? mx : W + SRH_PADR - 1;
+		bad = c0 != mn || c1 != mx;
+		const size_t a0 = (size_t)(y0 + r + SRH_PADY)*SP + (size_t)(c0 + SRH_PADL), a1 = a0 + (size_t)(c1 - c0);
+		const uint32_t *wp = reinterpret_cast<const uint32_t *>(oth_fullp);
+		const size_t k0 = a0 >> 2, k1 = a1 >> 2;
+		uint32_t acc = 0x01010101u;
+#pragma unroll 4
+		for (size_t k = k0; k <= k1; ++k) {
+			uint32_t v = wp[k];
+			if (k == k0) v |= (1u << 8*(a0 & 3)) - 1u;
+			if (k == k1 && (a1 & 3) != 3) v |= ~0u << 8*((a1 & 3) + 1);
+			acc &= v;
+		}
+		bad = bad || (acc & 0x01010101u) != 0x01010101u;
+	}
+	TileRec rec; rec.cmin_raw = mn; rec.cmax = mx; rec.flags = bad ? 1u : 0u; rec.pad = 0;
+	trec[t] = rec;
+}
+
+void launch_tile_records(hipStream_t st, int width, int y0, int nrows, const PixRange *prange, const double *pconst,
+                         const uint8_t *oth_fullp, int lanes, TileRec *trec)
+{
+	const int n = nrows*((width + ST_TP - 1)/ST_TP);
+	const dim3 grid((unsigned)((n + 63)/64)), block(64);
+	if (lanes == 8) hipLaunchKernelGGL(tile_record_kernel<8>, grid, block, 0, st, width, y0, nrows, prange, pconst, oth_fullp, trec);
+	else            hipLaunchKernelGGL(tile_record_kernel<16>, grid, block, 0, st, width, y0, nrows, prange, pconst, oth_fullp, trec);
+}
+
 struct StripArgs {
 	int W, H, y0, nrows;
 	const double *wimg;
 	const double *pconst;
 	const PixRange *prange;
+	const TileRec *trec;
 	const double *ref_tvp, *oth_tvp;
 	const uint8_t *oth_fullp;
 	double *cost; int cstride;
@@ -128,6 +182,7 @@
 	alignas(16) double lt[NS][LW];
 	alignas(16) double pc[2][ST_TP][SRH_PC];
 	alignas(16) PixRange pr[2][ST_TP];
+	alignas(16) TileRec trec[2];
 	alignas(16) unsigned char full[2][FW];
 	unsigned short glist[GL_CAP];
 	int glist_n, gsingle_n;
@@ -371,7 +426,11 @@
 		auto issue_tile_inputs = [&](int r, int buf, int wb, bool consts, bool windows) {
 			const size_t px0 = (size_t)r*W + x0;
 			if (consts && wv == 0) st_dma16(A.pconst + px0*SRH_PC, &S.pc[buf][0][0], ST_TP*SRH_PC*8, lane);
-			if (consts && wv == 1) st_dma4(A.prange + px0, &S.pr[buf][0], ST_TP*8, lane);
+			if (consts && wv == 1) {
+				st_dma4(A.prange + px0, &S.pr[buf][0], ST_TP*8, lane);
+				if (!BORDER && lane == 0)
+					__builtin_amdgcn_global_load_lds((st_gbl_void *)(A.trec + ((size_t)r*tiles_per_row + tx)), (st_lds_void *)&S.trec[buf], 16, 0, 0);
+			}
 			if (windows) {
 				const double *wt = A.wimg + ((size_t)r*tiles_per_row + tx)*(size_t)(ST_TP*WPIX);
 				if (NBUF == 1) {
@@ -416,7 +475,14 @@
 			ST_STAMP(2);
 
 			int cmin, cmax, cmin_raw;
-			{
+			bool need_general = false;
+			if (!BORDER) {
+				const int4 rec = *reinterpret_cast<const int4 *>(&CS.trec[cur]);
+				cmin_raw = __builtin_amdgcn_readfirstlane(rec.x);
+				cmax = __builtin_amdgcn_readfirstlane(rec.y);
+				need_general = (__builtin_amdgcn_readfirstlane(rec.z) & 1) != 0;
+				cmin = cmin_raw & ~1;
+			} else {
 				const int pi = lane & 31;
 				const PixRange q = CS.pr[cur][pi];
 				int lo = q.lo, hi = q.hi;
@@ -509,8 +575,7 @@
 				__syncthreads();
 			}
 
-			bool need_general = false;
-			{
+			if (BORDER) {
 				const int pi = lane & 31;
 				const PixRange q = CS.pr[cur][pi];
 				const bool live = x0 + pi < W && q.hi >= q.lo;
@@ -535,7 +600,7 @@
 				if (e_max >= e_min) e_max = dense_cover_hi(e_min, e_max, NCB, G, PAD);
 			}
 			const bool lall = CS.pc[cur][i][3] != 0.0;
-			const double sig3 = CERT ? A.cb.sigma3(CS.pc[cur][i][2]) : 0.0;
+			const double sig3 = CERT ? CS.pc[cur][i][5] : 0.0;
 			const bool pix_exact = CERT && A.redo && !(sig3 < __builtin_inf());
 			const size_t tile = (size_t)r*tiles_per_row + tx;
 			ST_STAMP(3);
@@ -755,42 +820,55 @@
 			ST_STAMP(4);
 			if (need_general) {
 				if (tid == 0) { S.glist_n = 0; S.gsingle_n = 0; }
+				if (!BORDER && wv == 0) {
+#pragma unroll
+					for (int it = 0; it < (CHUNK + 63)/64 + 1; ++it) {
+						const int k = it*64 + lane;
+						const unsigned long long m = __ballot(k < CHUNK + NCB && rfull[k] == 0);
+						if (lane == 0) S.badcols[it] = m;
+					}
+				}
 				__syncthreads();
-				for (int p = tid; p < ST_TP*Smem::NBMAX; p += NT) {
-					const int pi = p / Smem::NBMAX, b = p % Smem::NBMAX;
+				static_assert(NT >= ST_TP*((Smem::NBMAX + 7)/8), "one pass over the (pixel, run) pairs");
+				if (tid < ST_TP*((Smem::NBMAX + 7)/8)) {
+					const int pi = tid & (ST_TP - 1), run = tid / ST_TP;
 					const PixRange q = CS.pr[cur][pi];
 					int qlo = q.lo, qhi = q.hi;
 					if (x0 + pi >= W) { qlo = 0; qhi = -1; }
 					if (qhi >= qlo) qhi = dense_cover_hi(qlo, qhi, NCB, G, PAD);
 					if (qhi > cs + CHUNK - 1) qhi = cs + CHUNK - 1;
-					if (qhi < qlo) continue;
-					const int c0 = (PAD ? (qlo & ~1) : qlo) + b*NCB;
-					if (c0 > qhi) continue;
-					const bool pall = CS.pc[cur][pi][3] != 0.0;
-					unsigned need = 0xffu;
-					if (qlo > c0) need &= 0xffu << (qlo - c0);
-					if (c0 + NCB - 1 > qhi) need &= 0xffu >> (c0 + NCB - 1 - qhi);
-					if (pall) {
-						const int rc = c0 - cs, wd = rc >> 6, sh = rc & 63;
-						unsigned long long bits = CS.badcols[wd] >> sh;
-						if (sh) bits |= CS.badcols[wd + 1] << (64 - sh);
-						need &= (unsigned)bits;
-					}
-					if (!need) continue;
-					bool as_block = __builtin_popcount(need) == NCB;
-					if (!as_block) {
-						const int at = atomicAdd(&S.gsingle_n, __builtin_popcount(need));
-						if (at + __builtin_popcount(need) <= Smem::GL_SINGLES) {
-							int k = 0;
-#pragma unroll
-							for (int j = 0; j < NCB; ++j)
-								if ((need >> j) & 1u) { S.glist[Smem::GL_CAP - 1 - (at + k)] = (unsigned short)(pi*512 + (c0 + j - cs)); ++k; }
-						} else {
-							for (int k = at; k < at + __builtin_popcount(need) && k < Smem::GL_SINGLES; ++k) S.glist[Smem::GL_CAP - 1 - k] = 0xffffu;
-							as_block = true;
+					const int cw = (PAD ? (qlo & ~1) : qlo) + run*8*NCB;
+					unsigned long long bits = 0;
+					if (qhi >= qlo && cw <= qhi) {
+						const int b0 = qlo > cw ? qlo - cw : 0, b1 = qhi - cw < 63 ? qhi - cw : 63;
+						bits = (~0ull << b0) & (~0ull >> (63 - b1));
+						if (CS.pc[cur][pi][3] != 0.0) {
+							const int rc = cw - cs, wd = rc >> 6, sh = rc & 63;
+							unsigned long long bad = CS.badcols[wd] >> sh;
+							if (sh) bad |= CS.badcols[wd + 1] << (64 - sh);
+							bits &= bad;
 						}
 					}
-					if (as_block) S.glist[atomicAdd(&S.glist_n, 1)] = (unsigned short)(pi*64 + b);
+					while (bits) {
+						const int j = (__builtin_ctzll(bits) >> 3), b = run*8 + j;
+						const unsigned need = (unsigned)(bits >> 8*j) & 0xffu;
+						bits &= ~(0xffull << 8*j);
+						const int c0 = cw + j*NCB;
+						bool as_block = __builtin_popcount(need) == NCB;
+						if (!as_block) {
+							const int at = atomicAdd(&S.gsingle_n, __builtin_popcount(need));
+							if (at + __builtin_popcount(need) <= Smem::GL_SINGLES) {
+								int k = 0;
+#pragma unroll
+								for (int jj = 0; jj < NCB; ++jj)
+									if ((need >> jj) & 1u) { S.glist[Smem::GL_CAP - 1 - (at + k)] = (unsigned short)(pi*512 + (c0 + jj - cs)); ++k; }
+							} else {
+								for (int k = at; k < at + __builtin_popcount(need) && k < Smem::GL_SINGLES; ++k) S.glist[Smem::GL_CAP - 1 - k] = 0xffffu;
+								as_block = true;
+							}
+						}
+						if (as_block) S.glist[atomicAdd(&S.glist_n, 1)] = (unsigned short)(pi*64 + b);
+					}
 				}
 				__syncthreads();
 				ST_STAMP(5);
@@ -876,6 +954,7 @@
 		m.wimg = a.wimg + tiles*(ST_TP*StripSmem<R, NBUF>::WPIX);
 		m.pconst = a.pconst + (size_t)t*a.W*SRH_PC;
 		m.prange = a.prange + (size_t)t*a.W;
+		m.trec = a.trec + tiles;
 		m.cost = a.cost + tiles*(size_t)a.cstride*ST_TP;
 		strip_items(m);
 		if (arith == 5) launch_strip_variant<R, NWV, NBUF, 5, false>(st, m, num_cus);
@@ -899,14 +978,14 @@
 
 bool launch_twoview_strip_cost(hipStream_t st, const ViewDev *views, int ref, int oth, int width, int height,
                                const srh_params &P, int y0, int nrows, const double *wimg, const double *pconst,
-                               const PixRange *prange, const double *ref_tvp, const double *oth_tvp,
+                               const PixRange *prange, const TileRec *trec, const double *ref_tvp, const double *oth_tvp,
                                const uint8_t *oth_fullp, double *cost, int cstride, Counters *cnt, int arith, int num_cus,
                                int lanes, bool raw)
 {
 	(void)views; (void)ref; (void)oth;
 	StripArgs a;
 	a.W = width; a.H = height; a.y0 = y0; a.nrows = nrows;
-	a.wimg = wimg; a.pconst = pconst; a.prange = prange;
+	a.wimg = wimg; a.pconst = pconst; a.prange = prange; a.trec = trec;
 	a.ref_tvp = ref_tvp; a.oth_tvp = oth_tvp; a.oth_fullp = oth_fullp;
 	a.cost = cost; a.cstride = cstride; a.cnt = cnt;
 	a.weight_cutoff = P.weight_cutoff; a.bad_ret = P.bad_ret; a.max_color_diff = P.max_color_diff;
```

Result: no change. 46360 Mhyp/s, median of 6 (+1.0%).
